# geloescht/mxnet-maintenance

Measured on AMD Instinct MI355X. Metric: images/sec (whole node) ResNet-50 fp16 batch 256/GPU at 1/2/4/8 MI355X, higher is better.
Workload: dtype fp16; 1 GPU; model=ResNet-50 v1b, global_batch=256, per_gpu_batch=256, image_size=224, parallelism=dp1, layout=NHWC, optimizer=mp-SGD momentum 0.9, lr 0.1 (linear warm-up 40 steps), hip_graph=True, deterministic=True

## Files before the change

mxnet_maintenance_amd/ops/kernel_fns.py:

```python
import os

import torch

from . import kernels as _K
from .. import _state
from ..utils import env as _env

__all__ = ['BatchNormNHWC', 'BatchNormDualTailNHWC', 'SoftmaxCE', 'GlobalAvgPoolNHWC', 'flat_sgd']

_DT = {torch.float32: 0, torch.float16: 1, torch.bfloat16: 2}


def _stream():
    return torch.cuda.current_stream().cuda_stream


def _p(t):
    return 0 if t is None else t.data_ptr()


def _f32(t):
    if t.dtype == torch.float32 and t.is_contiguous():
        return t
    m = getattr(t, '_mxamd_master', None)
# ... 314 lines not shown
        zout = torch.empty(5, C, dtype=torch.float32, device=dev)
        dg_ptr, db_ptr, accum, direct, _k1 = _bn_param_grad_dst(gamma_ref, beta_ref, need[2], need[3], out, C, dev)
        zdg_ptr, zdb_ptr, zaccum, zdirect, _k2 = _bn_param_grad_dst(zgamma_ref, zbeta_ref, need[4], need[5], zout, C,
                                                                    dev)
        ride = training and _BN_TAIL_DS[0]
        dkw, zpart, znblk = {}, None, 0
        if ride:
            znblk = lib.bn_tail_ds_rows(R, C)
            zpart = torch.empty(2 * znblk * C, dtype=torch.float32, device=dev)
            dkw = dict(ds_z=z.data_ptr(), ds_mean=zmean.data_ptr(), ds_part=zpart.data_ptr())
        else:
            zpart = torch.empty(2 * lib.bn_partials_rows(R, C) * C, dtype=torch.float32, device=dev)
        lib.bn_nhwc_backward(dt, x.data_ptr(), gy.data_ptr(), 0, mask.data_ptr(), dx.data_ptr(), 0, g.data_ptr(),
                             mean.data_ptr(), invstd.data_ptr(), 0, 0, part.data_ptr(), dg_ptr, db_ptr,
                             out[2].data_ptr(), R, C, 3, 0, int(training), accum, _stream(), ext_nblk, **dkw)
        lib.bn_nhwc_backward(dt, z.data_ptr(), gy.data_ptr(), 0, mask.data_ptr(), dzs.data_ptr(), 0, zg.data_ptr(),
                             zmean.data_ptr(), zinvstd.data_ptr(), 0, 0, zpart.data_ptr(), zdg_ptr, zdb_ptr,
                             zout[2].data_ptr(), R, C, 3, 0, int(training), zaccum, _stream(), znblk)
        dgamma = None if direct or not need[2] else out[0].to(gdt)
        dbeta = None if direct or not need[3] else out[1].to(bdt)
        zdgamma = None if zdirect or not need[4] else zout[0].to(zgdt)
        zdbeta = None if zdirect or not need[5] else zout[1].to(zbdt)
        return dx, dzs, dgamma, dbeta, zdgamma, zdbeta, None, None, None, None, None, None, None


def bnrelu_pool_ok(x, kernel, stride, pad):
    return (bn_ok(x) and tuple(kernel) == (3, 3) and pool_ok(x, kernel, stride, pad)
            and x.numel() + 256 * 32 * 256 * 8 < 2 ** 31 and hasattr(_K.lib(), 'pool_nhwc_forward_bnrelu'))


class SoftmaxCE(torch.autograd.Function):

    @staticmethod
    def forward(ctx, logits, label):
        lib = _K.lib()
        N, K = logits.shape
        lab = label.reshape(-1)
        is_int = not lab.is_floating_point()
        lab = lab.to(torch.int64).contiguous() if is_int else lab.float().contiguous()
        loss = torch.empty(N, dtype=torch.float32, device=logits.device)
        lse = torch.empty(N, dtype=torch.float32, device=logits.device)
        lib.softmax_ce_forward(_DT[logits.dtype], int(is_int), logits.data_ptr(), lab.data_ptr(), loss.data_ptr(),
                               lse.data_ptr(), N, K, _stream())
        ctx.save_for_backward(logits, lab, lse)
        ctx.is_int = is_int
        return loss

    @staticmethod
    def backward(ctx, gout):
        lib = _K.lib()
        logits, lab, lse = ctx.saved_tensors
        N, K = logits.shape
        g = gout.float().contiguous()
        dl = torch.empty_like(logits)
        lib.softmax_ce_backward(_DT[logits.dtype], int(ctx.is_int), logits.data_ptr(), lab.data_ptr(),
                                lse.data_ptr(), g.data_ptr(), dl.data_ptr(), N, K, _stream())
        return dl, None


class GlobalAvgPoolNHWC(torch.autograd.Function):
    @staticmethod
    def forward(ctx, x):
        lib = _K.lib()
        x = x.contiguous()
        N, C = x.shape[0], x.shape[-1]
        HW = x.numel() // (N * C)
        y = torch.empty((N,) + (1,) * (x.dim() - 2) + (C,), dtype=x.dtype, device=x.device)
        lib.gap_nhwc_forward(_DT[x.dtype], x.data_ptr(), y.data_ptr(), N, HW, C, _stream())
        ctx.shape = x.shape
        return y

    @staticmethod
    def backward(ctx, gy):
        lib = _K.lib()
        shape = ctx.shape
        N, C = shape[0], shape[-1]
        HW = int(torch.tensor(shape[1:-1]).prod())
        gy = gy.contiguous()
        dx = torch.empty(shape, dtype=gy.dtype, device=gy.device)
        lib.gap_nhwc_backward(_DT[gy.dtype], gy.data_ptr(), dx.data_ptr(), N, HW, C, _stream())
        return dx


def gap_ok(x):
    return x.dtype in _DT and x.is_contiguous() and x.shape[-1] % 8 == 0


class ReluHip(torch.autograd.Function):

    @staticmethod
    def forward(ctx, x):
        x = x.contiguous()
        y = torch.empty_like(x)
        _K.lib().relu_forward(_DT[x.dtype], x.data_ptr(), y.data_ptr(), x.numel(), _stream())
        ctx.save_for_backward(y)
        return y

    @staticmethod
    def backward(ctx, gy):
        y, = ctx.saved_tensors
        gy = gy.contiguous()
        dx = torch.empty_like(y)
        _K.lib().relu_backward(_DT[y.dtype], y.data_ptr(), gy.data_ptr(), dx.data_ptr(), y.numel(), _stream())
        return dx


def relu_ok(x):
    return x.dtype in _DT and x.is_cuda and x.numel() > 0 and x.data_ptr() % 16 == 0 and x.is_contiguous()


_PW_OPS = {'add': 0, 'sub': 1, 'mul': 2, 'div': 3, 'maximum': 4, 'minimum': 5}


def _bcast_strides(t, shape):
    lead = len(shape) - t.dim()
    st = [0] * lead + list(t.stride())
    sz = [1] * lead + list(t.shape)
    return [0 if sz[d] == 1 and shape[d] != 1 else st[d] for d in range(len(shape))]


def _collapse(shape, sa, sb):
    dims = [(n, a, b) for n, a, b in zip(shape, sa, sb) if n != 1] or [(1, 0, 0)]
    out = [list(dims[-1])]
    for n, a, b in reversed(dims[:-1]):
        pn, pa, pb = out[0]
        if a == pa * pn and b == pb * pn:
            out[0] = [n * pn, pa, pb]
        else:
            out.insert(0, [n, a, b])
    return [d[0] for d in out], [d[1] for d in out], [d[2] for d in out]


def _is_row(t, full):
    ts = tuple(t.shape)
    while ts and ts[0] == 1:
        ts = ts[1:]
    return len(ts) <= len(full) and ts == full[len(full) - len(ts):]


def binary_hip(op, a, b):
    shape = torch.broadcast_shapes(a.shape, b.shape)
    out = torch.empty(shape, dtype=a.dtype, device=a.device)
    n = out.numel()
    if n == 0:
        return out
    vec = 4 if a.dtype == torch.float32 else 8
    aligned = a.data_ptr() % 16 == 0 and b.data_ptr() % 16 == 0
    mode, row = 3, 0
    full = tuple(shape)
    if aligned and a.is_contiguous() and b.is_contiguous():
        if tuple(a.shape) == full and tuple(b.shape) == full:
            mode = 0
        elif tuple(a.shape) == full and _is_row(b, full) and b.numel() % vec == 0:
            mode, row = 1, b.numel()
        elif tuple(b.shape) == full and _is_row(a, full) and a.numel() % vec == 0:
            mode, row = 2, a.numel()
    if mode == 3:
        shp, sa, sb = _collapse(list(shape), _bcast_strides(a, shape), _bcast_strides(b, shape))
        if len(shp) > 6:
            return {'add': torch.add, 'sub': torch.sub, 'mul': torch.mul, 'div': torch.div,
                    'maximum': torch.maximum, 'minimum': torch.minimum}[op](a, b)
    else:
        shp, sa, sb = [], [], []
    _K.lib().pointwise_binary(_DT[a.dtype], _PW_OPS[op], a.data_ptr(), b.data_ptr(), out.data_ptr(), n, mode, row,
                              shp, sa, sb, _stream())
    return out


def _sum_to(g, shape):
    if tuple(g.shape) == tuple(shape):
        return g
    return g.sum_to_size(shape) if len(shape) else g.sum()


class BinaryHip(torch.autograd.Function):

    @staticmethod
    def forward(ctx, a, b, op):
        ctx.op = op
        ctx.sa, ctx.sb = tuple(a.shape), tuple(b.shape)
        if op in ('mul', 'div', 'maximum', 'minimum'):
            ctx.save_for_backward(a, b)
        return binary_hip(op, a, b)

    @staticmethod
    def backward(ctx, g):
        op = ctx.op
        g = g.contiguous()
        if op == 'add':
            return _sum_to(g, ctx.sa), _sum_to(g, ctx.sb), None
        if op == 'sub':
            return _sum_to(g, ctx.sa), _sum_to(-g, ctx.sb), None
        a, b = ctx.saved_tensors
        if op == 'mul':
            return _sum_to(binary_hip('mul', g, b), ctx.sa), _sum_to(binary_hip('mul', g, a), ctx.sb), None
        if op == 'div':
            ga = binary_hip('div', g, b)
            gb = -binary_hip('div', binary_hip('mul', ga, a), b)
            return _sum_to(ga, ctx.sa), _sum_to(gb, ctx.sb), None
        take_a = (a >= b) if op == 'maximum' else (a <= b)
        ga = torch.where(take_a, g, torch.zeros_like(g))
        return _sum_to(ga, ctx.sa), _sum_to(g - ga, ctx.sb), None


def binary_ok(a, b):
    return (a.is_cuda and b.is_cuda and a.dtype == b.dtype and a.dtype in _DT and a.numel() > 0 and
            b.numel() > 0 and a.device == b.device)


__all__ += ['ReluHip', 'relu_ok', 'BinaryHip', 'binary_ok', 'binary_hip']




def flat_sgd(w, g, mom, w32, lr, wd, momentum, rescale, clip, hp=None):
    lib = _K.lib()
    n = w.numel()
    assert n % 8 == 0 and g.numel() == n and w.dtype == g.dtype and w.dtype in _DT
    assert mom is None or (mom.dtype == torch.float32 and mom.numel() == n)
    assert w32 is None or (w32.dtype == torch.float32 and w32.numel() == n)
    if momentum == 0.0:
        mom = None
    args = (_DT[w.dtype], w.data_ptr(), g.data_ptr(), _p(mom), _p(w32), n, float(lr), float(wd),
            float(momentum), float(rescale), float(clip), _stream())
    lib.flat_sgd(*args) if hp is None else lib.flat_sgd(*args, hp.data_ptr())



import os as _os

_CONV_HIP = _env.get('MXAMD_CONV_HIP') != 0


def conv_ok_shape(x, w, stride, pad, dilate=(1, 1), groups=1):
    return (_CONV_HIP and x.dim() == 4 and w.dim() == 4 and groups == 1 and tuple(dilate) == (1, 1)
            and x.dtype in (torch.float16, torch.bfloat16) and w.dtype == x.dtype
            and x.is_contiguous() and w.is_contiguous() and x.shape[3] % 32 == 0 and w.shape[0] % 64 == 0
            and w.shape[3] == x.shape[3] and x.numel() < 2 ** 31 and x.data_ptr() % 16 == 0
            and w.data_ptr() % 16 == 0)


def stem_ok(x, w, stride, pad, bias=None):
    return (_CONV_HIP and bias is None and x.dim() == 4 and w.dim() == 4 and x.dtype in (torch.float16, torch.bfloat16)
            and w.dtype == x.dtype and x.is_contiguous() and w.is_contiguous() and 1 <= x.shape[3] <= 4
            and w.shape[3] == x.shape[3] and w.shape[0] == 64 and w.shape[1] <= 8 and w.shape[2] <= 8
            and tuple(stride) == (2, 2) and all(0 <= p < 8 for p in pad) and _K.available()
            and hasattr(_K.lib(), 'conv_stem_fwd'))


def conv_stem_fwd(x, w, pad, bn_stats=False):
    N, H, W, C = x.shape
    K, R, S, _ = w.shape
    Ho = (H + 2 * pad[0] - R) // 2 + 1
    Wo = (W + 2 * pad[1] - S) // 2 + 1
    y = torch.empty((N, Ho, Wo, K), dtype=x.dtype, device=x.device)
    lib = _K.lib()
    part, nparts = None, 0
    if bn_stats:
        nparts = 4 * lib.conv_stem_grid(N, H, W, R, S, pad[0], pad[1])
        part = torch.empty(2 * K * nparts, dtype=torch.float32, device=x.device)
    lib.conv_stem_fwd(_DT[x.dtype], x.data_ptr(), w.data_ptr(), y.data_ptr(), N, H, W, C, K, R, S, 2, 2, pad[0],
                      pad[1], _p(part), nparts, _stream())
    if part is not None:
        y._mxamd_bn_part = (part, nparts)
    return y


def conv_stem_wgrad(x, dy, wshape, pad, out=None, accum=False):
    N, H, W, C = x.shape
    K, R, S, _ = wshape
    dy = dy.contiguous()
    lib = _K.lib()
    slab = torch.empty(lib.conv_stem_wgrad_workspace(N, H, W, R, S, pad[0], pad[1]), dtype=torch.float32,
                       device=x.device)
    if out is None:
        out = torch.empty((K, R, S, C), dtype=x.dtype, device=x.device)
        accum = False
    assert out.is_contiguous() and out.numel() == K * R * S * C and out.dtype in _DT
    lib.conv_stem_wgrad(_DT[x.dtype], x.data_ptr(), dy.data_ptr(), slab.data_ptr(), _DT[out.dtype], out.data_ptr(),
                        int(bool(accum)), N, H, W, C, K, R, S, 2, 2, pad[0], pad[1], _stream())
    return out


_BIG_VARIANTS = {10: (256, 256), 11: (128, 256), 12: (64, 512), 13: (256, 128), 14: (128, 256), 15: (256, 128),
                 16: (256, 256), 17: (128, 256), 18: (64, 512), 19: (256, 128),
                 26: (256, 224), 27: (128, 448)}
_BIG_SKINNY = (14, 15)
_SKINNY_ON = os.environ.get('MXAMD_CONV_SKINNY', '0') == '1'
_RING_VARIANTS = {20: (128, 128), 21: (256, 128), 22: (128, 256), 23: (64, 256), 24: (256, 256), 25: (64, 128)}


def conv_up2_ok(dy, w, stride, pad, xshape):
    K, R, S, C = w.shape
    return (_CONV_HIP and R == 1 and S == 1 and tuple(stride) == (2, 2) and tuple(pad) == (0, 0)
            and dy.dtype in (torch.float16, torch.bfloat16) and dy.is_cuda and dy.dim() == 4 and K % 64 == 0
            and xshape[1] == 2 * dy.shape[1] and xshape[2] == 2 * dy.shape[2] and xshape[3] == C)


def conv_dgrad_up2(dy, w, variant, bn_bwd=None):
    wt = _dgrad_weight(w.contiguous())
    return conv_fwd(dy.contiguous(), wt, (1, 1), (0, 0), None, variant, bn_bwd=bn_bwd, up=2)


def conv_fwd(x, w, stride, pad, bias=None, variant=0, bn_stats=False, addend=None, bn_bwd=None, up=0, dil=(1, 1)):
    N, H, W, C = x.shape
    K, R, S, _ = w.shape
    dil = tuple(dil)
    Ho = (H + 2 * pad[0] - dil[0] * (R - 1) - 1) // stride[0] + 1
    Wo = (W + 2 * pad[1] - dil[1] * (S - 1) - 1) // stride[1] + 1
    assert dil == (1, 1) or (variant in _BIG_VARIANTS and not bn_stats and bn_bwd is None and up == 0), \
        'conv_fwd: dilation runs on the big-tile kernel without fused epilogues'
    assert up in (0, 2) and (up == 0 or (variant in _BIG_VARIANTS and addend is None and not bn_stats))
    y = torch.empty((N, Ho * max(up, 1), Wo * max(up, 1), K), dtype=x.dtype, device=x.device)
    if N * Ho * Wo * K >= 2 ** 31:
        raise ValueError('conv_fwd: output too large for 32-bit indexing')
    b = _f32(bias) if bias is not None else None
    if addend is not None:
        assert variant in _BIG_VARIANTS and addend.shape == y.shape and addend.dtype == y.dtype
        addend = addend.contiguous()
    if variant in _RING_VARIANTS:
        assert bias is None and addend is None, 'conv ring kernel: no bias / addend'
        lib = _K.lib()
        v = variant - 20
        part, nparts = None, 0
        if bn_stats:
            nparts = lib.conv_nhwc_fwd_ring_nparts(N, H, W, R, S, stride[0], stride[1], pad[0], pad[1], v)
            part = torch.empty(2 * K * nparts, dtype=torch.float32, device=x.device)
        lib.conv_nhwc_fwd_ring(_DT[x.dtype], x.data_ptr(), w.data_ptr(), y.data_ptr(), _zero_page(x.device).data_ptr(),
                               N, H, W, C, K, R, S, stride[0], stride[1], pad[0], pad[1], v, _p(part), nparts,
                               _stream())
        if part is not None:
            y._mxamd_bn_part = (part, nparts)
        return y
    if variant in _BIG_VARIANTS:
        lib = _K.lib()
        v = variant - 10
        part, nparts = None, 0
        if bn_stats:
            nparts = lib.conv_nhwc_fwd_big_nparts(N, H, W, R, S, stride[0], stride[1], pad[0], pad[1], v)
            part = torch.empty(2 * K * nparts, dtype=torch.float32, device=x.device)
        bkw = {}
        if bn_bwd is not None:
            z, bmean, bscale, bshift, bmask, bmode, token = bn_bwd
            assert z.shape == y.shape and z.dtype == y.dtype and z.is_contiguous()
            bnp = lib.conv_nhwc_fwd_big_bwd_nparts(N, H, W, R, S, stride[0], stride[1], pad[0], pad[1], v)
            bpart = torch.empty(2 * K * bnp, dtype=torch.float32, device=x.device)
            bkw = dict(bn_z=z.data_ptr(), bn_mean=bmean.data_ptr(), bn_scale=_p(bscale), bn_shift=_p(bshift),
                       bn_mask=_p(bmask), bn_mode=int(bmode), bn_part=bpart.data_ptr(), bn_nparts=bnp)
        lib.conv_nhwc_fwd_big(_DT[x.dtype], x.data_ptr(), w.data_ptr(), _p(b), y.data_ptr(),
                              _zero_page(x.device).data_ptr(), N, H, W, C, K, R, S, stride[0], stride[1],
                              pad[0], pad[1], v, _p(part), nparts, _p(addend), _stream(), up=int(up), dh=dil[0],
                              dw=dil[1], **bkw)
        if bkw:
            y._mxamd_bn_bwd = (bpart, bnp, bn_bwd[6], y._version)
        if part is not None:
            y._mxamd_bn_part = (part, nparts)
        return y
    if variant in (5, 6):
        lib = _K.lib()
        bco = 128 if variant == 5 else 64
        bkw = _glds_bnb(bn_bwd, y, lib.conv_glds_bwd_nparts(N * Ho * Wo, bco))
        part = bkw.pop('_part', None)
        lib.conv_nhwc_fwd_glds(_DT[x.dtype], x.data_ptr(), w.data_ptr(), _p(b), y.data_ptr(),
                               _zero_page(x.device).data_ptr(), N, H, W, C, K, R, S, stride[0], stride[1],
                               pad[0], pad[1], bco, _stream(), **bkw)
        if part is not None:
            y._mxamd_bn_bwd = (part, bkw['bn_nparts'], bn_bwd[6], y._version)
        return y
    _K.lib().conv_nhwc_fwd(_DT[x.dtype], x.data_ptr(), w.data_ptr(), _p(b), y.data_ptr(), N, H, W, C, K, R, S,
                           stride[0], stride[1], pad[0], pad[1], int(variant), _stream())
    return y


def halo_ok(x, w, stride, pad):
    K, R, S, C = w.shape
    return (_CONV_HIP and x.is_cuda and x.dtype in (torch.float16, torch.bfloat16) and x.dim() == 4
            and x.is_contiguous() and w.is_contiguous() and x.data_ptr() % 16 == 0 and w.data_ptr() % 16 == 0
            and hasattr(_K.lib(), 'conv3x3_halo')
            and bool(_K.lib().conv3x3_halo_ok(C, K, R, S, stride[0], stride[1], pad[0], pad[1], x.shape[2])))


def conv_halo(x, w, bn_stats=False, bn_bwd=None):
    N, H, W, C = x.shape
    K = w.shape[0]
    lib = _K.lib()
    y = torch.empty((N, H, W, K), dtype=x.dtype, device=x.device)
    nparts = lib.conv3x3_halo_nparts(N, H)
    part = torch.empty(2 * K * nparts, dtype=torch.float32, device=x.device) if (bn_stats or bn_bwd) else None
    kw = {}
    if bn_bwd is not None:
        z, bmean, bscale, bshift, _bmask, bmode, _token = bn_bwd
        assert int(bmode) in (0, 2) and z.shape == y.shape and z.dtype == y.dtype and z.is_contiguous()
        kw = dict(bn_z=z.data_ptr(), bn_mean=bmean.data_ptr(), bn_scale=_p(bscale), bn_shift=_p(bshift),
                  bn_mode=int(bmode), bn_part=part.data_ptr())
    lib.conv3x3_halo(_DT[x.dtype], x.data_ptr(), w.data_ptr(), y.data_ptr(), _zero_page(x.device).data_ptr(), N, H,
                     W, C, K, _p(part) if bn_bwd is None else 0, nparts if bn_bwd is None else 0, s=_stream(), **kw)
    if bn_bwd is not None:
        y._mxamd_bn_bwd = (part, nparts, bn_bwd[6], y._version)
    elif part is not None:
        y._mxamd_bn_part = (part, nparts)
    return y


def glds_bnb_ok(bn_src):
    return bn_src is not None and int(bn_src[5]) in (0, 2) and hasattr(_K.lib(), 'conv_glds_bwd_nparts')


def _glds_bnb(bn_bwd, y, nparts):
    if bn_bwd is None:
        return {}
    z, bmean, bscale, bshift, _bmask, bmode, _token = bn_bwd
    assert int(bmode) in (0, 2) and z.shape == y.shape and z.dtype == y.dtype and z.is_contiguous()
    part = torch.empty(2 * y.shape[-1] * nparts, dtype=torch.float32, device=y.device)
    return dict(bn_z=z.data_ptr(), bn_mean=bmean.data_ptr(), bn_scale=_p(bscale), bn_shift=_p(bshift),
                bn_part=part.data_ptr(), bn_nparts=nparts, _part=part)


_ZERO = {}


def _zero_page(dev):
    z = _ZERO.get(dev)
    if z is None:
        z = _ZERO[dev] = torch.zeros(128, dtype=torch.float16, device=dev)
    return z


def _fwd_variants(C, K, bias=False, ktot=None):
    v = []
    if C % 64 == 0 and not bias:
        v.extend(b for b, (bco, _bpix) in sorted(_RING_VARIANTS.items()) if K % bco == 0)
    if C % 64 == 0:
        v.extend(b for b, (bco, _bpix) in sorted(_BIG_VARIANTS.items())
                 if K % bco == 0 and (b not in _BIG_SKINNY or (_SKINNY_ON and ktot == 64)))
    if C % 64 == 0 and K % 128 == 0:
        v.append(5)
    if C % 64 == 0:
        v.append(6)
    if K % 128 == 0 and C % 64 == 0:
        v.append(1)
    if K % 128 == 0:
        v.append(2)
    if C % 64 == 0:
        v.append(3)
    v.append(4)
    return v


def conv_wgrad_ok(x, w):
    return (_CONV_HIP and x.dim() == 4 and w.dim() == 4 and x.dtype in (torch.float16, torch.bfloat16)
            and x.is_contiguous() and x.shape[3] % 64 == 0 and w.shape[0] % 64 == 0 and w.shape[3] == x.shape[3]
            and x.numel() < 2 ** 31 and x.data_ptr() % 16 == 0)


def conv_wgrad(x, dy, wshape, stride, pad, out=None, accum=False, dma=True, ring=0, dil=(1, 1)):
    N, H, W, C = x.shape
    K, R, S, _ = wshape
    dy = dy.contiguous()
    assert dy.dtype == x.dtype and dy.shape[0] == N and dy.shape[3] == K
    dh, dw = dil
    Ho = (H + 2 * pad[0] - dh * (R - 1) - 1) // stride[0] + 1
    Wo = (W + 2 * pad[1] - dw * (S - 1) - 1) // stride[1] + 1
    assert tuple(dy.shape[1:3]) == (Ho, Wo), 'conv_wgrad: dy shape does not match the conv geometry'
    assert dy.numel() < 2 ** 31 and dy.data_ptr() % 16 == 0
    lib = _K.lib()
    if ring:
        ws = lib.conv_nhwc_wgrad_ring_workspace(N, H, W, C, K, R, S, stride[0], stride[1], pad[0], pad[1], ring,
                                                dh=dh, dw=dw)
    else:
        ws = lib.conv_nhwc_wgrad_workspace(N, H, W, C, K, R, S, stride[0], stride[1], pad[0], pad[1], dh=dh, dw=dw)
    slab = torch.empty(ws, dtype=torch.float32, device=x.device)
    if out is None:
        out = torch.empty((K, R, S, C), dtype=x.dtype, device=x.device)
        accum = False
    assert out.is_contiguous() and out.numel() == K * R * S * C and out.dtype in _DT
    if ring:
        lib.conv_nhwc_wgrad_ring(_DT[x.dtype], x.data_ptr(), dy.data_ptr(), slab.data_ptr(), _DT[out.dtype],
                                 out.data_ptr(), int(bool(accum)), N, H, W, C, K, R, S, stride[0], stride[1], pad[0],
                                 pad[1], _zero_page(x.device).data_ptr(), int(ring), _stream(), dh=dh, dw=dw)
        return out
    lib.conv_nhwc_wgrad(_DT[x.dtype], x.data_ptr(), dy.data_ptr(), slab.data_ptr(), _DT[out.dtype], out.data_ptr(),
                        int(bool(accum)), N, H, W, C, K, R, S, stride[0], stride[1], pad[0], pad[1],
                        _zero_page(x.device).data_ptr() if dma else 0, _stream(), dh=dh, dw=dw)
    return out


def _taps_t(w, out, src, base, rstride):
    K, R, S, C = w.shape
    for i in range(0, len(src), 32):
        _K.lib().weight_taps_t(w.element_size(), w.data_ptr(), out.data_ptr(), K, R * S, C, src[i:i + 32],
                               base[i:i + 32], rstride[i:i + 32], _stream())
    return out


def _dgrad_weight(w):
    K, R, S, C = w.shape
    if not (w.is_cuda and w.is_contiguous() and w.element_size() in (2, 4) and _K.available()):
        return w.flip(1, 2).permute(3, 1, 2, 0).contiguous()
    T = R * S
    out = torch.empty((C, R, S, K), dtype=w.dtype, device=w.device)
    return _taps_t(w, out, [T - 1 - t for t in range(T)], [t * K for t in range(T)], [T * K] * T)


def transpose2d(w):
    R, C = w.shape
    if w.is_cuda and w.is_contiguous() and w.element_size() in (2, 4) and R % 8 == 0 and C % 8 == 0:
        return _dgrad_weight(w.view(R, 1, 1, C)).view(C, R)
    return w.t().contiguous()


def _phase_taps(R, P, s, ph):
    return sorted(((ph + P - r) // s, r) for r in range(R) if (ph + P - r) % s == 0)


def conv_dgrad_strided_ok(dy, w, stride, pad, xshape, bco=128):
    K, R, S, C = w.shape
    s = tuple(stride)
    return (_CONV_HIP and s != (1, 1) and s[0] == s[1] and s[0] <= 2 and dy.dtype in (torch.float16, torch.bfloat16)
            and dy.dim() == 4 and K % 64 == 0 and C % bco == 0 and xshape[1] % s[0] == 0 and xshape[2] % s[1] == 0
            and dy.is_cuda and all(0 <= p < k for p, k in zip(pad, (R, S))))


_PHASE_PLANS = {}


def _phase_plan(wshape, stride, pad, device):
    key = (tuple(wshape), tuple(stride), tuple(pad), device)
    plan = _PHASE_PLANS.get(key)
    if plan is not None:
        return plan
    K, R, S, C = wshape
    st = stride[0]
    phases, empty, idx, off = [], [], [], 0
    for ph in range(st):
        th = _phase_taps(R, pad[0], st, ph)
        for pw in range(st):
            tw = _phase_taps(S, pad[1], st, pw)
            if not th or not tw:
                empty.append((ph, pw))
                continue
            dh = [d for d, _ in th]
            dw = [d for d, _ in tw]
            if dh != list(range(dh[0], dh[0] + len(dh))) or dw != list(range(dw[0], dw[0] + len(dw))):
                raise ValueError('conv_dgrad_strided: non-contiguous phase taps')
            nt = len(th) * len(tw)
            for i, (_, r) in enumerate(th):
                for j, (_, c) in enumerate(tw):
                    idx.append((r * S + c, off + (i * len(tw) + j) * K, nt * K))
            phases.append((ph, pw, len(th), len(tw), -dh[0], -dw[0], off))
            off += C * nt * K
    plan = (phases, empty, (idx, off))
    _PHASE_PLANS[key] = plan
    return plan


def conv_dgrad_strided(dy, w, stride, pad, xshape, bco=128, bn_bwd=None):
    K, R, S, C = w.shape
    N, H, W, _ = xshape
    st = stride[0]
    Ho, Wo = H // st, W // st
    dy = dy.contiguous()
    phases, empty, gidx = _phase_plan(w.shape, stride, pad, w.device)
    if len(phases) > 4:
        raise ValueError('conv_dgrad_strided: at most 4 phases per launch')
    dx = torch.empty((N, H, W, C), dtype=dy.dtype, device=dy.device)
    if len(empty) > 3:
        raise ValueError('conv_dgrad_strided: at most 3 phases without taps')
    slots, total = gidx
    wsub = _taps_t(w.contiguous(), torch.empty(total, dtype=w.dtype, device=w.device), [t[0] for t in slots],
                   [t[1] for t in slots], [t[2] for t in slots])
    cols = list(zip(*phases))
    lib = _K.lib()
    bkw = _glds_bnb(bn_bwd, dx, len(phases) * lib.conv_glds_bwd_nparts(N * Ho * Wo, bco)) if bn_bwd else {}
    part = bkw.pop('_part', None)
    lib.conv_nhwc_dgrad_phases_glds(_DT[dy.dtype], dy.data_ptr(), wsub.data_ptr(), dx.data_ptr(),
                                    _zero_page(dy.device).data_ptr(), N, dy.shape[1], dy.shape[2], K, C, Ho, Wo,
                                    st, list(cols[0]), list(cols[1]), list(cols[2]), list(cols[3]),
                                    list(cols[4]), list(cols[5]), list(cols[6]), [e[0] for e in empty],
                                    [e[1] for e in empty], bco, _stream(), **bkw)
    if part is not None:
        dx._mxamd_bn_bwd = (part, bkw['bn_nparts'], bn_bwd[6], dx._version)
    return dx


def _conv_bwd_torch(dy, x, w, stride, pad, mask):
    xc = x.permute(0, 3, 1, 2)
    wc = w.permute(0, 3, 1, 2)
    dyc = dy.permute(0, 3, 1, 2)
    dx, dw, _ = torch.ops.aten.convolution_backward(dyc, xc, wc, None, list(stride), list(pad), [1, 1], False,
                                                    [0, 0], 1, [mask[0], mask[1], False])
    if dx is not None:
        dx = dx.permute(0, 2, 3, 1)
    if dw is not None:
        dw = dw.permute(0, 2, 3, 1)
    return dx, dw



_AUTOTUNE = _env.get('MXNET_CUDNN_AUTOTUNE_DEFAULT') > 0
_ALGO = {}
_TIMES = {}


_REJECTED = {}


def _rel_err(a, b):
    a = a.float()
    b = b.float()
    return float((a - b).abs().max() / (b.abs().max() + 1e-6))


_VENDOR = ('mm', 'miopen')
_VENDOR_PREFIX = ('splitk', 'blaslt', 'sk')
_VENDOR_MARGIN = float(os.environ.get('MXAMD_VENDOR_MARGIN', '0.03'))


def _is_vendor(name):
    return name in _VENDOR or name.startswith(_VENDOR_PREFIX)
_TUNE_ROUNDS = int(os.environ.get('MXAMD_TUNE_ROUNDS', '2'))


def _time_candidates(cands, reps=3, key=None, tol=2e-2):
    ref = None
    ref_name = next((n for n, _ in cands if n in ('mm', 'miopen')), None)
    if ref_name is not None:
        ref = dict(cands)[ref_name]()
        if isinstance(ref, torch.Tensor):
            ref = ref.detach().clone()
        else:
            ref = None
    ok = []
    for name, fn in cands:
        if ref is not None and name != ref_name:
            r = fn()
            if isinstance(r, torch.Tensor) and r.shape == ref.shape:
                err = _rel_err(r, ref)
                if not err <= tol:
                    _REJECTED.setdefault(key, {})[name] = err
                    continue
        ok.append((name, fn))
    times, outs = {}, {}
    for _ in range(_TUNE_ROUNDS):
        for name, fn in ok:
            fn()
            t, r = _measure(fn, reps)
            if name not in times or t < times[name]:
                times[name] = t
                outs[name] = r
    names = [n for n, _ in cands]
    agreed = _agree_times([times.get(n, float('inf')) for n in names])
    best, best_t = None, None
    for name, t in zip(names, agreed):
        if t == float('inf'):
            continue
        if key is not None:
            _TIMES.setdefault(key, {})[name] = t / reps
        if _is_vendor(name):
            t *= 1.0 + _VENDOR_MARGIN
        if best_t is None or t < best_t:
            best, best_t = name, t
    if best is not None and best not in outs:
        best = None
    return best, (outs[best] if best is not None else None)


def _measure(fn, reps):
    if torch.cuda.is_available():
        s, e = torch.cuda.Event(enable_timing=True), torch.cuda.Event(enable_timing=True)
        s.record()
        for _ in range(reps):
            r = fn()
        e.record()
        e.synchronize()
        return s.elapsed_time(e), r
    import time
    t0 = time.perf_counter()
    for _ in range(reps):
        r = fn()
    return (time.perf_counter() - t0) * 1e3, r


def _agree_times(vals):
    from ..parallel import dist
    if dist.world_size() <= 1 or not vals:
        return vals
    t = torch.tensor(vals, dtype=torch.float64)
    dist.all_reduce(t, op='max')
    return [float(v) for v in t.tolist()]


_DETERMINISTIC = [_env.get('MXNET_ENFORCE_DETERMINISM') != 0]
_NONDET = ('mm', 'miopen', 'sk', 'splitk', 'bmm', 'blaslt')


def _apply_torch_determinism(flag):
    torch.backends.cudnn.deterministic = bool(flag)
    if flag:
        torch.backends.cudnn.benchmark = False
    try:
        torch.use_deterministic_algorithms(bool(flag), warn_only=True)
    except Exception:
        pass


def set_deterministic(flag):
    _DETERMINISTIC[0] = bool(flag)
    _apply_torch_determinism(flag)


def deterministic():
    return _DETERMINISTIC[0]


if _DETERMINISTIC[0]:
    _apply_torch_determinism(True)


def _det_filter(cands):
    if not _DETERMINISTIC[0] or cands is None:
        return cands
    keep = [(n, f) for n, f in cands if not n.startswith(_NONDET)]
    return keep or cands


def _akey(key):
    return key + ('det',) if _DETERMINISTIC[0] else key


_FILE_ALGO = {}
_FILE_STATE = {'loaded': False}


def _tuning_file():
    return os.environ.get('MXAMD_AUTOTUNE_FILE', '')


def _load_tuning_file():
    if _FILE_STATE['loaded']:
        return
    _FILE_STATE['loaded'] = True
    path = _tuning_file()
    if path and os.path.exists(path):
        import json
        try:
            with open(path) as f:
                _FILE_ALGO.update(json.load(f))
        except (OSError, ValueError):
            pass


def _save_tuning_file(key, name):
    path = _tuning_file()
    if not path or name is None:
        return
    from ..parallel import dist
    if dist.rank() != 0:
        return
    import json
    _FILE_ALGO[repr(key)] = name
    tmp = path + '.tmp'
    try:
        with open(tmp, 'w') as f:
            json.dump(_FILE_ALGO, f, indent=0, sort_keys=True)
        os.replace(tmp, path)
    except OSError:
        pass


def _select(key, cands, default, timing=None):
    key = _akey(key)
    cands = _det_filter(cands)
    timing = _det_filter(timing)
    _load_tuning_file()
    name = _ALGO.get(key)
    if name is None:
        name = _FILE_ALGO.get(repr(key))
        if name is not None and name in dict(cands):
            _ALGO[key] = name
    if name is None:
        if _AUTOTUNE and not torch.cuda.is_current_stream_capturing() and len(cands) > 1:
            name, out = _time_candidates(timing or cands, key=key)
            _ALGO[key] = name
            _save_tuning_file(key, name)
            return out
        name = default
    table = dict(cands)
    return (table[name] if name in table else cands[0][1])()


_NCU = {}


def _num_cus(dev):
    n = _NCU.get(dev)
    if n is None:
        n = _NCU[dev] = torch.cuda.get_device_properties(dev).multi_processor_count
    return n


def pw_ok(x, kin, nout):
    return (_CONV_HIP and x.is_cuda and x.dtype in (torch.float16, torch.bfloat16) and x.is_contiguous()
            and x.data_ptr() % 16 == 0 and hasattr(_K.lib(), 'conv_pw_stream')
            and bool(_K.lib().conv_pw_stream_ok(int(kin), int(nout))))


def pw_bnb_ok(kin, nout, add, bn_src):
    return (bn_src is not None and int(bn_src[5]) in (2, 3) and hasattr(_K.lib(), 'conv_pw_stream_bnb_ok')
            and bool(_K.lib().conv_pw_stream_bnb_ok(int(kin), int(nout), int(bool(add)), int(bn_src[5]))))


def conv_pw(x, w2, bn_stats=False, addend=None, bn_bwd=None, addend_mask=None):
    C = x.shape[-1]
    K = w2.shape[0]
    M = x.numel() // C
    wt = int(w2.dim() == 2 and w2.stride() == (1, K) and not w2.is_contiguous() and w2.data_ptr() % 16 == 0
             and K % 8 == 0)
    if not wt:
        w2 = w2.contiguous()
    y = torch.empty(x.shape[:-1] + (K,), dtype=x.dtype, device=x.device)
    if addend is not None:
        addend = addend.contiguous()
        if tuple(addend.shape) != tuple(y.shape) or addend.dtype != y.dtype or addend.data_ptr() % 16:
            raise ValueError('conv_pw: addend must match the output (shape, dtype, 16-byte alignment)')
    lib = _K.lib()
    grid = lib.conv_pw_stream_grid(M, C, K, _num_cus(x.device), int(addend is not None or bn_bwd is not None))
    nparts = grid // max(1, lib.conv_pw_stream_slices(C, K))
    part = torch.empty(2 * K * nparts, dtype=torch.float32, device=x.device) if (bn_stats or bn_bwd) else None
    bkw = {}
    if bn_bwd is not None:
        assert not bn_stats, 'conv_pw: forward and backward statistics are exclusive'
        z, bmean, bscale, bshift, bmask, bmode, _token = bn_bwd
        assert z.shape == y.shape and z.dtype == y.dtype and z.is_contiguous() and z.data_ptr() % 16 == 0
        bkw = dict(bn_z=z.data_ptr(), bn_mask=_p(bmask), bn_mean=bmean.data_ptr(), bn_scale=_p(bscale),
                   bn_shift=_p(bshift), bn_mode=int(bmode))
    if addend_mask is not None:
        assert bn_bwd is not None and addend is not None and addend_mask.dtype == torch.uint8
        assert addend_mask.numel() * 8 == addend.numel() and addend_mask.is_contiguous()
        bkw['addend_mask'] = addend_mask.data_ptr()
    lib.conv_pw_stream(_DT[x.dtype], x.data_ptr(), w2.data_ptr(), y.data_ptr(), _zero_page(x.device).data_ptr(), M, C,
                       K, _p(part), grid, _stream(), _p(addend), wt, **bkw)
    if bn_bwd is not None:
        y._mxamd_bn_bwd = (part, nparts, bn_bwd[6], y._version)
    elif part is not None:
        y._mxamd_bn_part = (part, nparts)
    return y


def _fwd_candidates(x, w, stride, pad, bias):
    c = []
    K, R, S, C = w.shape
    if (R == 1 and S == 1 and tuple(stride) == (1, 1) and tuple(pad) == (0, 0) and bias is None
            and pw_ok(x, C, K)):
        c.append(('pw', lambda: conv_pw(x, w.reshape(K, C), bn_stats=bool(_state.STATE.training))))
    if stem_ok(x, w, stride, pad, bias):
        c.append(('stem', lambda: conv_stem_fwd(x, w, pad, bn_stats=bool(_state.STATE.training))))
    if bias is None and halo_ok(x, w, stride, pad):
        c.append(('halo', lambda: conv_halo(x, w, bn_stats=bool(_state.STATE.training))))
    if conv_ok_shape(x, w, stride, pad):
        c.append(('hip', lambda: conv_fwd(x, w, stride, pad, bias)))
        stats = bool(_state.STATE.training)
        for v in _fwd_variants(C, K, bias is not None, ktot=R * S * C):
            c.append(('hip%d' % v, lambda v=v: conv_fwd(x, w, stride, pad, bias, v, bn_stats=stats)))
    if R == 1 and S == 1 and tuple(stride) == (1, 1) and tuple(pad) == (0, 0):
        x2, w2 = x.reshape(-1, C), w.reshape(K, C)
        for name, fn in _gemm().candidates(x2, w2, bias=bias):
            c.append((name, lambda fn=fn: fn().view(x.shape[0], x.shape[1], x.shape[2], K)))

        def mm():
            y = torch.mm(x.reshape(-1, C), w.reshape(K, C).t())
            if bias is not None:
                y = y + bias.to(y.dtype)
            return y.view(x.shape[0], x.shape[1], x.shape[2], K)
        c.append(('mm', mm))

    def miopen():
        y = torch.nn.functional.conv2d(x.permute(0, 3, 1, 2), w.permute(0, 3, 1, 2), bias, tuple(stride), tuple(pad))
        return y.permute(0, 2, 3, 1).contiguous()
    c.append(('miopen', miopen))
    return c


_STATS_SCRATCH = {}


def _bn_stats_pass(y):
    C = y.shape[-1]
    R = y.numel() // C
    lib = _K.lib()
    n = 2 * lib.bn_partials_rows(R, C) * C
    buf = _STATS_SCRATCH.get(y.device)
    if buf is None or buf.numel() < n:
        buf = _STATS_SCRATCH[y.device] = torch.empty(n, dtype=torch.float32, device=y.device)
    lib.bn_nhwc_stats(_DT[y.dtype], y.data_ptr(), _zeros_f32(C, y.device).data_ptr(), buf.data_ptr(), R, C,
                      _stream())


def _fwd_timing(cands):
    if not _state.STATE.training:
        return None

    def charged(fn):
        def run():
            y = fn()
            if getattr(y, '_mxamd_bn_part', None) is None and y.shape[-1] % 8 == 0 and y.is_contiguous():
                _bn_stats_pass(y)
            return y
        return run
    return [(n, charged(fn)) for n, fn in cands]


def _fwd_default(x, w, stride):
    K, R, S, C = w.shape
    if C <= 4 and K == 64 and tuple(stride) == (2, 2) and R <= 8 and S <= 8:
        return 'stem'
    if R == 1 and S == 1 and tuple(stride) == (1, 1) and (K >= 256 or x.shape[1] * x.shape[2] <= 784):
        return 'mm'
    return 'hip'


def _dgrad_candidates(dy, x, w, stride, pad):
    c = []
    K, R, S, C = w.shape
    if R == 1 and S == 1 and tuple(stride) == (1, 1) and tuple(pad) == (0, 0):
        c.append(('mm', lambda: torch.mm(dy.reshape(-1, K), w.reshape(K, C)).view(x.shape)))
        if pw_ok(dy, K, C):
            c.append(('pw', lambda: conv_pw(dy, w.reshape(K, C).t())))
        c.extend(_gemm_dgrad_1x1(dy, w, x.shape))
    if (tuple(stride) == (1, 1) and C % 64 == 0 and K % 32 == 0 and 2 * pad[0] == R - 1 and 2 * pad[1] == S - 1
            and _CONV_HIP):
        c.append(('hip', lambda: conv_fwd(dy, _dgrad_weight(w), (1, 1), (R - 1 - pad[0], S - 1 - pad[1]))))
        for v in _fwd_variants(K, C, ktot=R * S * K):
            c.append(('hip%d' % v, lambda v=v: conv_fwd(dy, _dgrad_weight(w), (1, 1), (R - 1 - pad[0], S - 1 - pad[1]),
                                                        None, v)))
    for bco in (128, 64):
        if conv_dgrad_strided_ok(dy, w, stride, pad, x.shape, bco):
            c.append(('phase%d' % bco, lambda bco=bco: conv_dgrad_strided(dy, w, stride, pad, x.shape, bco)))
    if halo_ok(dy, w, stride, pad) and tuple(dy.shape) == tuple(x.shape[:3]) + (K,):
        c.append(('halo', lambda: conv_halo(dy, _dgrad_weight(w))))
    if conv_up2_ok(dy, w, stride, pad, x.shape):
        for v, (bco, _bpix) in sorted(_BIG_VARIANTS.items()):
            if C % bco == 0 and v not in _BIG_SKINNY:
                c.append(('up%d' % v, lambda v=v: conv_dgrad_up2(dy, w, v)))
    c.append(('miopen', lambda: _conv_bwd_torch(dy, x, w, stride, pad, (True, False))[0]))
    return c


def _gemm():
    from . import gemm
    return gemm


def _gemm_dgrad_1x1(dy, w, xshape, addend=None):
    K, C = w.shape[0], w.shape[3]
    G = _gemm()
    d2 = dy.reshape(-1, K)
    if not (K % 64 == 0 and C % 64 == 0 and d2.is_cuda and d2.dtype in G._DT and w.dtype == d2.dtype
            and d2.is_contiguous() and d2.data_ptr() % 16 == 0 and _K.available()):
        return []
    out = []
    for cfg in G.configs(d2.shape[0], C, K, G.AUTOTUNE_TILES):
        def run(cfg=cfg):
            add = addend.contiguous().view(-1, C) if addend is not None else None
            return G.gemm_nt(d2, transpose2d(w.reshape(K, C)), addend=add, cfg=cfg).view(xshape)
        out.append(('gemm%ds%d' % cfg, run))
    return out


def _big_algo(key):
    algo = _ALGO.get(_akey(key))
    if algo and algo.startswith('hip') and algo[3:].isdigit() and int(algo[3:]) in _BIG_VARIANTS:
        return int(algo[3:])
    return None


def _bn_bwd_fusable(bn_src, out_shape):
    return bn_src is not None and _BN_BWD_FUSE[0] and tuple(bn_src[0].shape) == tuple(out_shape)


def _charge_bn_bwd(cands, z):
    def charged(fn):
        def run():
            r = fn()
            if isinstance(r, torch.Tensor) and r.shape[-1] % 8 == 0 and r.is_contiguous():
                _bn_stats_pass(r)
                _bn_stats_pass(z)
            return r
        return run
    return [(n, charged(fn)) for n, fn in cands]


def _dgrad_bn_candidates(dy, x, w, stride, pad, bn_src):
    cands = _dgrad_candidates(dy, x, w, stride, pad)
    K, R, S, C = w.shape
    fused = []
    if (R == 1 and S == 1 and tuple(stride) == (1, 1) and tuple(pad) == (0, 0) and pw_ok(dy, K, C)
            and pw_bnb_ok(K, C, False, bn_src)):
        fused.append(('pw+bn', lambda: conv_pw(dy, w.reshape(K, C).t(), bn_bwd=bn_src)))
    if (_CONV_HIP and tuple(stride) == (1, 1) and 2 * pad[0] == R - 1 and 2 * pad[1] == S - 1
            and K % 64 == 0):
        for v in _fwd_variants(K, C, ktot=R * S * K):
            if v in _BIG_VARIANTS or (v in (5, 6) and glds_bnb_ok(bn_src)):
                fused.append(('hip%d+bn' % v, lambda v=v: conv_fwd(dy, _dgrad_weight(w), (1, 1),
                                                                   (R - 1 - pad[0], S - 1 - pad[1]), None, v,
                                                                   bn_bwd=bn_src)))
    if conv_up2_ok(dy, w, stride, pad, x.shape):
        for v, (bco, _bpix) in sorted(_BIG_VARIANTS.items()):
            if C % bco == 0 and v not in _BIG_SKINNY:
                fused.append(('up%d+bn' % v, lambda v=v: conv_dgrad_up2(dy, w, v, bn_bwd=bn_src)))
    if glds_bnb_ok(bn_src) and halo_ok(dy, w, stride, pad) and tuple(dy.shape) == tuple(x.shape[:3]) + (K,):
        fused.append(('halo+bn', lambda: conv_halo(dy, _dgrad_weight(w), bn_bwd=bn_src)))
    if glds_bnb_ok(bn_src):
        for bco in (128, 64):
            if conv_dgrad_strided_ok(dy, w, stride, pad, x.shape, bco):
                fused.append(('phase%d+bn' % bco, lambda bco=bco: conv_dgrad_strided(dy, w, stride, pad, x.shape, bco,
                                                                                     bn_bwd=bn_src)))
    return cands + fused, _charge_bn_bwd(cands, bn_src[0]) + fused


def _dgrad_default(w, stride):
    K, R, S, C = w.shape
    if tuple(stride) != (1, 1):
        return 'miopen'
    if R == 1 and S == 1:
        return 'mm' if C >= 128 else 'miopen'
    return 'hip' if C >= 128 and C % 64 == 0 else 'miopen'


def _wgrad_candidates(dy, x, w, stride, pad):
    c = [('miopen', lambda: _conv_bwd_torch(dy, x, w, stride, pad, (False, True))[1])]
    K, R, S, C = w.shape
    if stem_ok(x, w, stride, pad):
        c.insert(0, ('stem', lambda: conv_stem_wgrad(x, dy, w.shape, pad)))
    if conv_wgrad_ok(x, w):
        c.insert(0, ('hip', lambda: conv_wgrad(x, dy, w.shape, stride, pad)))
        c.insert(1, ('hipreg', lambda: conv_wgrad(x, dy, w.shape, stride, pad, dma=False)))
        lib = _K.lib()
        for v in range(1, 10):
            if lib.conv_nhwc_wgrad_ring_ok(C, K, R, S, v):
                c.insert(2, ('ring%d' % v, lambda v=v: conv_wgrad(x, dy, w.shape, stride, pad, ring=v)))
    if R == 1 and S == 1 and tuple(stride) == (1, 1) and tuple(pad) == (0, 0):
        P = dy.numel() // K
        for chunks in (16, 64):
            if P % chunks == 0 and P // chunks >= 1024:
                def splitk(chunks=chunks):
                    return _splitk_wgrad(dy, x, chunks)
                c.append(('splitk%d' % chunks, splitk))
    return c


_BMM_OUT_DTYPE = [None]


def _splitk_wgrad(dy, x, chunks, out=None):
    K, C = dy.shape[-1], x.shape[-1]
    P = dy.numel() // K
    d3 = dy.reshape(chunks, P // chunks, K).transpose(1, 2)
    x3 = x.reshape(chunks, P // chunks, C)
    part = _bmm_f32(d3, x3)
    if not part.is_contiguous() or (K * C) % 4:
        r = part.sum(0).view(K, 1, 1, C)
        if out is not None:
            out.add_(r.view(out.shape))
            return None
        return r
    lib = _K.lib()
    if out is None:
        r = torch.empty(K, 1, 1, C, dtype=torch.float32, device=dy.device)
        lib.slab_reduce(0, part.data_ptr(), chunks, K * C, r.data_ptr(), 0, _stream())
        return r
    lib.slab_reduce(_DT[out.dtype], part.data_ptr(), chunks, K * C, out.data_ptr(), 1, _stream())
    return None


def _bmm_f32(a, b):
    if _BMM_OUT_DTYPE[0] is not False:
        try:
            r = torch.bmm(a, b, out_dtype=torch.float32)
            _BMM_OUT_DTYPE[0] = True
            return r
        except (RuntimeError, TypeError):
            _BMM_OUT_DTYPE[0] = False
    return torch.bmm(a, b).float()


def _wgrad(dy, x, w, w_ref, stride, pad):
    key = ('wgrad', tuple(x.shape), tuple(w.shape), tuple(stride), tuple(pad), x.dtype)
    algo = _ALGO.get(_akey(key))
    if algo == 'stem':
        tgt = _leaf_grad(w_ref, dtype=w.dtype)
        if tgt is not None:
            conv_stem_wgrad(x, dy, w.shape, pad, out=tgt, accum=True)
            return None
    if algo in ('hip', 'hipreg') or (algo or '').startswith('ring'):
        tgt = _leaf_grad(w_ref, dtype=w.dtype)
        if tgt is not None:
            conv_wgrad(x, dy, w.shape, stride, pad, out=tgt, accum=True, dma=algo == 'hip',
                       ring=int(algo[4:]) if algo.startswith('ring') else 0)
            return None
    elif algo is not None and algo.startswith('splitk'):
        tgt = _leaf_grad(w_ref, dtype=w.dtype)
        if tgt is not None:
            _splitk_wgrad(dy, x, int(algo[6:]), out=tgt)
            return None
    default = 'stem' if stem_ok(x, w, stride, pad) else ('hip' if conv_wgrad_ok(x, w) else 'miopen')
    dw = _select(key, _wgrad_candidates(dy, x, w, stride, pad), default)
    if dw.dtype != w.dtype:
        tgt = _leaf_grad(w_ref, dtype=w.dtype)
        if tgt is not None:
            tgt.add_(dw)
            return None
        dw = dw.to(w.dtype)
    return dw


_WGRAD_SIDE = [os.environ.get('MXAMD_WGRAD_STREAM', '0') == '1']
_SIDE_STREAMS = {}
_SIDE_KEEP = []
_SIDE_DIRTY = set()


def join_side_streams():
    if not _SIDE_DIRTY:
        return
    for dev in list(_SIDE_DIRTY):
        torch.cuda.current_stream(dev).wait_stream(_SIDE_STREAMS[dev])
    _SIDE_DIRTY.clear()
    del _SIDE_KEEP[:]


def _wgrad_maybe_side(dy, x, w, w_ref, stride, pad):
    if not (_WGRAD_SIDE[0] and dy.is_cuda):
        return _wgrad(dy, x, w, w_ref, stride, pad)
    dev = dy.device.index
    side = _SIDE_STREAMS.get(dev)
    if side is None:
        side = _SIDE_STREAMS[dev] = torch.cuda.Stream(device=dev)
        from .. import engine
        engine.add_join_hook(join_side_streams)
    main = torch.cuda.current_stream(dev)
    side.wait_stream(main)
    with torch.cuda.stream(side):
        dw = _wgrad(dy, x, w, w_ref, stride, pad)
    _SIDE_KEEP.append((dy, x))
    _SIDE_DIRTY.add(dev)
    if dw is not None:
        main.wait_stream(side)
        dw.record_stream(main)
    return dw


class ConvNHWC(torch.autograd.Function):

    @staticmethod
    def forward(ctx, x, w, bias, stride, pad, dilate):
        key = ('fwd', tuple(x.shape), tuple(w.shape), tuple(stride), tuple(pad), x.dtype, bias is not None)
        cands = _fwd_candidates(x, w, stride, pad, bias)
        y = _select(key, cands, _fwd_default(x, w, stride), timing=_fwd_timing(cands))
        ctx.save_for_backward(x, w)
        ctx.stride, ctx.pad = stride, pad
        ctx.has_bias = bias is not None
        ctx.b_ref = bias
        ctx.w_ref = w
        ctx.bn_src = getattr(x, '_mxamd_bn_src', None)
        return y

    @staticmethod
    def backward(ctx, dy):
        x, w = ctx.saved_tensors
        dy = dy.contiguous()
        stride, pad = ctx.stride, ctx.pad
        dx = dw = db = None
        if ctx.needs_input_grad[1] and _WGRAD_SIDE[0]:
            dw = _wgrad_maybe_side(dy, x, w, ctx.w_ref, stride, pad)
        if ctx.needs_input_grad[0]:
            key = ('dgrad', tuple(x.shape), tuple(w.shape), tuple(stride), tuple(pad), x.dtype)
            if _bn_bwd_fusable(ctx.bn_src, x.shape):
                cands, timing = _dgrad_bn_candidates(dy, x, w, stride, pad, ctx.bn_src)
                dx = _select(key + ('bnbwd',), cands, _dgrad_default(w, stride), timing=timing)
            else:
                dx = _select(key, _dgrad_candidates(dy, x, w, stride, pad), _dgrad_default(w, stride))
        if ctx.needs_input_grad[1] and not _WGRAD_SIDE[0]:
            dw = _wgrad(dy, x, w, ctx.w_ref, stride, pad)
        if ctx.has_bias and ctx.needs_input_grad[2]:
            db = _conv_bias_grad(dy, ctx.b_ref)
        return dx, dw, db, None, None, None


def _conv_bias_grad(dy, b_ref):
    from .nlp_fns import bias_grad
    return bias_grad(dy.reshape(-1, dy.shape[-1]), b_ref, b_ref.dtype)


class ConvTeeNHWC(torch.autograd.Function):

    @staticmethod
    def forward(ctx, x, w, inplace_grad=False):
        stride, pad = (1, 1), (0, 0)
        key = ('fwd', tuple(x.shape), tuple(w.shape), stride, pad, x.dtype, False)
        cands = _fwd_candidates(x, w, stride, pad, None)
        y = _select(key, cands, _fwd_default(x, w, stride), timing=_fwd_timing(cands))
        ctx.save_for_backward(x, w)
        ctx.w_ref = w
        ctx.inplace_grad = inplace_grad
        ctx.bn_src = getattr(x, '_mxamd_bn_src', None)
        xp = x.view_as(x)
        xp._mxamd_tee_key = _tee_key(x, w, ctx.bn_src)
        return y, xp

    @staticmethod
    def backward(ctx, gy, gpass):
        x, w = ctx.saved_tensors
        K, C = w.shape[0], w.shape[3]
        dx = dw = None
        if gy is None:
            return gpass, None, None
        gy = gy.contiguous()
        if ctx.needs_input_grad[1] and _WGRAD_SIDE[0]:
            dw = _wgrad_maybe_side(gy, x, w, ctx.w_ref, (1, 1), (0, 0))
        if ctx.needs_input_grad[0]:
            dx = _tee_dgrad(gy, x, w, gpass, ctx.inplace_grad, ctx.bn_src)
        if ctx.needs_input_grad[1] and not _WGRAD_SIDE[0]:
            dw = _wgrad(gy, x, w, ctx.w_ref, (1, 1), (0, 0))
        return dx, dw, None


def _tee_key(x, w, bn_src):
    return ('teedgrad', tuple(x.shape), tuple(w.shape), x.dtype) + (('bnbwd',) if _bn_bwd_fusable(bn_src, x.shape)
                                                                     else ())


_LAZY_DZ = [os.environ.get('MXAMD_LAZY_SHORTCUT_GRAD', '1') != '0']
_LAZY_USED = [0]


def lazy_shortcut_ok(tee_key):
    return _LAZY_DZ[0] and tee_key is not None and _ALGO.get(_akey(tee_key)) == 'pw+bn'


def _unpack_lazy_dz(gpass):
    lz = getattr(gpass, '_mxamd_lazy_mask', None) if gpass is not None else None
    if lz is None or lz[1] != gpass._version:
        return None
    return lz[0]


def _materialize_dz(gpass, mask):
    bits = (mask.view(-1, 1) >> torch.arange(8, device=mask.device, dtype=torch.uint8)) & 1
    return gpass * bits.view(gpass.shape).to(gpass.dtype)


def _tee_dgrad(gy, x, w, gpass, inplace, bn_src=None):
    K, C = w.shape[0], w.shape[3]
    g2 = gy.reshape(-1, K)
    w2 = w.reshape(K, C)
    amask = _unpack_lazy_dz(gpass)
    if amask is not None:
        key = _tee_key(x, w, bn_src)
        if (_ALGO.get(_akey(key)) == 'pw+bn' and _bn_bwd_fusable(bn_src, x.shape) and pw_ok(gy, K, C)
                and pw_bnb_ok(K, C, True, bn_src) and gpass.is_contiguous() and gpass.data_ptr() % 16 == 0):
            _LAZY_USED[0] += 1
            return conv_pw(gy, w2.t(), addend=gpass, bn_bwd=bn_src, addend_mask=amask)
        gpass, inplace = _materialize_dz(gpass, amask), True

    def mm():
        if gpass is not None and inplace and gpass.is_contiguous():
            return gpass.view(-1, C).addmm_(g2, w2).view(x.shape)
        if gpass is not None:
            return torch.addmm(gpass.contiguous().reshape(-1, C), g2, w2).view(x.shape)
        return torch.mm(g2, w2).view(x.shape)

    cands = []
    fused = []
    fuse_bn = _bn_bwd_fusable(bn_src, x.shape)
    if _CONV_HIP and K % 64 == 0 and gy.dtype in (torch.float16, torch.bfloat16) and gy.numel() < 2 ** 31:
        wt = None
        for v, (bco, _bpix) in sorted(_BIG_VARIANTS.items()):
            if C % bco or (v in _BIG_SKINNY and not (_SKINNY_ON and K == 64)):
                continue
            if wt is None:
                wt = _dgrad_weight(w.contiguous())

            def big(v=v, wt=wt, bn=None):
                add = gpass.contiguous() if gpass is not None else None
                return conv_fwd(gy, wt, (1, 1), (0, 0), None, v, addend=add, bn_bwd=bn)
            cands.append(('hip%d' % v, big))
            if fuse_bn:
                fused.append(('hip%d+bn' % v, lambda big=big: big(bn=bn_src)))
    cands.extend(_gemm_dgrad_1x1(gy, w, x.shape, addend=gpass))
    if pw_ok(gy, K, C) and (gpass is None or (gpass.is_contiguous() and gpass.data_ptr() % 16 == 0)):
        cands.append(('pw', lambda: conv_pw(gy, w2.t(), addend=gpass)))
        if fuse_bn and gpass is not None and pw_bnb_ok(K, C, True, bn_src):
            fused.append(('pw+bn', lambda: conv_pw(gy, w2.t(), addend=gpass, bn_bwd=bn_src)))
    cands.append(('mm', lambda: mm() if not (gpass is not None and inplace) else
                  torch.addmm(gpass.reshape(-1, C), g2, w2).view(x.shape)))
    key = ('teedgrad', tuple(x.shape), tuple(w.shape), x.dtype) + (('bnbwd',) if fuse_bn else ())
    if _ALGO.get(_akey(key)) == 'mm':
        return mm()
    if fuse_bn:
        return _select(key, cands + fused, 'mm', timing=_charge_bn_bwd(cands, bn_src[0]) + fused)
    return _select(key, cands, 'mm')


def conv_tee_ok(x, w):
    return (conv_ok(x, w, (1, 1), (0, 0), (1, 1), 1) and w.shape[1] == 1 and w.shape[2] == 1
            and x.shape[3] == w.shape[3])




def conv_algos():
    return dict(_ALGO)


def conv_algo_times():
    return {k: dict(v) for k, v in _TIMES.items()}


def _conv_bwd_dil_torch(dy, x, w, stride, pad, dil, mask):
    r = torch.ops.aten.convolution_backward(dy.permute(0, 3, 1, 2), x.permute(0, 3, 1, 2), w.permute(0, 3, 1, 2),
                                            None, tuple(stride), tuple(pad), tuple(dil), False, (0, 0), 1,
                                            (mask[0], mask[1], False))
    return (r[0].permute(0, 2, 3, 1).contiguous() if mask[0] else None,
            r[1].permute(0, 2, 3, 1).contiguous() if mask[1] else None)


def dil_ok(x, w, dilate):
    K, R, S, C = w.shape
    return (_CONV_HIP and tuple(dilate) != (1, 1) and C % 64 == 0 and K % 64 == 0 and x.is_contiguous()
            and x.dtype in (torch.float16, torch.bfloat16) and x.numel() < 2 ** 31)


class ConvDilNHWC(torch.autograd.Function):

    @staticmethod
    def forward(ctx, x, w, bias, stride, pad, dilate):
        K, R, S, C = w.shape
        key = ('fwd-dil', tuple(x.shape), tuple(w.shape), tuple(stride), tuple(pad), tuple(dilate), x.dtype,
               bias is not None)
        cands = [('hip%d' % v, lambda v=v: conv_fwd(x, w, stride, pad, bias, v, dil=dilate))
                 for v, (bco, _bpix) in sorted(_BIG_VARIANTS.items()) if K % bco == 0 and v not in _BIG_SKINNY]

        def miopen():
            y = torch.nn.functional.conv2d(x.permute(0, 3, 1, 2), w.permute(0, 3, 1, 2), bias, tuple(stride),
                                           tuple(pad), tuple(dilate))
            return y.permute(0, 2, 3, 1).contiguous()
        cands.append(('miopen', miopen))
        y = _select(key, cands, cands[0][0])
        ctx.save_for_backward(x, w)
        ctx.cfg = (tuple(stride), tuple(pad), tuple(dilate))
        ctx.has_bias = bias is not None
        ctx.b_ref = bias
        return y

    @staticmethod
    def backward(ctx, dy):
        x, w = ctx.saved_tensors
        stride, pad, dil = ctx.cfg
        dy = dy.contiguous()
        K, R, S, C = w.shape
        dx = dw = db = None
        if ctx.needs_input_grad[0]:
            key = ('dgrad-dil', tuple(x.shape), tuple(w.shape), stride, pad, dil, x.dtype)
            cands = []
            pp = (dil[0] * (R - 1) - pad[0], dil[1] * (S - 1) - pad[1])
            if stride == (1, 1) and pp[0] >= 0 and pp[1] >= 0:
                cands = [('hip%d' % v, lambda v=v: conv_fwd(dy, _dgrad_weight(w), (1, 1), pp, None, v, dil=dil))
                         for v, (bco, _bpix) in sorted(_BIG_VARIANTS.items())
                         if C % bco == 0 and v not in _BIG_SKINNY]
            cands.append(('miopen', lambda: _conv_bwd_dil_torch(dy, x, w, stride, pad, dil, (True, False))[0]))
            dx = _select(key, cands, cands[0][0])
        if ctx.needs_input_grad[1]:
            key = ('wgrad-dil', tuple(x.shape), tuple(w.shape), stride, pad, dil, x.dtype)
            cands = []
            if conv_wgrad_ok(x, w):
                cands.append(('hip', lambda: conv_wgrad(x, dy, w.shape, stride, pad, dil=dil)))
                lib = _K.lib()
                for v in range(1, 10):
                    if lib.conv_nhwc_wgrad_ring_ok(C, K, R, S, v):
                        cands.append(('ring%d' % v, lambda v=v: conv_wgrad(x, dy, w.shape, stride, pad, ring=v,
                                                                          dil=dil)))
            cands.append(('miopen', lambda: _conv_bwd_dil_torch(dy, x, w, stride, pad, dil, (False, True))[1]))
            dw = _select(key, cands, cands[0][0]).to(w.dtype)
        if ctx.has_bias and ctx.needs_input_grad[2]:
            db = _conv_bias_grad(dy, ctx.b_ref)
        return dx, dw, db, None, None, None


_KPAD = _os.environ.get('MXAMD_CONV_KPAD', '1') == '1'


def kpad_ok(x, w):
    return _KPAD and w.shape[0] % 64 != 0 and w.shape[3] % 64 == 0 and w.shape[0] >= 8


def conv_kpad(x, w, bias, stride, pad, dilate):
    K = w.shape[0]
    Kp = (K + 63) // 64 * 64
    wp = torch.nn.functional.pad(w, (0, 0, 0, 0, 0, 0, 0, Kp - K))
    bp = None if bias is None else torch.nn.functional.pad(bias, (0, Kp - K))
    return ConvNHWC.apply(x, wp, bp, tuple(stride), tuple(pad), tuple(dilate))[..., :K]


def conv_ok(x, w, stride, pad, dilate, groups):
    return (len(stride) == 2 and x.dim() == 4 and groups == 1 and tuple(dilate) == (1, 1) and x.is_contiguous()
            and w.is_contiguous() and x.dtype in (torch.float16, torch.bfloat16) and w.dtype == x.dtype)


__all__ += ['ConvNHWC', 'ConvTeeNHWC', 'ConvDilNHWC', 'dil_ok', 'conv_kpad', 'kpad_ok', 'conv_fwd', 'conv_ok_shape', 'conv_wgrad', 'conv_wgrad_ok', 'stem_ok',
            'conv_stem_fwd', 'conv_stem_wgrad']



def _pool_out(n, k, s, p, full):
    if full:
        return -(-(n + 2 * p - k) // s) + 1
    return (n + 2 * p - k) // s + 1


def pool_ok(x, kernel, stride, pad):
    return (x.dim() == 4 and x.dtype in _DT and x.is_contiguous() and x.shape[3] % 8 == 0 and x.numel() > 0
            and min(x.shape[1] + 2 * pad[0] - kernel[0], x.shape[2] + 2 * pad[1] - kernel[1]) >= 0
            and len(kernel) == 2 and kernel[0] * kernel[1] <= 256 and x.data_ptr() % 16 == 0
            and all(p < k for p, k in zip(pad, kernel)))


class PoolNHWC(torch.autograd.Function):

    @staticmethod
    def forward(ctx, x, pool_type, kernel, stride, pad, full, count_include_pad):
        N, H, W, C = x.shape
        Ho = _pool_out(H, kernel[0], stride[0], pad[0], full)
        Wo = _pool_out(W, kernel[1], stride[1], pad[1], full)
        is_max = pool_type == 'max'
        y = torch.empty((N, Ho, Wo, C), dtype=x.dtype, device=x.device)
        arg = torch.empty((N, Ho, Wo, C), dtype=torch.uint8, device=x.device) if is_max else None
        geo = (N, H, W, C, Ho, Wo, kernel[0], kernel[1], stride[0], stride[1], pad[0], pad[1],
               int(bool(count_include_pad)))
        _K.lib().pool_nhwc_forward(_DT[x.dtype], int(is_max), x.data_ptr(), y.data_ptr(), _p(arg), *geo, _stream())
        ctx.geo, ctx.is_max, ctx.dt = geo, is_max, x.dtype
        if is_max:
            ctx.save_for_backward(arg)
        return y

    @staticmethod
    def backward(ctx, dy):
        dy = dy.contiguous()
        geo = ctx.geo
        arg = ctx.saved_tensors[0] if ctx.is_max else None
        dx = torch.empty((geo[0], geo[1], geo[2], geo[3]), dtype=ctx.dt, device=dy.device)
        _K.lib().pool_nhwc_backward(_DT[ctx.dt], int(ctx.is_max), dy.data_ptr(), _p(arg), dx.data_ptr(), *geo,
                                    _stream())
        return dx, None, None, None, None, None, None


__all__ += ['PoolNHWC']
```

src/kernels/bindings.cc:

```cpp
#include <hip/hip_runtime.h>
#include <pybind11/pybind11.h>
#include <pybind11/stl.h>

#include <cstdint>
#include <stdexcept>
#include <vector>

namespace py = pybind11;

namespace mxamd {
void bn_nhwc_forward(int dtype, const void* x, const void* addend, void* y, uint8_t* mask, const float* gamma,
                     const float* beta,
                     const float* center, float* part, float* mean, float* invstd, float* var, float* scale,
                     float* shift, int64_t R, int C, float eps, int training, int relu, int fix_gamma,
                     float momentum, float* mm_upd, float* mv_upd, int ext_nblk, hipStream_t s, const float* ascale,
                     const float* ashift);
void bn_nhwc_backward(int dtype, const void* x, const void* dy, const void* y, const uint8_t* mask, void* dx,
                      void* dz,
                      const float* gamma, const float* mean, const float* invstd, const float* fscale,
                      const float* fshift, float* part, float* dgamma, float* dbeta, float* coef, int64_t R, int C,
                      int relu_mode, int fix_gamma, int training, int accum, hipStream_t s, int ext_nblk, const void* ds_z, const float* ds_mean, float* ds_part);
int bn_partials_rows(int64_t R, int C);
int bn_tail_ds_rows(int64_t R, int C);
void gemm_nt(int dtype, const void* a, const void* b, const void* bias, const void* addend, void* c, int out_f32,
             int M, int N, int K, int lda, int ldb, int ldc, int act, int cfg, int splits, float* ws, hipStream_t s,
             int bias_lowp);
int gemm_nt_tile_n(int cfg);
int gemm_nt_tile_m(int cfg);
void int8_gemm(const int8_t* A, const int8_t* B, int32_t* C, int M, int N, int K, hipStream_t s);
void csr_dot_dense(int dtype, const int64_t* indptr, const int64_t* indices, const void* vals, const void* rhs,
                   void* out, int64_t M, int64_t K, int N, hipStream_t s);
void csrT_dot_dense(int dtype, const int64_t* indptr, const int64_t* indices, const void* vals, const void* rhs,
                    const int64_t* slot, float* out32, int64_t M, int64_t K, int N, hipStream_t s);
void embedding_forward(int dtype, int itype, const void* idx, const void* w, void* y, int64_t n, int V, int C,
                       hipStream_t s);
void embedding_backward(int dtype, int itype, const void* idx, const void* dy, float* acc, uint8_t* touched,
                        int out_dtype, void* grad, int accum, int64_t n, int V, int C, hipStream_t s);
int bn_nhwc_stats(int dtype, const void* x, const float* center, float* part, int64_t R, int C, hipStream_t s,
                  int total_blocks);
int64_t colsum_partials(int64_t R, int C);
void colsum_rows(int dtype, const void* x, const float* zeros, float* part, int64_t R, int C, int out_dtype,
                 void* out, int accum, hipStream_t s);
void softmax_ce_forward(int dtype, int label_is_int, const void* logits, const void* label, float* loss, float* lse,
                        int N, int K, hipStream_t s);
void softmax_ce_backward(int dtype, int label_is_int, const void* logits, const void* label, const float* lse,
                         const float* gout, void* dlogits, int N, int K, hipStream_t s);
void gap_nhwc_forward(int dtype, const void* x, void* y, int N, int HW, int C, hipStream_t s);
void relu_forward(int dtype, const void* x, void* y, int64_t n, hipStream_t s);
void relu_backward(int dtype, const void* y, const void* dy, void* dx, int64_t n, hipStream_t s);
void pointwise_binary(int dtype, int op, const void* a, const void* b, void* out, int64_t n, int mode, int64_t row,
                      int ndim, const int64_t* shape, const int64_t* astride, const int64_t* bstride, hipStream_t s);
void gap_nhwc_backward(int dtype, const void* dy, void* dx, int N, int HW, int C, hipStream_t s);
void flat_sgd(int dtype, void* w, const void* g, float* mom, float* w32, int64_t n, float lr, float wd,
              float momentum, float rescale, float clip, const float* hp, hipStream_t s);
void conv_nhwc_fwd(int dtype, const void* x, const void* w, const float* bias, void* y, int N, int H, int W, int C,
                   int K, int R, int S, int sh, int sw, int ph, int pw, int variant, hipStream_t s);
int conv_nhwc_fwd_big_nparts(int N, int H, int W, int R, int S, int sh, int sw, int ph, int pw, int variant);
void conv_nhwc_fwd_big(int dtype, const void* x, const void* w, const float* bias, void* y, const void* zero, int N,
                       int H, int W, int C, int K, int R, int S, int sh, int sw, int ph, int pw, int variant,
                       float* part, int nparts, const void* addend, hipStream_t s, const void* bn_z,
                       const float* bn_mean, const float* bn_scale, const float* bn_shift, const uint8_t* bn_mask,
                       int bn_mode, float* bn_part, int bn_nparts, int up, int dh, int dw);
int conv_nhwc_fwd_big_bwd_nparts(int N, int H, int W, int R, int S, int sh, int sw, int ph, int pw, int variant);
void conv_nhwc_fwd_glds(int dtype, const void* x, const void* w, const float* bias, void* y, const void* zero, int N,
                        int H, int W, int C, int K, int R, int S, int sh, int sw, int ph, int pw, int bco,
                        hipStream_t s, const void* bn_z, const float* bn_mean, const float* bn_scale,
                        const float* bn_shift, float* bn_part, int bn_nparts);
int conv_glds_bwd_nparts(int M, int bco);
void conv_nhwc_dgrad_phases_glds(int dtype, const void* dy, const void* w, void* dx, const void* zero, int N, int Hi,
                                 int Wi, int Cin, int Cout, int Ho, int Wo, int stride, int nph, const int* ph,
                                 const int* pw, const int* R, const int* S, const int* pad_h, const int* pad_w,
                                 const int64_t* w_off, int nzero, const int* zph, const int* zpw, int bco,
                                 hipStream_t s, const void* bn_z, const float* bn_mean, const float* bn_scale,
                                 const float* bn_shift, float* bn_part, int bn_nparts);
int conv_nhwc_fwd_ring_nparts(int N, int H, int W, int R, int S, int sh, int sw, int ph, int pw, int variant);
void conv_nhwc_fwd_ring(int dtype, const void* x, const void* w, void* y, const void* zero, int N, int H, int W, int C,
                        int K, int R, int S, int sh, int sw, int ph, int pw, int variant, float* part, int nparts,
                        hipStream_t s);
bool conv3x3_halo_ok(int C, int K, int R, int S, int sh, int sw, int ph, int pw, int W);
int conv3x3_halo_nparts(int N, int H);
void conv3x3_halo(int dtype, const void* x, const void* w, void* y, const void* zero, int N, int H, int W, int C, int K,
                  float* part, int nparts, const void* bn_z, const float* bn_mean, const float* bn_scale,
                  const float* bn_shift, int bn_mode, float* bn_part, hipStream_t s);
int conv_nhwc_wgrad_ring_ok(int C, int K, int R, int S, int variant);
int64_t conv_nhwc_wgrad_ring_workspace(int N, int H, int W, int C, int K, int R, int S, int sh, int sw, int ph, int pw,
                                       int variant, int dh, int dw);
void conv_nhwc_wgrad_ring(int dtype, const void* x, const void* dy, float* slab, int out_dtype, void* out, int accum,
                          int N, int H, int W, int C, int K, int R, int S, int sh, int sw, int ph, int pw,
                          const void* zero, int variant, hipStream_t s, int dh, int dw);
int64_t conv_nhwc_wgrad_workspace(int N, int H, int W, int C, int K, int R, int S, int sh, int sw, int ph, int pw,
                                  int dh, int dw);
void conv_nhwc_wgrad(int dtype, const void* x, const void* dy, float* slab, int out_dtype, void* out, int accum, int N,
                     int H, int W, int C, int K, int R, int S, int sh, int sw, int ph, int pw, const void* zero,
                     hipStream_t s, int dh, int dw);
int conv_stem_grid(int N, int H, int W, int R, int S, int ph, int pw);
void conv_stem_fwd(int dtype, const void* x, const void* w, void* y, int N, int H, int W, int C, int K, int R, int S,
                   int sh, int sw, int ph, int pw, float* part, int nparts, hipStream_t s);
int64_t conv_stem_wgrad_workspace(int N, int H, int W, int R, int S, int ph, int pw);
void conv_stem_wgrad(int dtype, const void* x, const void* dy, float* slab, int out_dtype, void* out, int accum, int N,
                     int H, int W, int C, int K, int R, int S, int sh, int sw, int ph, int pw, hipStream_t s);
int layernorm_bwd_partials(int M);
void layernorm_forward(int dtype, const void* x, const void* gamma, const void* beta, int pt, void* y, float* mean,
                       float* rstd, int M, int D, float eps, hipStream_t s);
void layernorm_backward(int dtype, const void* x, const void* dy, const void* gamma, int pt, const float* mean,
                        const float* rstd, void* dx, float* part, void* dgamma, void* dbeta, int gdtype, int accum,
                        int M, int D, hipStream_t s);
void add_dropout_ln_forward(int dtype, const void* x, const void* h, const void* gamma, const void* beta, int pt,
                            void* y, void* s_out, uint8_t* mask, float* mean, float* rstd, int M, int D, float eps,
                            float p, uint64_t seed, const uint64_t* seed_base, hipStream_t s);
void add_dropout_ln_backward(int dtype, const void* s_in, const void* dy, const void* gamma, int pt, const float* mean,
                             const float* rstd, const uint8_t* mask, float p, void* ds, void* dh, float* part,
                             float* hpart, void* dgamma, void* dbeta, int gdtype, int accum, int M, int D,
                             hipStream_t s);
void column_sum_partials(int gdtype, const float* part, int nb, int ncol, void* out, int accum, hipStream_t s);
void gelu_forward(int dtype, const void* x, void* y, int64_t n, hipStream_t s);
void gelu_backward(int dtype, const void* x, const void* dy, void* dx, int64_t n, hipStream_t s);
void gelu_backward_colpart(int dtype, const void* x, const void* dy, void* dx, float* part, int M, int N,
                           hipStream_t s);
int gelu_colpart_blocks(int M, int N);
void softmax_forward(int dtype, int log, const void* x, void* y, int M, int L, float scale, hipStream_t s);
void softmax_backward(int dtype, int log, const void* y, const void* dy, void* dx, int M, int L, float scale,
                      hipStream_t s);
void dropout_forward(int dtype, const void* x, void* y, uint8_t* mask, int64_t n, float p, uint64_t seed,
                     const uint64_t* seed_base, hipStream_t s);
void dropout_backward(int dtype, const void* dy, const uint8_t* mask, void* dx, int64_t n, float p, hipStream_t s);
int attention_max_seq();
void attention_forward(int dtype, const void* qkv, const float* kmask, void* out, float* lse, int S, int B, int H,
                       int D, float scale, float p, uint64_t seed, const uint64_t* seed_base, hipStream_t s);
void attention_backward(int dtype, const void* qkv, const float* kmask, const void* out, const void* dout,
                        const float* lse, float* delta, void* dqkv, int S, int B, int H, int D, float scale, float p,
                        uint64_t seed, const uint64_t* seed_base, hipStream_t s);
void flat_adam(int dtype, int mode, void* w, const void* g, float* mean, float* var, float* w32, int64_t n, float lr,
               float beta1, float beta2, float eps, float wd, float eta, float rescale, float clip, const float* hp,
               hipStream_t s);
void lamb_update(int dtype, void* w, const void* g, float* mean, float* var, float* w32, float* upd,
                 const void* chunks, int nchunks, float* nrm, int nseg, float lr, float beta1, float beta2, float eps,
                 float bc1, float bc2, float wd, float rescale, float clip, float lb, float ub, const float* hp,
                 hipStream_t s);
void seg_sumsq(int dtype, const void* x, const void* chunks, int nchunks, float* out, int nseg, hipStream_t s);
void all_finite(int dtype, const void* x, int64_t n, float scale, int* flag, int init, hipStream_t s);
void pool_nhwc_forward(int dtype, int is_max, const void* x, void* y, uint8_t* arg, int N, int H, int W, int C,
                       int Ho, int Wo, int kh, int kw, int sh, int sw, int ph, int pw, int cip, hipStream_t s,
                       const float* scale, const float* shift);
int bn_pool_bwd_blocks();
void bn_pool_backward(int dtype, const void* x, const void* dy, const uint8_t* arg, void* dx, const float* gamma,
                      const float* mean, const float* invstd, const float* fscale, const float* fshift, float* part,
                      float* dgamma, float* dbeta, float* coef, int N, int H, int W, int C, int Ho, int Wo, int kh,
                      int kw, int sh, int sw, int ph, int pw, int fix_gamma, int training, int accum,
                      hipStream_t s);
void pool_nhwc_backward(int dtype, int is_max, const void* dy, const uint8_t* arg, void* dx, int N, int H, int W,
                        int C, int Ho, int Wo, int kh, int kw, int sh, int sw, int ph, int pw, int cip,
                        hipStream_t s);
void deform_im2col(int dtype, const void* x, const void* off, const void* msk, void* cols, int N, int C, int H, int W,
                   int Ho, int Wo, int kh, int kw, int sh, int sw, int ph, int pw, int dh, int dw, int dg,
                   int rows, hipStream_t s);
void deform_col2im(int dtype, const void* off, const void* msk, const void* gcols, float* gx, int N, int C, int H,
                   int W, int Ho, int Wo, int kh, int kw, int sh, int sw, int ph, int pw, int dh, int dw, int dg,
                   int rows, hipStream_t s);
void deform_col2im_coord(int dtype, const void* x, const void* off, const void* msk, const void* gcols, void* goff,
                         void* gmsk, int N, int C, int H, int W, int Ho, int Wo, int kh, int kw, int sh, int sw,
                         int ph, int pw, int dh, int dw, int dg, int rows, hipStream_t s);
void deform_im2col_nhwc(int dtype, const void* x, const void* off, const void* msk, void* cols, const int* g,
                        int ld_off, int ld_msk, hipStream_t s);
void deform_bwd_nhwc(int dtype, const void* x, const void* off, const void* msk, const void* gcols, float* gx,
                     void* goff, void* gmsk, const int* g, int ld_off, int ld_msk, hipStream_t s);
void conv_dw_fwd(int dtype, const void* x, const void* wt, const float* bias, void* y, const int* gm, hipStream_t s);
void conv_dw_dgrad(int dtype, const void* dy, const void* wt, void* dx, const int* gm, hipStream_t s);
void conv_dw_wgrad(int dtype, const void* x, const void* dy, float* slab, int nslice, int out_dtype, void* out,
                   int accum, const int* gm, hipStream_t s);
int ssd_loss_blocks(int rows);
void ssd_loss_fwd(int dtype, const void* cls, const void* loc, const float* cls_t, const float* loc_t,
                  const float* loc_m, int rows, int C1, float lambd, float* part, float* out, hipStream_t s);
void ssd_loss_bwd(int dtype, const void* cls, const void* loc, const float* cls_t, const float* loc_t,
                  const float* loc_m, const float* stats, const float* gout, int rows, int C1, float lambd, void* dcls,
                  void* dloc, hipStream_t s);
void multibox_target(int dtype, const float* anchors, const float* labels, const void* cls_pred, float* loc_target,
                     float* loc_mask, float* cls_target, float* match_iou, int* match_gt, uint32_t* key, int B, int A,
                     int L, int W, int C, float thr, float ignore_label, float neg_ratio, float neg_thresh,
                     int min_neg, float v0, float v1, float v2, float v3, hipStream_t s);
void slab_reduce(int out_dtype, float* slab, int splits, int64_t n, void* out, int accum, hipStream_t s);
void twobit_quantize(int dtype, const void* g, float* res, void* packed, int64_t n, float thr, hipStream_t s);
void twobit_dequantize_sum(const void* packed, int64_t row_bytes, int nrows, int64_t n, float thr, float* out,
                           hipStream_t s);
int conv_pw_stream_ok(int kin, int nout);
int conv_pw_stream_grid(int M, int kin, int nout, int ncu, int add);
int conv_pw_stream_slices(int kin, int nout);
void weight_taps_t(int elem_bytes, const void* w, void* out, int K, int RS, int C, int n, const int* src,
                   const int64_t* base, const int64_t* rstride, hipStream_t s);
void conv_pw_stream(int dtype, const void* x, const void* w, void* y, const void* zero, int M, int kin, int nout,
                    float* part, int grid, hipStream_t s, const void* addend, int wt, const void* bn_z,
                    const uint8_t* bn_mask, const float* bn_mean, const float* bn_scale, const float* bn_shift,
                    int bn_mode, const uint8_t* addend_mask);
int conv_pw_stream_bnb_ok(int kin, int nout, int add, int mode);
void conv_gen(int dtype, int mode, const void* src, const void* wsrc, const float* bias, void* dst, const int* geom,
              int splits, hipStream_t s);
void rnn_fwd_seq(int dtype, int mode, const float* gx, const void* h0, const float* c0, const void* whh,
                 const float* bhh, void* out, int ldo, float* cseq, float* save, int Tn, int N, int H, int reverse,
                 hipStream_t s);
void rnn_bwd_seq(int dtype, int mode, const void* whhT, const void* dy, int ldy, const float* dhT,
                 const float* save, const float* cseq, const float* c0, const void* h0, const void* out, int ldo,
                 void* dgh, void* dgx, float* dc, float* dhd, float* dh0, int Tn, int N, int H, int reverse,
                 hipStream_t s);
}

using namespace mxamd;

template <typename T>
static inline T* P(uintptr_t p) {
  return reinterpret_cast<T*>(p);
}
static inline hipStream_t S(uintptr_t s) { return reinterpret_cast<hipStream_t>(s); }
static inline hipStream_t S_(uintptr_t s) { return reinterpret_cast<hipStream_t>(s); }

static void check_launch(const char* name) {
  hipError_t e = hipGetLastError();
  if (e != hipSuccess) throw std::runtime_error(std::string(name) + ": " + hipGetErrorString(e));
}

PYBIND11_MODULE(_hip_kernels, m) {
  m.doc() = "gfx950 HIP kernels for mxnet_maintenance_amd";
  m.attr("arch") = "gfx950";

  m.def("bn_partials_rows", &bn_partials_rows);
  m.def("bn_tail_ds_rows", &bn_tail_ds_rows);
  m.def("bn_nhwc_stats", [](int dt, uintptr_t x, uintptr_t center, uintptr_t part, int64_t R, int C, uintptr_t s) {
    int nblk = bn_nhwc_stats(dt, P<const void>(x), P<const float>(center), P<float>(part), R, C, S(s), 512);
    check_launch("bn_nhwc_stats");
    return nblk;
  });
  m.def("embedding_forward", [](int dt, int it, uintptr_t idx, uintptr_t w, uintptr_t y, int64_t n, int V, int C,
                                uintptr_t s) {
    embedding_forward(dt, it, P<const void>(idx), P<const void>(w), P<void>(y), n, V, C, S(s));
    check_launch("embedding_forward");
  });
  m.def("embedding_backward", [](int dt, int it, uintptr_t idx, uintptr_t dy, uintptr_t acc, uintptr_t touched,
                                 int odt, uintptr_t grad, int accum, int64_t n, int V, int C, uintptr_t s) {
    embedding_backward(dt, it, P<const void>(idx), P<const void>(dy), P<float>(acc), P<uint8_t>(touched), odt,
                       P<void>(grad), accum, n, V, C, S(s));
    check_launch("embedding_backward");
  });
  m.def("csr_dot_dense", [](int dt, uintptr_t indptr, uintptr_t indices, uintptr_t vals, uintptr_t rhs, uintptr_t out,
                            int64_t M, int64_t K, int N, uintptr_t s) {
    csr_dot_dense(dt, P<const int64_t>(indptr), P<const int64_t>(indices), P<const void>(vals), P<const void>(rhs),
                  P<void>(out), M, K, N, S(s));
    check_launch("csr_dot_dense");
  });
  m.def("csrT_dot_dense", [](int dt, uintptr_t indptr, uintptr_t indices, uintptr_t vals, uintptr_t rhs,
                             uintptr_t slot, uintptr_t out32, int64_t M, int64_t K, int N, uintptr_t s) {
    csrT_dot_dense(dt, P<const int64_t>(indptr), P<const int64_t>(indices), P<const void>(vals), P<const void>(rhs),
                   P<const int64_t>(slot), P<float>(out32), M, K, N, S(s));
    check_launch("csrT_dot_dense");
  });
  m.def("int8_gemm", [](uintptr_t a, uintptr_t b, uintptr_t c, int M, int N, int K, uintptr_t s) {
    int8_gemm(P<const int8_t>(a), P<const int8_t>(b), P<int32_t>(c), M, N, K, S(s));
    check_launch("int8_gemm");
  });
  m.def("colsum_partials", [](int64_t R, int C) { return colsum_partials(R, C); });
  m.def("colsum_rows", [](int dt, uintptr_t x, uintptr_t zeros, uintptr_t part, int64_t R, int C, int odt,
                          uintptr_t out, int accum, uintptr_t s) {
    colsum_rows(dt, P<const void>(x), P<const float>(zeros), P<float>(part), R, C, odt, P<void>(out), accum, S(s));
    check_launch("colsum_rows");
  });
  m.def("twobit_quantize", [](int dt, uintptr_t g, uintptr_t res, uintptr_t packed, int64_t n, float thr,
                              uintptr_t s) {
    twobit_quantize(dt, P<void>(g), P<float>(res), P<void>(packed), n, thr, S(s));
    check_launch("twobit_quantize");
  });
  m.def("twobit_dequantize_sum", [](uintptr_t packed, int64_t row_bytes, int nrows, int64_t n, float thr,
                                    uintptr_t out, uintptr_t s) {
    twobit_dequantize_sum(P<void>(packed), row_bytes, nrows, n, thr, P<float>(out), S(s));
    check_launch("twobit_dequantize_sum");
  });
  m.def("gemm_nt", [](int dt, uintptr_t a, uintptr_t b, uintptr_t bias, uintptr_t addend, uintptr_t c, int out_f32,
                      int M, int N, int K, int lda, int ldb, int ldc, int act, int cfg, int splits, uintptr_t ws,
                      uintptr_t s, int bias_lowp) {
    gemm_nt(dt, P<void>(a), P<void>(b), P<void>(bias), P<void>(addend), P<void>(c), out_f32, M, N, K, lda, ldb, ldc,
            act, cfg, splits, P<float>(ws), S(s), bias_lowp);
    check_launch("gemm_nt");
  }, py::arg("dt"), py::arg("a"), py::arg("b"), py::arg("bias"), py::arg("addend"), py::arg("c"), py::arg("out_f32"),
     py::arg("M"), py::arg("N"), py::arg("K"), py::arg("lda"), py::arg("ldb"), py::arg("ldc"), py::arg("act"),
     py::arg("cfg"), py::arg("splits"), py::arg("ws"), py::arg("s"), py::arg("bias_lowp") = 0);
  m.def("weight_taps_t", [](int eb, uintptr_t w, uintptr_t out, int K, int RS, int C, std::vector<int> src,
                            std::vector<int64_t> base, std::vector<int64_t> rstride, uintptr_t s) {
    if (src.size() != base.size() || src.size() != rstride.size()) throw std::runtime_error("weight_taps_t: table sizes");
    weight_taps_t(eb, P<const void>(w), P<void>(out), K, RS, C, static_cast<int>(src.size()), src.data(), base.data(),
                  rstride.data(), S(s));
    check_launch("weight_taps_t");
  });
  m.def("conv_pw_stream_ok", &conv_pw_stream_ok);
  m.def("conv_pw_stream_slices", &conv_pw_stream_slices);
  m.def("conv_pw_stream_grid", [](int M, int kin, int nout, int ncu, int add) {
    return conv_pw_stream_grid(M, kin, nout, ncu, add);
  }, pybind11::arg("M"), pybind11::arg("kin"), pybind11::arg("nout"), pybind11::arg("ncu"), pybind11::arg("add") = 0);
  m.def("conv_pw_stream", [](int dt, uintptr_t x, uintptr_t w, uintptr_t y, uintptr_t zero, int M, int kin, int nout,
                             uintptr_t part, int grid, uintptr_t s, uintptr_t addend, int wt, uintptr_t bn_z,
                             uintptr_t bn_mask, uintptr_t bn_mean, uintptr_t bn_scale, uintptr_t bn_shift, int bn_mode,
                             uintptr_t addend_mask) {
    conv_pw_stream(dt, P<const void>(x), P<const void>(w), P<void>(y), P<const void>(zero), M, kin, nout,
                   P<float>(part), grid, S(s), P<const void>(addend), wt, P<const void>(bn_z), P<const uint8_t>(bn_mask),
                   P<const float>(bn_mean), P<const float>(bn_scale), P<const float>(bn_shift), bn_mode,
                   P<const uint8_t>(addend_mask));
    check_launch("conv_pw_stream");
  }, pybind11::arg("dt"), pybind11::arg("x"), pybind11::arg("w"), pybind11::arg("y"), pybind11::arg("zero"),
     pybind11::arg("M"), pybind11::arg("kin"), pybind11::arg("nout"), pybind11::arg("part"), pybind11::arg("grid"),
     pybind11::arg("s"), pybind11::arg("addend"), pybind11::arg("wt") = 0, pybind11::arg("bn_z") = 0,
     pybind11::arg("bn_mask") = 0, pybind11::arg("bn_mean") = 0, pybind11::arg("bn_scale") = 0,
     pybind11::arg("bn_shift") = 0, pybind11::arg("bn_mode") = 0, pybind11::arg("addend_mask") = 0);
  m.def("conv_pw_stream_bnb_ok", &conv_pw_stream_bnb_ok);
  m.def("conv_gen", [](int dt, int mode, uintptr_t src, uintptr_t wsrc, uintptr_t bias, uintptr_t dst,
                       std::vector<int> geom, int splits, uintptr_t s) {
    if (geom.size() != 22) throw std::runtime_error("conv_gen: geometry needs 22 ints");
    conv_gen(dt, mode, P<const void>(src), P<const void>(wsrc), P<const float>(bias), P<void>(dst), geom.data(),
             splits, S(s));
    check_launch("conv_gen");
  });
  m.def("rnn_fwd_seq", [](int dt, int mode, uintptr_t gx, uintptr_t h0, uintptr_t c0, uintptr_t whh, uintptr_t bhh,
                          uintptr_t out, int ldo, uintptr_t cseq, uintptr_t save, int T, int N, int H, int reverse,
                          uintptr_t s) {
    rnn_fwd_seq(dt, mode, P<const float>(gx), P<const void>(h0), P<const float>(c0), P<const void>(whh),
                P<const float>(bhh), P<void>(out), ldo, P<float>(cseq), P<float>(save), T, N, H, reverse, S(s));
    check_launch("rnn_fwd_seq");
  });
  m.def("rnn_bwd_seq", [](int dt, int mode, uintptr_t whhT, uintptr_t dy, int ldy, uintptr_t dhT, uintptr_t save,
                          uintptr_t cseq, uintptr_t c0, uintptr_t h0, uintptr_t out, int ldo, uintptr_t dgh,
                          uintptr_t dgx, uintptr_t dc, uintptr_t dhd, uintptr_t dh0, int T, int N, int H, int reverse,
                          uintptr_t s) {
    rnn_bwd_seq(dt, mode, P<const void>(whhT), P<const void>(dy), ldy, P<const float>(dhT), P<const float>(save),
                P<const float>(cseq), P<const float>(c0), P<const void>(h0), P<const void>(out), ldo, P<void>(dgh),
                P<void>(dgx), P<float>(dc), P<float>(dhd), P<float>(dh0), T, N, H, reverse, S(s));
    check_launch("rnn_bwd_seq");
  });
  m.def("gemm_nt_tile_n", &gemm_nt_tile_n);
  m.def("gemm_nt_tile_m", &gemm_nt_tile_m);
  m.def("slab_reduce", [](int odt, uintptr_t slab, int splits, int64_t n, uintptr_t out, int accum, uintptr_t s) {
    slab_reduce(odt, P<float>(slab), splits, n, P<void>(out), accum, S(s));
    check_launch("slab_reduce");
  });
  m.def("deform_im2col", [](int dt, uintptr_t x, uintptr_t off, uintptr_t msk, uintptr_t cols, std::vector<int> g,
                            uintptr_t s) {
    if (g.size() != 15 && g.size() != 16) throw std::runtime_error("deform_im2col: geometry needs 15 or 16 ints");
    const int rows = g.size() == 16 ? g[15] : 0;
    deform_im2col(dt, P<void>(x), P<void>(off), P<void>(msk), P<void>(cols), g[0], g[1], g[2], g[3], g[4], g[5], g[6],
                  g[7], g[8], g[9], g[10], g[11], g[12], g[13], g[14], rows, S(s));
    check_launch("deform_im2col");
  });
  m.def("deform_col2im", [](int dt, uintptr_t off, uintptr_t msk, uintptr_t gcols, uintptr_t gx, std::vector<int> g,
                            uintptr_t s) {
    if (g.size() != 15 && g.size() != 16) throw std::runtime_error("deform_col2im: geometry needs 15 or 16 ints");
    const int rows = g.size() == 16 ? g[15] : 0;
    deform_col2im(dt, P<void>(off), P<void>(msk), P<void>(gcols), P<float>(gx), g[0], g[1], g[2], g[3], g[4], g[5],
                  g[6], g[7], g[8], g[9], g[10], g[11], g[12], g[13], g[14], rows, S(s));
    check_launch("deform_col2im");
  });
  m.def("deform_col2im_coord", [](int dt, uintptr_t x, uintptr_t off, uintptr_t msk, uintptr_t gcols, uintptr_t goff,
                                  uintptr_t gmsk, std::vector<int> g, uintptr_t s) {
    if (g.size() != 15 && g.size() != 16) throw std::runtime_error("deform_col2im_coord: geometry needs 15 or 16 ints");
    const int rows = g.size() == 16 ? g[15] : 0;
    deform_col2im_coord(dt, P<void>(x), P<void>(off), P<void>(msk), P<void>(gcols), P<void>(goff), P<void>(gmsk),
                        g[0], g[1], g[2], g[3], g[4], g[5], g[6], g[7], g[8], g[9], g[10], g[11], g[12], g[13], g[14],
                        rows, S(s));
    check_launch("deform_col2im_coord");
  });
  m.def("deform_im2col_nhwc", [](int dt, uintptr_t x, uintptr_t off, uintptr_t msk, uintptr_t cols, std::vector<int> g,
                                 int ld_off, int ld_msk, uintptr_t s) {
    if (g.size() != 15) throw std::runtime_error("deform_im2col_nhwc: geometry needs 15 ints");
    deform_im2col_nhwc(dt, P<void>(x), P<void>(off), P<void>(msk), P<void>(cols), g.data(), ld_off, ld_msk, S(s));
    check_launch("deform_im2col_nhwc");
  });
  m.def("deform_bwd_nhwc", [](int dt, uintptr_t x, uintptr_t off, uintptr_t msk, uintptr_t gcols, uintptr_t gx,
                              uintptr_t goff, uintptr_t gmsk, std::vector<int> g, int ld_off, int ld_msk, uintptr_t s) {
    if (g.size() != 15) throw std::runtime_error("deform_bwd_nhwc: geometry needs 15 ints");
    deform_bwd_nhwc(dt, P<void>(x), P<void>(off), P<void>(msk), P<void>(gcols), P<float>(gx), P<void>(goff),
                    P<void>(gmsk), g.data(), ld_off, ld_msk, S(s));
    check_launch("deform_bwd_nhwc");
  });
  m.def("conv_dw_fwd", [](int dt, uintptr_t x, uintptr_t wt, uintptr_t bias, uintptr_t y, std::vector<int> g,
                          uintptr_t s) {
    if (g.size() != 14) throw std::runtime_error("conv_dw_fwd: geometry needs 14 ints");
    conv_dw_fwd(dt, P<void>(x), P<void>(wt), P<float>(bias), P<void>(y), g.data(), S(s));
    check_launch("conv_dw_fwd");
  });
  m.def("conv_dw_dgrad", [](int dt, uintptr_t dy, uintptr_t wt, uintptr_t dx, std::vector<int> g, uintptr_t s) {
    if (g.size() != 14) throw std::runtime_error("conv_dw_dgrad: geometry needs 14 ints");
    conv_dw_dgrad(dt, P<void>(dy), P<void>(wt), P<void>(dx), g.data(), S(s));
    check_launch("conv_dw_dgrad");
  });
  m.def("conv_dw_wgrad", [](int dt, uintptr_t x, uintptr_t dy, uintptr_t slab, int nslice, int out_dt, uintptr_t out,
                            int accum, std::vector<int> g, uintptr_t s) {
    if (g.size() != 14) throw std::runtime_error("conv_dw_wgrad: geometry needs 14 ints");
    conv_dw_wgrad(dt, P<void>(x), P<void>(dy), P<float>(slab), nslice, out_dt, P<void>(out), accum, g.data(), S(s));
    check_launch("conv_dw_wgrad");
  });
  m.def("ssd_loss_blocks", &ssd_loss_blocks);
  m.def("ssd_loss_fwd", [](int dt, uintptr_t cls, uintptr_t loc, uintptr_t ct, uintptr_t lt, uintptr_t lm, int rows,
                           int C1, float lambd, uintptr_t part, uintptr_t out, uintptr_t s) {
    ssd_loss_fwd(dt, P<void>(cls), P<void>(loc), P<float>(ct), P<float>(lt), P<float>(lm), rows, C1, lambd,
                 P<float>(part), P<float>(out), S(s));
    check_launch("ssd_loss_fwd");
  });
  m.def("ssd_loss_bwd", [](int dt, uintptr_t cls, uintptr_t loc, uintptr_t ct, uintptr_t lt, uintptr_t lm,
                           uintptr_t stats, uintptr_t gout, int rows, int C1, float lambd, uintptr_t dcls, uintptr_t dloc,
                           uintptr_t s) {
    ssd_loss_bwd(dt, P<void>(cls), P<void>(loc), P<float>(ct), P<float>(lt), P<float>(lm), P<float>(stats),
                 P<float>(gout), rows, C1, lambd, P<void>(dcls), P<void>(dloc), S(s));
    check_launch("ssd_loss_bwd");
  });
  m.def("multibox_target", [](int dt, uintptr_t anchors, uintptr_t labels, uintptr_t cls_pred, uintptr_t loc_target,
                              uintptr_t loc_mask, uintptr_t cls_target, uintptr_t match_iou, uintptr_t match_gt,
                              uintptr_t key, int B, int A, int L, int W, int C, float thr, float ignore_label,
                              float neg_ratio, float neg_thresh, int min_neg, float v0, float v1, float v2, float v3,
                              uintptr_t s) {
    multibox_target(dt, P<float>(anchors), P<float>(labels), P<void>(cls_pred), P<float>(loc_target),
                    P<float>(loc_mask), P<float>(cls_target), P<float>(match_iou), P<int>(match_gt),
                    P<uint32_t>(key), B, A, L, W, C, thr, ignore_label, neg_ratio, neg_thresh, min_neg, v0, v1, v2,
                    v3, S(s));
    check_launch("multibox_target");
  });
  m.def("bn_nhwc_forward", [](int dt, uintptr_t x, uintptr_t add, uintptr_t y, uintptr_t mask, uintptr_t g, uintptr_t b,
                              uintptr_t center, uintptr_t part, uintptr_t mean, uintptr_t inv, uintptr_t var,
                              uintptr_t scale, uintptr_t shift, int64_t R, int C, float eps, int training, int relu,
                              int fix_gamma, float momentum, uintptr_t mm_upd, uintptr_t mv_upd, int ext_nblk,
                              uintptr_t s, uintptr_t ascale, uintptr_t ashift) {
    bn_nhwc_forward(dt, P<void>(x), P<void>(add), P<void>(y), P<uint8_t>(mask), P<float>(g), P<float>(b), P<float>(center),
                    P<float>(part), P<float>(mean), P<float>(inv), P<float>(var), P<float>(scale), P<float>(shift), R,
                    C, eps, training, relu, fix_gamma, momentum, P<float>(mm_upd), P<float>(mv_upd), ext_nblk, S(s),
                    P<const float>(ascale), P<const float>(ashift));
    check_launch("bn_nhwc_forward");
  }, py::arg("dt"), py::arg("x"), py::arg("add"), py::arg("y"), py::arg("mask"), py::arg("g"), py::arg("b"),
     py::arg("center"), py::arg("part"), py::arg("mean"), py::arg("inv"), py::arg("var"), py::arg("scale"),
     py::arg("shift"), py::arg("R"), py::arg("C"), py::arg("eps"), py::arg("training"), py::arg("relu"),
     py::arg("fix_gamma"), py::arg("momentum"), py::arg("mm_upd"), py::arg("mv_upd"), py::arg("ext_nblk"),
     py::arg("stream"), py::arg("ascale") = 0, py::arg("ashift") = 0);
  m.def("bn_nhwc_backward", [](int dt, uintptr_t x, uintptr_t dy, uintptr_t y, uintptr_t mask, uintptr_t dx,
                               uintptr_t dz,
                               uintptr_t g, uintptr_t mean, uintptr_t inv, uintptr_t fscale, uintptr_t fshift,
                               uintptr_t part, uintptr_t dgamma, uintptr_t dbeta, uintptr_t coef, int64_t R, int C,
                               int relu_mode, int fix_gamma, int training, int accum, uintptr_t s, int ext_nblk,
                               uintptr_t ds_z, uintptr_t ds_mean, uintptr_t ds_part) {
    bn_nhwc_backward(dt, P<void>(x), P<void>(dy), P<void>(y), P<uint8_t>(mask), P<void>(dx), P<void>(dz), P<float>(g), P<float>(mean),
                     P<float>(inv), P<float>(fscale), P<float>(fshift), P<float>(part), P<float>(dgamma),
                     P<float>(dbeta), P<float>(coef), R, C, relu_mode, fix_gamma, training, accum, S(s), ext_nblk,
                     P<const void>(ds_z), P<const float>(ds_mean), P<float>(ds_part));
    check_launch("bn_nhwc_backward");
  }, py::arg("dt"), py::arg("x"), py::arg("dy"), py::arg("y"), py::arg("mask"), py::arg("dx"), py::arg("dz"),
     py::arg("g"), py::arg("mean"), py::arg("inv"), py::arg("fscale"), py::arg("fshift"), py::arg("part"),
     py::arg("dgamma"), py::arg("dbeta"), py::arg("coef"), py::arg("R"), py::arg("C"), py::arg("relu_mode"),
     py::arg("fix_gamma"), py::arg("training"), py::arg("accum"), py::arg("stream"), py::arg("ext_nblk") = 0,
     py::arg("ds_z") = 0, py::arg("ds_mean") = 0, py::arg("ds_part") = 0);
  m.def("softmax_ce_forward", [](int dt, int li, uintptr_t logits, uintptr_t label, uintptr_t loss, uintptr_t lse,
                                 int N, int K, uintptr_t s) {
    softmax_ce_forward(dt, li, P<void>(logits), P<void>(label), P<float>(loss), P<float>(lse), N, K, S(s));
    check_launch("softmax_ce_forward");
  });
  m.def("softmax_ce_backward", [](int dt, int li, uintptr_t logits, uintptr_t label, uintptr_t lse, uintptr_t gout,
                                  uintptr_t dlogits, int N, int K, uintptr_t s) {
    softmax_ce_backward(dt, li, P<void>(logits), P<void>(label), P<float>(lse), P<float>(gout), P<void>(dlogits), N,
                        K, S(s));
    check_launch("softmax_ce_backward");
  });
  m.def("relu_forward", [](int dt, uintptr_t x, uintptr_t y, int64_t n, uintptr_t s) {
    relu_forward(dt, P<void>(x), P<void>(y), n, S(s));
    check_launch("relu_forward");
  });
  m.def("relu_backward", [](int dt, uintptr_t y, uintptr_t dy, uintptr_t dx, int64_t n, uintptr_t s) {
    relu_backward(dt, P<void>(y), P<void>(dy), P<void>(dx), n, S(s));
    check_launch("relu_backward");
  });
  m.def("pointwise_binary", [](int dt, int op, uintptr_t a, uintptr_t b, uintptr_t out, int64_t n, int mode,
                               int64_t row, std::vector<int64_t> shape, std::vector<int64_t> sa,
                               std::vector<int64_t> sb, uintptr_t s) {
    if (shape.size() != sa.size() || shape.size() != sb.size()) throw std::runtime_error("pointwise_binary: rank");
    pointwise_binary(dt, op, P<void>(a), P<void>(b), P<void>(out), n, mode, row, static_cast<int>(shape.size()),
                     shape.data(), sa.data(), sb.data(), S(s));
    check_launch("pointwise_binary");
  });
  m.def("gap_nhwc_forward", [](int dt, uintptr_t x, uintptr_t y, int N, int HW, int C, uintptr_t s) {
    gap_nhwc_forward(dt, P<void>(x), P<void>(y), N, HW, C, S(s));
    check_launch("gap_nhwc_forward");
  });
  m.def("gap_nhwc_backward", [](int dt, uintptr_t dy, uintptr_t dx, int N, int HW, int C, uintptr_t s) {
    gap_nhwc_backward(dt, P<void>(dy), P<void>(dx), N, HW, C, S(s));
    check_launch("gap_nhwc_backward");
  });
  m.def("flat_sgd", [](int dt, uintptr_t w, uintptr_t g, uintptr_t mom, uintptr_t w32, int64_t n, float lr,
                       float wd, float momentum, float rescale, float clip, uintptr_t s) {
    flat_sgd(dt, P<void>(w), P<void>(g), P<float>(mom), P<float>(w32), n, lr, wd, momentum, rescale, clip, nullptr,
             S(s));
    check_launch("flat_sgd");
  });
  m.def("flat_sgd", [](int dt, uintptr_t w, uintptr_t g, uintptr_t mom, uintptr_t w32, int64_t n, float lr,
                       float wd, float momentum, float rescale, float clip, uintptr_t s, uintptr_t hp) {
    flat_sgd(dt, P<void>(w), P<void>(g), P<float>(mom), P<float>(w32), n, lr, wd, momentum, rescale, clip,
             P<float>(hp), S(s));
    check_launch("flat_sgd");
  });
  m.def("conv_nhwc_fwd", [](int dt, uintptr_t x, uintptr_t w, uintptr_t bias, uintptr_t y, int N, int H, int W,
                            int C, int K, int R, int Sf, int sh, int sw, int ph, int pw, int variant, uintptr_t s) {
    conv_nhwc_fwd(dt, P<void>(x), P<void>(w), P<float>(bias), P<void>(y), N, H, W, C, K, R, Sf, sh, sw, ph, pw,
                  variant, S(s));
    check_launch("conv_nhwc_fwd");
  });
  m.def("conv_nhwc_fwd_glds", [](int dt, uintptr_t x, uintptr_t w, uintptr_t bias, uintptr_t y, uintptr_t zero, int N,
                                 int H, int W, int C, int K, int R, int Sf, int sh, int sw, int ph, int pw, int bco,
                                 uintptr_t s, uintptr_t bn_z, uintptr_t bn_mean, uintptr_t bn_scale,
                                 uintptr_t bn_shift, uintptr_t bn_part, int bn_nparts) {
    conv_nhwc_fwd_glds(dt, P<void>(x), P<void>(w), P<float>(bias), P<void>(y), P<void>(zero), N, H, W, C, K, R, Sf,
                       sh, sw, ph, pw, bco, S(s), P<void>(bn_z), P<float>(bn_mean), P<float>(bn_scale),
                       P<float>(bn_shift), P<float>(bn_part), bn_nparts);
    check_launch("conv_nhwc_fwd_glds");
  }, py::arg("dtype"), py::arg("x"), py::arg("w"), py::arg("bias"), py::arg("y"), py::arg("zero"), py::arg("N"),
     py::arg("H"), py::arg("W"), py::arg("C"), py::arg("K"), py::arg("R"), py::arg("S"), py::arg("sh"),
     py::arg("sw"), py::arg("ph"), py::arg("pw"), py::arg("bco"), py::arg("stream"), py::arg("bn_z") = 0,
     py::arg("bn_mean") = 0, py::arg("bn_scale") = 0, py::arg("bn_shift") = 0, py::arg("bn_part") = 0,
     py::arg("bn_nparts") = 0);
  m.def("conv_glds_bwd_nparts", &conv_glds_bwd_nparts);
  m.def("conv_nhwc_dgrad_phases_glds",
        [](int dt, uintptr_t dy, uintptr_t w, uintptr_t dx, uintptr_t zero, int N, int Hi, int Wi, int Cin, int Cout,
           int Ho, int Wo, int stride, std::vector<int> ph, std::vector<int> pw, std::vector<int> R,
           std::vector<int> Sf, std::vector<int> pad_h, std::vector<int> pad_w, std::vector<int64_t> w_off,
           std::vector<int> zph, std::vector<int> zpw, int bco, uintptr_t s, uintptr_t bn_z, uintptr_t bn_mean,
           uintptr_t bn_scale, uintptr_t bn_shift, uintptr_t bn_part, int bn_nparts) {
          const size_t n = ph.size();
          if (pw.size() != n || R.size() != n || Sf.size() != n || pad_h.size() != n || pad_w.size() != n ||
              w_off.size() != n || zph.size() != zpw.size())
            throw std::runtime_error("conv_nhwc_dgrad_phases_glds: per-phase lists differ in length");
          conv_nhwc_dgrad_phases_glds(dt, P<void>(dy), P<void>(w), P<void>(dx), P<void>(zero), N, Hi, Wi, Cin, Cout,
                                      Ho, Wo, stride, (int)n, ph.data(), pw.data(), R.data(), Sf.data(),
                                      pad_h.data(), pad_w.data(), w_off.data(), (int)zph.size(), zph.data(),
                                      zpw.data(), bco, S(s), P<void>(bn_z), P<float>(bn_mean), P<float>(bn_scale),
                                      P<float>(bn_shift), P<float>(bn_part), bn_nparts);
          check_launch("conv_nhwc_dgrad_phases_glds");
        },
        py::arg("dtype"), py::arg("dy"), py::arg("w"), py::arg("dx"), py::arg("zero"), py::arg("N"), py::arg("Hi"),
        py::arg("Wi"), py::arg("Cin"), py::arg("Cout"), py::arg("Ho"), py::arg("Wo"), py::arg("stride"),
        py::arg("ph"), py::arg("pw"), py::arg("R"), py::arg("S"), py::arg("pad_h"), py::arg("pad_w"),
        py::arg("w_off"), py::arg("zph"), py::arg("zpw"), py::arg("bco"), py::arg("stream"), py::arg("bn_z") = 0,
        py::arg("bn_mean") = 0, py::arg("bn_scale") = 0, py::arg("bn_shift") = 0, py::arg("bn_part") = 0,
        py::arg("bn_nparts") = 0);
  m.def("conv_stem_grid", &conv_stem_grid);
  m.def("conv_stem_wgrad_workspace", &conv_stem_wgrad_workspace);
  m.def("conv_stem_fwd", [](int dt, uintptr_t x, uintptr_t w, uintptr_t y, int N, int H, int W, int C, int K, int R,
                            int Sf, int sh, int sw, int ph, int pw, uintptr_t part, int nparts, uintptr_t s) {
    conv_stem_fwd(dt, P<void>(x), P<void>(w), P<void>(y), N, H, W, C, K, R, Sf, sh, sw, ph, pw, P<float>(part),
                  nparts, S(s));
    check_launch("conv_stem_fwd");
  });
  m.def("conv_stem_wgrad", [](int dt, uintptr_t x, uintptr_t dy, uintptr_t slab, int odt, uintptr_t out, int accum,
                              int N, int H, int W, int C, int K, int R, int Sf, int sh, int sw, int ph, int pw,
                              uintptr_t s) {
    conv_stem_wgrad(dt, P<void>(x), P<void>(dy), P<float>(slab), odt, P<void>(out), accum, N, H, W, C, K, R, Sf, sh,
                    sw, ph, pw, S(s));
    check_launch("conv_stem_wgrad");
  });
  m.def("conv_nhwc_fwd_big_nparts", &conv_nhwc_fwd_big_nparts);
  m.def("conv_nhwc_fwd_big_bwd_nparts", &conv_nhwc_fwd_big_bwd_nparts);
  m.def("conv_nhwc_fwd_big", [](int dt, uintptr_t x, uintptr_t w, uintptr_t bias, uintptr_t y, uintptr_t zero, int N,
                                int H, int W, int C, int K, int R, int Sf, int sh, int sw, int ph, int pw, int variant,
                                uintptr_t part, int nparts, uintptr_t addend, uintptr_t s, uintptr_t bz,
                                uintptr_t bmean, uintptr_t bscale, uintptr_t bshift, uintptr_t bmask, int bmode,
                                uintptr_t bpart, int bnparts, int up, int dh, int dw) {
    conv_nhwc_fwd_big(dt, P<void>(x), P<void>(w), P<float>(bias), P<void>(y), P<void>(zero), N, H, W, C, K, R, Sf, sh,
                      sw, ph, pw, variant, P<float>(part), nparts, P<void>(addend), S(s), P<void>(bz), P<float>(bmean),
                      P<float>(bscale), P<float>(bshift), P<uint8_t>(bmask), bmode, P<float>(bpart), bnparts, up, dh,
                      dw);
    check_launch("conv_nhwc_fwd_big");
  }, py::arg("dt"), py::arg("x"), py::arg("w"), py::arg("bias"), py::arg("y"), py::arg("zero"), py::arg("N"),
     py::arg("H"), py::arg("W"), py::arg("C"), py::arg("K"), py::arg("R"), py::arg("S"), py::arg("sh"),
     py::arg("sw"), py::arg("ph"), py::arg("pw"), py::arg("variant"), py::arg("part"), py::arg("nparts"),
     py::arg("addend"), py::arg("stream"), py::arg("bn_z") = 0, py::arg("bn_mean") = 0, py::arg("bn_scale") = 0,
     py::arg("bn_shift") = 0, py::arg("bn_mask") = 0, py::arg("bn_mode") = 0, py::arg("bn_part") = 0,
     py::arg("bn_nparts") = 0, py::arg("up") = 0, py::arg("dh") = 1, py::arg("dw") = 1);
  m.def("conv_nhwc_fwd_ring_nparts", &conv_nhwc_fwd_ring_nparts);
  m.def("conv_nhwc_fwd_ring", [](int dt, uintptr_t x, uintptr_t w, uintptr_t y, uintptr_t zero, int N, int H, int W,
                                 int C, int K, int R, int Sf, int sh, int sw, int ph, int pw, int variant, uintptr_t part,
                                 int nparts, uintptr_t s) {
    conv_nhwc_fwd_ring(dt, P<void>(x), P<void>(w), P<void>(y), P<void>(zero), N, H, W, C, K, R, Sf, sh, sw, ph, pw,
                       variant, P<float>(part), nparts, S(s));
    check_launch("conv_nhwc_fwd_ring");
  });
  m.def("conv3x3_halo_ok", &conv3x3_halo_ok);
  m.def("conv3x3_halo_nparts", &conv3x3_halo_nparts);
  m.def("conv3x3_halo", [](int dt, uintptr_t x, uintptr_t w, uintptr_t y, uintptr_t zero, int N, int H, int W, int C,
                           int K, uintptr_t part, int nparts, uintptr_t bn_z, uintptr_t bn_mean, uintptr_t bn_scale,
                           uintptr_t bn_shift, int bn_mode, uintptr_t bn_part, uintptr_t s) {
    conv3x3_halo(dt, P<void>(x), P<void>(w), P<void>(y), P<void>(zero), N, H, W, C, K, P<float>(part), nparts,
                 P<void>(bn_z), P<float>(bn_mean), P<float>(bn_scale), P<float>(bn_shift), bn_mode, P<float>(bn_part),
                 S(s));
    check_launch("conv3x3_halo");
  }, py::arg("dt"), py::arg("x"), py::arg("w"), py::arg("y"), py::arg("zero"), py::arg("N"), py::arg("H"),
     py::arg("W"), py::arg("C"), py::arg("K"), py::arg("part"), py::arg("nparts"), py::arg("bn_z") = 0,
     py::arg("bn_mean") = 0, py::arg("bn_scale") = 0, py::arg("bn_shift") = 0, py::arg("bn_mode") = 0,
     py::arg("bn_part") = 0, py::arg("s") = 0);
  m.def("conv_nhwc_wgrad_workspace", &conv_nhwc_wgrad_workspace, py::arg("N"), py::arg("H"), py::arg("W"), py::arg("C"),
        py::arg("K"), py::arg("R"), py::arg("S"), py::arg("sh"), py::arg("sw"), py::arg("ph"), py::arg("pw"),
        py::arg("dh") = 1, py::arg("dw") = 1);
  m.def("conv_nhwc_wgrad_ring_ok", &conv_nhwc_wgrad_ring_ok);
  m.def("conv_nhwc_wgrad_ring_workspace", &conv_nhwc_wgrad_ring_workspace, py::arg("N"), py::arg("H"), py::arg("W"),
        py::arg("C"), py::arg("K"), py::arg("R"), py::arg("S"), py::arg("sh"), py::arg("sw"), py::arg("ph"),
        py::arg("pw"), py::arg("variant"), py::arg("dh") = 1, py::arg("dw") = 1);
  m.def("conv_nhwc_wgrad_ring", [](int dt, uintptr_t x, uintptr_t dy, uintptr_t slab, int odt, uintptr_t out,
                                   int accum, int N, int H, int W, int C, int K, int R, int Sf, int sh, int sw, int ph,
                                   int pw, uintptr_t zero, int variant, uintptr_t s, int dh, int dw) {
    conv_nhwc_wgrad_ring(dt, P<void>(x), P<void>(dy), P<float>(slab), odt, P<void>(out), accum, N, H, W, C, K, R, Sf,
                         sh, sw, ph, pw, P<void>(zero), variant, S(s), dh, dw);
    check_launch("conv_nhwc_wgrad_ring");
  }, py::arg("dt"), py::arg("x"), py::arg("dy"), py::arg("slab"), py::arg("odt"), py::arg("out"), py::arg("accum"),
     py::arg("N"), py::arg("H"), py::arg("W"), py::arg("C"), py::arg("K"), py::arg("R"), py::arg("S"), py::arg("sh"),
     py::arg("sw"), py::arg("ph"), py::arg("pw"), py::arg("zero"), py::arg("variant"), py::arg("stream"),
     py::arg("dh") = 1, py::arg("dw") = 1);
  m.def("conv_nhwc_wgrad", [](int dt, uintptr_t x, uintptr_t dy, uintptr_t slab, int odt, uintptr_t out, int accum,
                              int N, int H, int W, int C, int K, int R, int Sf, int sh, int sw, int ph, int pw,
                              uintptr_t zero, uintptr_t s, int dh, int dw) {
    conv_nhwc_wgrad(dt, P<void>(x), P<void>(dy), P<float>(slab), odt, P<void>(out), accum, N, H, W, C, K, R, Sf, sh,
                    sw, ph, pw, P<void>(zero), S(s), dh, dw);
    check_launch("conv_nhwc_wgrad");
  }, py::arg("dt"), py::arg("x"), py::arg("dy"), py::arg("slab"), py::arg("odt"), py::arg("out"), py::arg("accum"),
     py::arg("N"), py::arg("H"), py::arg("W"), py::arg("C"), py::arg("K"), py::arg("R"), py::arg("S"), py::arg("sh"),
     py::arg("sw"), py::arg("ph"), py::arg("pw"), py::arg("zero"), py::arg("stream"), py::arg("dh") = 1,
     py::arg("dw") = 1);
  m.def("layernorm_bwd_partials", &layernorm_bwd_partials);
  m.def("layernorm_forward", [](int dt, uintptr_t x, uintptr_t g, uintptr_t b, uintptr_t y, uintptr_t mean,
                                uintptr_t rstd, int M, int D, float eps, uintptr_t s, int pt) {
    layernorm_forward(dt, P<void>(x), P<void>(g), P<void>(b), pt, P<void>(y), P<float>(mean), P<float>(rstd), M, D,
                      eps, S(s));
    check_launch("layernorm_forward");
  }, py::arg("dtype"), py::arg("x"), py::arg("gamma"), py::arg("beta"), py::arg("y"), py::arg("mean"),
     py::arg("rstd"), py::arg("M"), py::arg("D"), py::arg("eps"), py::arg("stream"), py::arg("pt") = 0);
  m.def("layernorm_backward", [](int dt, uintptr_t x, uintptr_t dy, uintptr_t g, uintptr_t mean, uintptr_t rstd,
                                 uintptr_t dx, uintptr_t part, uintptr_t dg, uintptr_t db, int gdt, int accum, int M,
                                 int D, uintptr_t s, int pt) {
    layernorm_backward(dt, P<void>(x), P<void>(dy), P<void>(g), pt, P<float>(mean), P<float>(rstd), P<void>(dx),
                       P<float>(part), P<void>(dg), P<void>(db), gdt, accum, M, D, S(s));
    check_launch("layernorm_backward");
  }, py::arg("dtype"), py::arg("x"), py::arg("dy"), py::arg("gamma"), py::arg("mean"), py::arg("rstd"),
     py::arg("dx"), py::arg("part"), py::arg("dgamma"), py::arg("dbeta"), py::arg("gdtype"), py::arg("accum"),
     py::arg("M"), py::arg("D"), py::arg("stream"), py::arg("pt") = 0);
  m.def("add_dropout_ln_forward", [](int dt, uintptr_t x, uintptr_t h, uintptr_t g, uintptr_t b, int pt, uintptr_t y,
                                     uintptr_t sum, uintptr_t mask, uintptr_t mean, uintptr_t rstd, int M, int D,
                                     float eps, float p, uint64_t seed, uintptr_t seed_base, uintptr_t s) {
    add_dropout_ln_forward(dt, P<void>(x), P<void>(h), P<void>(g), P<void>(b), pt, P<void>(y), P<void>(sum),
                           P<uint8_t>(mask), P<float>(mean), P<float>(rstd), M, D, eps, p, seed,
                           P<uint64_t>(seed_base), S(s));
    check_launch("add_dropout_ln_forward");
  });
  m.def("add_dropout_ln_backward", [](int dt, uintptr_t sum, uintptr_t dy, uintptr_t g, int pt, uintptr_t mean,
                                      uintptr_t rstd, uintptr_t mask, float p, uintptr_t ds, uintptr_t dh,
                                      uintptr_t part, uintptr_t hpart, uintptr_t dg, uintptr_t db, int gdt, int accum,
                                      int M, int D, uintptr_t s) {
    add_dropout_ln_backward(dt, P<void>(sum), P<void>(dy), P<void>(g), pt, P<float>(mean), P<float>(rstd),
                            P<uint8_t>(mask), p, P<void>(ds), P<void>(dh), P<float>(part), P<float>(hpart),
                            P<void>(dg), P<void>(db), gdt, accum, M, D, S(s));
    check_launch("add_dropout_ln_backward");
  });
  m.def("column_sum_partials", [](int gdt, uintptr_t part, int nb, int ncol, uintptr_t out, int accum, uintptr_t s) {
    column_sum_partials(gdt, P<float>(part), nb, ncol, P<void>(out), accum, S(s));
    check_launch("column_sum_partials");
  });
  m.def("gelu_forward", [](int dt, uintptr_t x, uintptr_t y, int64_t n, uintptr_t s) {
    gelu_forward(dt, P<void>(x), P<void>(y), n, S(s));
    check_launch("gelu_forward");
  });
  m.def("gelu_colpart_blocks", &gelu_colpart_blocks);
  m.def("gelu_backward_colpart", [](int dt, uintptr_t x, uintptr_t dy, uintptr_t dx, uintptr_t part, int M, int N,
                                    uintptr_t s) {
    gelu_backward_colpart(dt, P<void>(x), P<void>(dy), P<void>(dx), P<float>(part), M, N, S(s));
    check_launch("gelu_backward_colpart");
  });
  m.def("gelu_backward", [](int dt, uintptr_t x, uintptr_t dy, uintptr_t dx, int64_t n, uintptr_t s) {
    gelu_backward(dt, P<void>(x), P<void>(dy), P<void>(dx), n, S(s));
    check_launch("gelu_backward");
  });
  m.def("softmax_forward", [](int dt, int log, uintptr_t x, uintptr_t y, int M, int L, float scale, uintptr_t s) {
    softmax_forward(dt, log, P<void>(x), P<void>(y), M, L, scale, S(s));
    check_launch("softmax_forward");
  });
  m.def("softmax_backward", [](int dt, int log, uintptr_t y, uintptr_t dy, uintptr_t dx, int M, int L, float scale,
                               uintptr_t s) {
    softmax_backward(dt, log, P<void>(y), P<void>(dy), P<void>(dx), M, L, scale, S(s));
    check_launch("softmax_backward");
  });
  m.def("dropout_forward", [](int dt, uintptr_t x, uintptr_t y, uintptr_t mask, int64_t n, float p, uint64_t seed,
                              uintptr_t s) {
    dropout_forward(dt, P<void>(x), P<void>(y), P<uint8_t>(mask), n, p, seed, nullptr, S(s));
    check_launch("dropout_forward");
  });
  m.def("dropout_forward", [](int dt, uintptr_t x, uintptr_t y, uintptr_t mask, int64_t n, float p, uint64_t seed,
                              uintptr_t s, uintptr_t seed_base) {
    dropout_forward(dt, P<void>(x), P<void>(y), P<uint8_t>(mask), n, p, seed, P<uint64_t>(seed_base), S(s));
    check_launch("dropout_forward");
  });
  m.def("attention_max_seq", []() { return attention_max_seq(); });
  m.def("attention_forward", [](int dt, uintptr_t qkv, uintptr_t kmask, uintptr_t out, uintptr_t lse, int S, int B,
                                int H, int D, float scale, float p, uint64_t seed, uintptr_t seed_base, uintptr_t s) {
    attention_forward(dt, P<const void>(qkv), P<const float>(kmask), P<void>(out), P<float>(lse), S, B, H, D, scale, p,
                      seed, P<const uint64_t>(seed_base), S_(s));
    check_launch("attention_forward");
  });
  m.def("attention_backward", [](int dt, uintptr_t qkv, uintptr_t kmask, uintptr_t out, uintptr_t dout, uintptr_t lse,
                                 uintptr_t delta, uintptr_t dqkv, int S, int B, int H, int D, float scale, float p,
                                 uint64_t seed, uintptr_t seed_base, uintptr_t s) {
    attention_backward(dt, P<const void>(qkv), P<const float>(kmask), P<const void>(out), P<const void>(dout),
                       P<const float>(lse), P<float>(delta), P<void>(dqkv), S, B, H, D, scale, p, seed,
                       P<const uint64_t>(seed_base), S_(s));
    check_launch("attention_backward");
  });
  m.def("dropout_backward", [](int dt, uintptr_t dy, uintptr_t mask, uintptr_t dx, int64_t n, float p, uintptr_t s) {
    dropout_backward(dt, P<void>(dy), P<uint8_t>(mask), P<void>(dx), n, p, S(s));
    check_launch("dropout_backward");
  });
  m.def("flat_adam", [](int dt, int mode, uintptr_t w, uintptr_t g, uintptr_t mean, uintptr_t var, uintptr_t w32,
                        int64_t n, float lr, float b1, float b2, float eps, float wd, float eta, float rescale,
                        float clip, uintptr_t s) {
    flat_adam(dt, mode, P<void>(w), P<void>(g), P<float>(mean), P<float>(var), P<float>(w32), n, lr, b1, b2, eps, wd,
              eta, rescale, clip, nullptr, S(s));
    check_launch("flat_adam");
  });
  m.def("flat_adam", [](int dt, int mode, uintptr_t w, uintptr_t g, uintptr_t mean, uintptr_t var, uintptr_t w32,
                        int64_t n, float lr, float b1, float b2, float eps, float wd, float eta, float rescale,
                        float clip, uintptr_t s, uintptr_t hp) {
    flat_adam(dt, mode, P<void>(w), P<void>(g), P<float>(mean), P<float>(var), P<float>(w32), n, lr, b1, b2, eps, wd,
              eta, rescale, clip, P<float>(hp), S(s));
    check_launch("flat_adam");
  });
  m.def("lamb_update", [](int dt, uintptr_t w, uintptr_t g, uintptr_t mean, uintptr_t var, uintptr_t w32,
                          uintptr_t upd, uintptr_t chunks, int nchunks, uintptr_t nrm, int nseg, float lr, float b1,
                          float b2, float eps, float bc1, float bc2, float wd, float rescale, float clip, float lb,
                          float ub, uintptr_t s) {
    lamb_update(dt, P<void>(w), P<void>(g), P<float>(mean), P<float>(var), P<float>(w32), P<float>(upd),
                P<void>(chunks), nchunks, P<float>(nrm), nseg, lr, b1, b2, eps, bc1, bc2, wd, rescale, clip, lb, ub,
                nullptr, S(s));
    check_launch("lamb_update");
  });
  m.def("lamb_update", [](int dt, uintptr_t w, uintptr_t g, uintptr_t mean, uintptr_t var, uintptr_t w32,
                          uintptr_t upd, uintptr_t chunks, int nchunks, uintptr_t nrm, int nseg, float lr, float b1,
                          float b2, float eps, float bc1, float bc2, float wd, float rescale, float clip, float lb,
                          float ub, uintptr_t s, uintptr_t hp) {
    lamb_update(dt, P<void>(w), P<void>(g), P<float>(mean), P<float>(var), P<float>(w32), P<float>(upd),
                P<void>(chunks), nchunks, P<float>(nrm), nseg, lr, b1, b2, eps, bc1, bc2, wd, rescale, clip, lb, ub,
                P<float>(hp), S(s));
    check_launch("lamb_update");
  });
  m.def("seg_sumsq", [](int dt, uintptr_t x, uintptr_t chunks, int nchunks, uintptr_t out, int nseg, uintptr_t s) {
    seg_sumsq(dt, P<void>(x), P<void>(chunks), nchunks, P<float>(out), nseg, S(s));
    check_launch("seg_sumsq");
  });
  m.def("all_finite", [](int dt, uintptr_t x, int64_t n, float scale, uintptr_t flag, int init, uintptr_t s) {
    all_finite(dt, P<void>(x), n, scale, P<int>(flag), init, S(s));
    check_launch("all_finite");
  });
  m.def("pool_nhwc_forward", [](int dt, int is_max, uintptr_t x, uintptr_t y, uintptr_t arg, int N, int H, int W,
                                int C, int Ho, int Wo, int kh, int kw, int sh, int sw, int ph, int pw, int cip,
                                uintptr_t s) {
    pool_nhwc_forward(dt, is_max, P<void>(x), P<void>(y), P<uint8_t>(arg), N, H, W, C, Ho, Wo, kh, kw, sh, sw, ph, pw,
                      cip, S(s), nullptr, nullptr);
    check_launch("pool_nhwc_forward");
  });
  m.def("bn_pool_bwd_blocks", &bn_pool_bwd_blocks);
  m.def("bn_pool_backward", [](int dt, uintptr_t x, uintptr_t dy, uintptr_t arg, uintptr_t dx, uintptr_t gamma,
                               uintptr_t mean, uintptr_t invstd, uintptr_t fscale, uintptr_t fshift, uintptr_t part,
                               uintptr_t dgamma, uintptr_t dbeta, uintptr_t coef, int N, int H, int W, int C, int Ho,
                               int Wo, int kh, int kw, int sh, int sw, int ph, int pw, int fix_gamma, int training,
                               int accum, uintptr_t s) {
    bn_pool_backward(dt, P<void>(x), P<void>(dy), P<uint8_t>(arg), P<void>(dx), P<float>(gamma), P<float>(mean),
                     P<float>(invstd), P<float>(fscale), P<float>(fshift), P<float>(part), P<float>(dgamma),
                     P<float>(dbeta), P<float>(coef), N, H, W, C, Ho, Wo, kh, kw, sh, sw, ph, pw, fix_gamma, training,
                     accum, S(s));
    check_launch("bn_pool_backward");
  });
  m.def("pool_nhwc_forward_bnrelu", [](int dt, uintptr_t x, uintptr_t y, uintptr_t arg, int N, int H, int W, int C,
                                       int Ho, int Wo, int kh, int kw, int sh, int sw, int ph, int pw, int cip,
                                       uintptr_t s, uintptr_t scale, uintptr_t shift) {
    pool_nhwc_forward(dt, 1, P<void>(x), P<void>(y), P<uint8_t>(arg), N, H, W, C, Ho, Wo, kh, kw, sh, sw, ph, pw, cip,
                      S(s), P<float>(scale), P<float>(shift));
    check_launch("pool_nhwc_forward_bnrelu");
  });
  m.def("pool_nhwc_backward", [](int dt, int is_max, uintptr_t dy, uintptr_t arg, uintptr_t dx, int N, int H, int W,
                                 int C, int Ho, int Wo, int kh, int kw, int sh, int sw, int ph, int pw, int cip,
                                 uintptr_t s) {
    pool_nhwc_backward(dt, is_max, P<void>(dy), P<uint8_t>(arg), P<void>(dx), N, H, W, C, Ho, Wo, kh, kw, sh, sw, ph,
                       pw, cip, S(s));
    check_launch("pool_nhwc_backward");
  });
}
```

src/kernels/conv_big.hip:

```cpp
#include <stdexcept>
#include <type_traits>

#include "common.h"
#include "mfma.h"

namespace mxamd {

namespace {

typedef _Float16 half8_t __attribute__((ext_vector_type(8)));
typedef __bf16 bf16x8_t __attribute__((ext_vector_type(8)));
typedef float f4_t __attribute__((ext_vector_type(4)));
typedef uint32_t u32x4 __attribute__((ext_vector_type(4)));
typedef __attribute__((address_space(3))) void lds_void;
typedef __attribute__((address_space(1))) void gbl_void;

template <typename T>
struct MfmaB : mfma::Op<T> {};

struct BnBwdFuse {
  const void* z;
  const float* mean;
  const float* scale;
  const float* shift;
  const uint8_t* mask;
  int mode;
  float* part;
  int nparts;
};

struct GeomB {
  int N, H, W, C, K, R, S;
  int Ho, Wo;
  int sh, sw, ph, pw;
  int M;
  int Ktot;
  int up;
  int dh, dw;
};

__device__ __forceinline__ void glds16(const void* src, void* lds_base) {
  __builtin_amdgcn_global_load_lds((gbl_void*)src, (lds_void*)lds_base, 16, 0, 0);
}

__device__ __forceinline__ float row16_sum(float v) {
  v += __shfl_xor(v, 1, 64);
  v += __shfl_xor(v, 2, 64);
  v += __shfl_xor(v, 4, 64);
  v += __shfl_xor(v, 8, 64);
  return v;
}

template <int BCO, int BPIX>
struct BigCfg {
  static constexpr int STAGE = (BCO + BPIX) * 128;
  static constexpr int PITCH = BCO * 2 + 16;
  static constexpr int EPI = BPIX * PITCH;
  static constexpr int SMEM = (2 * STAGE > EPI ? 2 * STAGE : EPI);
};

template <typename T, int WCO, int FJ, int MINB, int MF>
__global__ void __launch_bounds__(512) __attribute__((amdgpu_waves_per_eu(2 * MINB))) conv_fwd_big_kernel(const T* __restrict__ x, const T* __restrict__ w,
                                                           const float* __restrict__ bias, T* __restrict__ y,
                                                           const T* __restrict__ zero, GeomB g, int tiles_co,
                                                           float* __restrict__ part, int nparts,
                                                           const T* __restrict__ addend, BnBwdFuse bf) {
  constexpr int WPIX = 8 / WCO;
  constexpr int BCO = WCO * 64;
  constexpr int BPIX = WPIX * FJ * 16;
  constexpr int BK = 64;
  constexpr int A_BYTES = BCO * 128;
  constexpr int STAGE = BigCfg<BCO, BPIX>::STAGE;
  constexpr int PITCH = BigCfg<BCO, BPIX>::PITCH;
  constexpr int A_INS = BCO / 64;
  constexpr int B_INS = (BPIX + 63) / 64;
  extern __shared__ __attribute__((aligned(1024))) char smem[];

  const int tid = threadIdx.x;
  const int lane = tid & 63;
  const int wid = tid >> 6;

  const int nblk = gridDim.x;
  const int orig = blockIdx.x;
  const int xcd = orig & 7;
  const int q = nblk >> 3, rr = nblk & 7;
  const int wgid = (xcd < rr ? xcd * (q + 1) : rr * (q + 1) + (xcd - rr) * q) + (orig >> 3);
  const int tco = wgid % tiles_co;
  const int tpix = wgid / tiles_co;
  const int co0 = tco * BCO;
  const int pix0 = tpix * BPIX;

  static_assert(MF == 16 || (MF == 32 && FJ % 2 == 0), "conv_big: MFMA shape");
  const int lrow = lane >> 3;
  const int gch = (lane & 7) ^ (MF == 32 ? (((wid & 1) << 2) | (lrow >> 1)) : lrow);

  int a_off[A_INS];
#pragma unroll
  for (int i = 0; i < A_INS; ++i) a_off[i] = (co0 + (i * 8 + wid) * 8 + lrow) * g.Ktot + gch * 8;
  int b_base[B_INS], b_hi[B_INS], b_wi[B_INS];
#pragma unroll
  for (int i = 0; i < B_INS; ++i) {
    const int p = pix0 + (i * 8 + wid) * 8 + lrow;
    if (p < g.M) {
      const int n = p / (g.Ho * g.Wo);
      const int rem = p - n * g.Ho * g.Wo;
      const int ho = rem / g.Wo;
      const int wo = rem - ho * g.Wo;
      b_hi[i] = ho * g.sh - g.ph;
      b_wi[i] = wo * g.sw - g.pw;
      b_base[i] = ((n * g.H + b_hi[i]) * g.W + b_wi[i]) * g.C + gch * 8;
    } else {
      b_hi[i] = -(1 << 20);
      b_wi[i] = 0;
      b_base[i] = 0;
    }
  }
  const T* zsrc = zero + gch * 8;

  const int KT = g.Ktot / BK;
  auto issue = [&](int kt, int stage) {
    const int k0 = kt * BK;
    const int rs = k0 / g.C;
    const int c0 = k0 - rs * g.C;
    const int r = rs / g.S;
    const int s = rs - r * g.S;
    char* sbase = smem + stage * STAGE;
#pragma unroll
    for (int i = 0; i < A_INS; ++i) glds16(w + a_off[i] + k0, sbase + (i * 8 + wid) * 1024);
    const int doff = (r * g.dh * g.W + s * g.dw) * g.C + c0;
#pragma unroll
    for (int i = 0; i < B_INS; ++i) {
      if (BPIX % 64 != 0 && (i * 8 + wid) * 8 >= BPIX) continue;
      const int hi = b_hi[i] + r * g.dh, wi = b_wi[i] + s * g.dw;
      const bool ok = (unsigned)hi < (unsigned)g.H && (unsigned)wi < (unsigned)g.W;
      const T* src = ok ? x + b_base[i] + doff : zsrc;
      glds16(src, sbase + A_BYTES + (i * 8 + wid) * 1024);
    }
  };

  constexpr int NI = MF == 32 ? 2 : 4;
  constexpr int NJ = MF == 32 ? FJ / 2 : FJ;
  typedef typename std::conditional<MF == 32, mfma::f16x, f4_t>::type acc_t;
  acc_t acc[NI][NJ];
#pragma unroll
  for (int i = 0; i < NI; ++i)
#pragma unroll
    for (int j = 0; j < NJ; ++j) acc[i][j] = acc_t{};

  const int wco = wid % WCO;
  const int wpix = wid / WCO;
  const int frag_r = lane & 15;
  const int fchunk = lane >> 4;
  const int a_row0 = (wco * 64 + (MF == 32 ? (lane & 31) : frag_r)) * 128;
  const int b_row0 = A_BYTES + (wpix * FJ * 16 + (MF == 32 ? (lane & 31) : frag_r)) * 128;
  const int sw = MF == 32 ? ((lane & 31) >> 1) & 7 : frag_r & 7;

  issue(0, 0);
  __syncthreads();
  for (int kt = 0; kt < KT; ++kt) {
    const int stage = kt & 1;
    if (kt + 1 < KT) issue(kt + 1, stage ^ 1);
    const char* sb = smem + stage * STAGE;
    if constexpr (MF == 32) {
#pragma unroll
      for (int kk = 0; kk < 4; ++kk) {
        const int ch = ((kk * 2 + (lane >> 5)) ^ sw) * 16;
        u32x4 af[NI], bf[NJ];
#pragma unroll
        for (int i = 0; i < NI; ++i) af[i] = *reinterpret_cast<const u32x4*>(sb + a_row0 + i * 32 * 128 + ch);
#pragma unroll
        for (int j = 0; j < NJ; ++j) bf[j] = *reinterpret_cast<const u32x4*>(sb + b_row0 + j * 32 * 128 + ch);
#pragma unroll
        for (int i = 0; i < NI; ++i)
#pragma unroll
          for (int j = 0; j < NJ; ++j) acc[i][j] = MfmaB<T>::run32(af[i], bf[j], acc[i][j]);
      }
    } else {
#pragma unroll
      for (int kk = 0; kk < 2; ++kk) {
        const int ch = ((kk * 4 + fchunk) ^ sw) * 16;
        u32x4 af[NI], bf[NJ];
#pragma unroll
        for (int i = 0; i < NI; ++i) af[i] = *reinterpret_cast<const u32x4*>(sb + a_row0 + i * 16 * 128 + ch);
#pragma unroll
        for (int j = 0; j < NJ; ++j) bf[j] = *reinterpret_cast<const u32x4*>(sb + b_row0 + j * 16 * 128 + ch);
#pragma unroll
        for (int i = 0; i < NI; ++i)
#pragma unroll
          for (int j = 0; j < NJ; ++j) acc[i][j] = MfmaB<T>::run(af[i], bf[j], acc[i][j]);
      }
    }
    __syncthreads();
  }

  const int pw0 = wpix * FJ * 16;
  auto bias4 = [&](int cl, float* b) {
#pragma unroll
    for (int t = 0; t < 4; ++t) b[t] = bias ? bias[co0 + cl + t] : 0.f;
  };
  auto write_part = [&](int cl, const float* s, const float* q) {
    const int pid = tpix * WPIX + wpix;
    const int64_t c = co0 + cl;
    float* p1 = part;
    float* p2 = part + static_cast<int64_t>(g.K) * nparts;
#pragma unroll
    for (int t = 0; t < 4; ++t) {
      p1[(c + t) * nparts + pid] = s[t];
      p2[(c + t) * nparts + pid] = q[t];
    }
  };
  if constexpr (MF == 32) {
#pragma unroll
    for (int i = 0; i < NI; ++i) {
#pragma unroll
      for (int gq = 0; gq < 4; ++gq) {
        const int cl = wco * 64 + i * 32 + gq * 8 + (lane >> 5) * 4;
        float b[4], s4[4] = {0.f, 0.f, 0.f, 0.f}, q4[4] = {0.f, 0.f, 0.f, 0.f};
        bias4(cl, b);
#pragma unroll
        for (int j = 0; j < NJ; ++j) {
          const int pl = pw0 + j * 32 + (lane & 31);
          float v[4];
#pragma unroll
          for (int t = 0; t < 4; ++t) v[t] = acc[i][j][gq * 4 + t] + b[t];
          *reinterpret_cast<uint2*>(smem + pl * PITCH + cl * 2) = MfmaB<T>::pack4(v[0], v[1], v[2], v[3]);
          if (part != nullptr && pix0 + pl < g.M) {
#pragma unroll
            for (int t = 0; t < 4; ++t) {
              s4[t] += v[t];
              q4[t] += v[t] * v[t];
            }
          }
        }
        if (part != nullptr) {
#pragma unroll
          for (int t = 0; t < 4; ++t) {
            s4[t] = row16_sum(s4[t]);
            s4[t] += __shfl_xor(s4[t], 16, 64);
            q4[t] = row16_sum(q4[t]);
            q4[t] += __shfl_xor(q4[t], 16, 64);
          }
          if ((lane & 31) == 0) write_part(cl, s4, q4);
        }
      }
    }
  } else {
    const int co_l = (lane >> 4) * 4;
#pragma unroll
    for (int i = 0; i < NI; ++i) {
      const int cl = wco * 64 + i * 16 + co_l;
      float b[4], s4[4] = {0.f, 0.f, 0.f, 0.f}, q4[4] = {0.f, 0.f, 0.f, 0.f};
      bias4(cl, b);
#pragma unroll
      for (int j = 0; j < NJ; ++j) {
        const int pl = pw0 + j * 16 + frag_r;
        float v[4];
#pragma unroll
        for (int t = 0; t < 4; ++t) v[t] = acc[i][j][t] + b[t];
        *reinterpret_cast<uint2*>(smem + pl * PITCH + cl * 2) = MfmaB<T>::pack4(v[0], v[1], v[2], v[3]);
        if (part != nullptr && pix0 + pl < g.M) {
#pragma unroll
          for (int t = 0; t < 4; ++t) {
            s4[t] += v[t];
            q4[t] += v[t] * v[t];
          }
        }
      }
      if (part != nullptr) {
#pragma unroll
        for (int t = 0; t < 4; ++t) {
          s4[t] = row16_sum(s4[t]);
          q4[t] = row16_sum(q4[t]);
        }
        if (frag_r == 0) write_part(cl, s4, q4);
      }
    }
  }
  __syncthreads();
  constexpr int CPR = BCO / 8;
  constexpr int TOTAL = BPIX * CPR;
  constexpr int ITERS = TOTAL / 512;
  static_assert(512 % CPR == 0 && TOTAL % 512 == 0, "each thread keeps one 8-channel group");
  const bool bnb = bf.part != nullptr;
  float s1[8], s2[8], bm[8], bsc[8], bsh[8];
#pragma unroll
  for (int t = 0; t < 8; ++t) {
    s1[t] = 0.f;
    s2[t] = 0.f;
  }
  if (bnb) {
    const int cb = co0 + (tid % CPR) * 8;
#pragma unroll
    for (int t = 0; t < 8; ++t) {
      bm[t] = bf.mean[cb + t];
      bsc[t] = bf.mode == 2 ? bf.scale[cb + t] : 0.f;
      bsh[t] = bf.mode == 2 ? bf.shift[cb + t] : 0.f;
    }
  }
  constexpr int DMAX = MINB > 1 ? 4 : 8;
  constexpr int D = ITERS < DMAX ? ITERS : DMAX;
  const T* zsrc_b = static_cast<const T*>(bf.z);
  uint4 ad_ring[D], z_ring[D];
  auto out_pix = [&](int p) -> int64_t {
    if (g.up != 2) return p;
    const int n = p / (g.Ho * g.Wo);
    const int rem = p - n * g.Ho * g.Wo;
    const int ho = rem / g.Wo;
    const int wo = rem - ho * g.Wo;
    return ((int64_t)n * 2 * g.Ho + 2 * ho) * (2 * g.Wo) + 2 * wo;
  };
  auto row_off = [&](int it, int64_t* off) -> bool {
    const int e = tid + it * 512;
    const int pl = e / CPR;
    const int c8 = e - pl * CPR;
    const int p = pix0 + pl;
    *off = out_pix(p < g.M ? p : 0) * g.K + co0 + c8 * 8;
    return p < g.M;
  };
#pragma unroll
  for (int it = 0; it < D; ++it) {
    int64_t off;
    const bool ok = row_off(it, &off);
    if (addend != nullptr && ok) ad_ring[it] = *reinterpret_cast<const uint4*>(addend + off);
    if (bnb && ok) z_ring[it] = *reinterpret_cast<const uint4*>(zsrc_b + off);
  }
#pragma unroll
  for (int it = 0; it < ITERS; ++it) {
    const int e = tid + it * 512;
    const int pl = e / CPR;
    const int c8 = e - pl * CPR;
    const int p = pix0 + pl;
    int64_t off;
    const bool ok = row_off(it, &off);
    uint4 ad_cur = ad_ring[it % D], z_cur = z_ring[it % D];
    if (it + D < ITERS) {
      int64_t off2;
      const bool ok2 = row_off(it + D, &off2);
      if (addend != nullptr && ok2) ad_ring[it % D] = *reinterpret_cast<const uint4*>(addend + off2);
      if (bnb && ok2) z_ring[it % D] = *reinterpret_cast<const uint4*>(zsrc_b + off2);
    }
    if (ok) {
      Vec8<T> v;
      v.raw = *reinterpret_cast<const uint4*>(smem + pl * PITCH + c8 * 16);
      if (addend != nullptr) {
        Vec8<T> a;
        a.raw = ad_cur;
#pragma unroll
        for (int t = 0; t < 8; ++t) v.set(t, v.get(t) + a.get(t));
      }
      v.store(y + off);
      if (g.up == 2) {
        const uint4 z4 = {0u, 0u, 0u, 0u};
        const int64_t rowp = (int64_t)2 * g.Wo * g.K;
        *reinterpret_cast<uint4*>(y + off + g.K) = z4;
        *reinterpret_cast<uint4*>(y + off + rowp) = z4;
        *reinterpret_cast<uint4*>(y + off + rowp + g.K) = z4;
      }
      if (bnb) {
        Vec8<T> zv;
        zv.raw = z_cur;
        const uint32_t mb = bf.mode == 3 ? bf.mask[off >> 3] : 0xffu;
#pragma unroll
        for (int t = 0; t < 8; ++t) {
          const float zt = zv.get(t);
          bool keep = true;
          if (bf.mode == 2) keep = fmaf(zt, bsc[t], bsh[t]) > 0.f;
          if (bf.mode == 3) keep = (mb >> t) & 1u;
          const float dz = keep ? v.get(t) : 0.f;
          s1[t] += dz;
          s2[t] += dz * (zt - bm[t]);
        }
      }
    }
    (void)p;
  }
  if (bnb) {
    constexpr int ROWS = 512 / CPR;
    float* red = reinterpret_cast<float*>(smem);
    __syncthreads();
#pragma unroll
    for (int t = 0; t < 8; ++t) {
      red[(tid / CPR) * BCO + (tid % CPR) * 8 + t] = s1[t];
      red[ROWS * BCO + (tid / CPR) * BCO + (tid % CPR) * 8 + t] = s2[t];
    }
    __syncthreads();
    for (int q = tid; q < 2 * BCO; q += 512) {
      const int which = q / BCO, ch = q - which * BCO;
      const float* col = red + which * ROWS * BCO + ch;
      float acc_s = 0.f;
#pragma unroll 8
      for (int r = 0; r < ROWS; ++r) acc_s += col[r * BCO];
      bf.part[(int64_t)which * g.K * bf.nparts + (int64_t)(co0 + ch) * bf.nparts + tpix] = acc_s;
    }
  }
}

template <typename T, int WCO, int FJ, int MINB, int MF = 16>
void launch_big(const void* x, const void* w, const float* bias, void* y, const void* zero, const GeomB& g,
                float* part, int nparts, const void* addend, const BnBwdFuse& bf, hipStream_t s) {
  constexpr int BCO = WCO * 64;
  constexpr int BPIX = (8 / WCO) * FJ * 16;
  constexpr int SMEM = BigCfg<BCO, BPIX>::SMEM;
  static_assert(SMEM <= 160 * 1024, "conv_big: LDS budget");
  static bool attr_set = false;
  if (!attr_set) {
    hipFuncSetAttribute(reinterpret_cast<const void*>(&conv_fwd_big_kernel<T, WCO, FJ, MINB, MF>),
                        hipFuncAttributeMaxDynamicSharedMemorySize, SMEM);
    attr_set = true;
  }
  const int tiles_co = g.K / BCO;
  const int tiles_pix = (g.M + BPIX - 1) / BPIX;
  constexpr int ONE_STAGE = BigCfg<BCO, BPIX>::STAGE > BigCfg<BCO, BPIX>::EPI ? BigCfg<BCO, BPIX>::STAGE
                                                                               : BigCfg<BCO, BPIX>::EPI;
  const int smem = g.Ktot / 64 > 1 ? SMEM : ONE_STAGE;
  hipLaunchKernelGGL((conv_fwd_big_kernel<T, WCO, FJ, MINB, MF>), dim3(tiles_co * tiles_pix), dim3(512), smem, s,
                     static_cast<const T*>(x), static_cast<const T*>(w), bias, static_cast<T*>(y),
                     static_cast<const T*>(zero), g, tiles_co, part, nparts, static_cast<const T*>(addend), bf);
}

static void big_tile(int variant, int* bco, int* bpix) {
  if (variant == 16) { *bco = 256; *bpix = 224; return; }
  if (variant == 17) { *bco = 128; *bpix = 448; return; }
  if (variant == 4) variant = 1;
  if (variant == 5) variant = 3;
  if (variant >= 6 && variant <= 9) variant -= 6;
  switch (variant) {
    case 0: *bco = 256; *bpix = 256; break;
    case 1: *bco = 128; *bpix = 256; break;
    case 2: *bco = 64; *bpix = 512; break;
    case 3: *bco = 256; *bpix = 128; break;
    default: throw std::runtime_error("conv_nhwc_fwd_big: unknown variant");
  }
}

template <typename T>
void dispatch_big(int variant, const void* x, const void* w, const float* bias, void* y, const void* zero,
                  const GeomB& g, float* part, int nparts, const void* addend, const BnBwdFuse& bf, hipStream_t s) {
  switch (variant) {
    case 0: launch_big<T, 4, 8, 1>(x, w, bias, y, zero, g, part, nparts, addend, bf, s); break;
    case 1: launch_big<T, 2, 4, 1>(x, w, bias, y, zero, g, part, nparts, addend, bf, s); break;
    case 2: launch_big<T, 1, 4, 1>(x, w, bias, y, zero, g, part, nparts, addend, bf, s); break;
    case 3: launch_big<T, 4, 4, 1>(x, w, bias, y, zero, g, part, nparts, addend, bf, s); break;
    case 4: launch_big<T, 2, 4, 2>(x, w, bias, y, zero, g, part, nparts, addend, bf, s); break;
    case 5: launch_big<T, 4, 4, 2>(x, w, bias, y, zero, g, part, nparts, addend, bf, s); break;
    case 6: launch_big<T, 4, 8, 1, 32>(x, w, bias, y, zero, g, part, nparts, addend, bf, s); break;
    case 7: launch_big<T, 2, 4, 1, 32>(x, w, bias, y, zero, g, part, nparts, addend, bf, s); break;
    case 8: launch_big<T, 1, 4, 1, 32>(x, w, bias, y, zero, g, part, nparts, addend, bf, s); break;
    case 9: launch_big<T, 4, 4, 1, 32>(x, w, bias, y, zero, g, part, nparts, addend, bf, s); break;
    case 16: launch_big<T, 4, 7, 1>(x, w, bias, y, zero, g, part, nparts, addend, bf, s); break;
    case 17: launch_big<T, 2, 7, 1>(x, w, bias, y, zero, g, part, nparts, addend, bf, s); break;
    default: throw std::runtime_error("conv_nhwc_fwd_big: unknown variant");
  }
}

}

int conv_nhwc_fwd_big_nparts(int N, int H, int W, int R, int S, int sh, int sw, int ph, int pw, int variant) {
  int bco, bpix;
  big_tile(variant, &bco, &bpix);
  const int Ho = (H + 2 * ph - R) / sh + 1;
  const int Wo = (W + 2 * pw - S) / sw + 1;
  const int M = N * Ho * Wo;
  return ((M + bpix - 1) / bpix) * (8 / (bco / 64));
}

int conv_nhwc_fwd_big_bwd_nparts(int N, int H, int W, int R, int S, int sh, int sw, int ph, int pw, int variant) {
  int bco, bpix;
  big_tile(variant, &bco, &bpix);
  const int Ho = (H + 2 * ph - R) / sh + 1;
  const int Wo = (W + 2 * pw - S) / sw + 1;
  return (N * Ho * Wo + bpix - 1) / bpix;
}

void conv_nhwc_fwd_big(int dtype, const void* x, const void* w, const float* bias, void* y, const void* zero, int N,
                       int H, int W, int C, int K, int R, int S, int sh, int sw, int ph, int pw, int variant,
                       float* part, int nparts, const void* addend, hipStream_t s, const void* bn_z,
                       const float* bn_mean, const float* bn_scale, const float* bn_shift, const uint8_t* bn_mask,
                       int bn_mode, float* bn_part, int bn_nparts, int up, int dh, int dw) {
  GeomB g;
  g.N = N; g.H = H; g.W = W; g.C = C; g.K = K; g.R = R; g.S = S;
  g.sh = sh; g.sw = sw; g.ph = ph; g.pw = pw;
  g.dh = dh; g.dw = dw;
  MXAMD_HOST_CHECK(dh >= 1 && dw >= 1, "conv_nhwc_fwd_big: dilation must be >= 1");
  MXAMD_HOST_CHECK((dh == 1 && dw == 1) || (part == nullptr && bn_part == nullptr && up == 0),
                   "conv_nhwc_fwd_big: dilated convolutions take no fused BN epilogue / upsampled output");
  g.Ho = (H + 2 * ph - dh * (R - 1) - 1) / sh + 1;
  g.Wo = (W + 2 * pw - dw * (S - 1) - 1) / sw + 1;
  MXAMD_HOST_CHECK(g.Ho > 0 && g.Wo > 0, "conv_nhwc_fwd_big: empty output");
  g.M = N * g.Ho * g.Wo;
  g.Ktot = R * S * C;
  g.up = up;
  int bco, bpix;
  big_tile(variant, &bco, &bpix);
  MXAMD_HOST_CHECK(C % 64 == 0 && K % bco == 0, "conv_nhwc_fwd_big: need Cin % 64 == 0 and Cout % BCO == 0");
  MXAMD_HOST_CHECK(up == 0 || (up == 2 && addend == nullptr && (int64_t)g.M * 4 * K < (1ll << 31)),
                   "conv_nhwc_fwd_big: the 2x upsampled output takes no addend and must fit 32-bit indexing");
  MXAMD_HOST_CHECK((int64_t)N * H * W * C < (1ll << 31) && (int64_t)g.M * K < (1ll << 31) &&
                       (int64_t)K * g.Ktot < (1ll << 31),
                   "conv_nhwc_fwd_big: tensor too large for 32-bit indexing");
  MXAMD_HOST_CHECK(part == nullptr || nparts == conv_nhwc_fwd_big_nparts(N, H, W, R, S, sh, sw, ph, pw, variant),
                   "conv_nhwc_fwd_big: wrong BN partials count");
  BnBwdFuse bf{bn_z, bn_mean, bn_scale, bn_shift, bn_mask, bn_mode, bn_part, bn_nparts};
  MXAMD_HOST_CHECK(bn_part == nullptr ||
                       (bn_z && bn_mean && bn_nparts == conv_nhwc_fwd_big_bwd_nparts(N, H, W, R, S, sh, sw, ph, pw,
                                                                                     variant) &&
                        (bn_mode != 2 || (bn_scale && bn_shift)) && (bn_mode != 3 || bn_mask)),
                   "conv_nhwc_fwd_big: bad BN-backward epilogue arguments");
  if (dtype == kF16) dispatch_big<__half>(variant, x, w, bias, y, zero, g, part, nparts, addend, bf, s);
  else if (dtype == kBF16) dispatch_big<__hip_bfloat16>(variant, x, w, bias, y, zero, g, part, nparts, addend, bf, s);
  else throw std::runtime_error("conv_nhwc_fwd_big: dtype must be f16 or bf16");
}

}
```

src/kernels/conv_pw.hip:

```cpp
#include <stdexcept>

#include "common.h"
#include "mfma.h"

namespace mxamd {

namespace {

typedef _Float16 half8_t __attribute__((ext_vector_type(8)));
typedef __bf16 bf16x8_t __attribute__((ext_vector_type(8)));
typedef float f4_t __attribute__((ext_vector_type(4)));
typedef uint32_t u32x4 __attribute__((ext_vector_type(4)));
typedef __attribute__((address_space(3))) void lds_void;
typedef __attribute__((address_space(1))) void gbl_void;

template <typename T>
struct PwM : mfma::Op<T> {
  template <typename V>
  static __device__ __forceinline__ f4_t mma(const V& a, const V& b, f4_t c) {
    return mfma::Op<T>::run(a, b, c);
  }
};

template <int N>
__device__ __forceinline__ void vm_wait() {
  static_assert(N >= 0 && N < 64, "vmcnt range");
  __builtin_amdgcn_s_waitcnt((N & 15) | (7 << 4) | (15 << 8) | ((N >> 4) << 14));
}

__device__ __forceinline__ void lds_barrier() { asm volatile("s_waitcnt lgkmcnt(0)\n\ts_barrier" ::: "memory"); }

__device__ __forceinline__ uint32_t lds_byte(const char* p) {
  const uintptr_t a = reinterpret_cast<uintptr_t>(p);
  return (*reinterpret_cast<const uint32_t*>(a & ~static_cast<uintptr_t>(3)) >> ((a & 3u) * 8)) & 0xffu;
}

constexpr int pw_bm(int kin, int nout, bool add) {
  const int in_rows = (8192 / kin) > 16 ? (8192 / kin) : 16;
  const int bm0 = (16384 / nout) < in_rows ? (16384 / nout) : in_rows;
  if (!add) return bm0;
  const int wp = 8 / ((nout / 16) < 8 ? (nout / 16) : 8);
  int bm = bm0 < 32 ? bm0 : 32;
  if (bm > 8192 / nout) bm = 8192 / nout;
  if (bm < 16 * wp) bm = 16 * wp;
  return bm;
}

constexpr int kPwBnbNone = 0;
constexpr int kPwBnbPlain = 1;
constexpr int kPwBnbFromZ = 2;
constexpr int kPwBnbMask = 3;

struct PwBnb {
  const void* z;
  const uint8_t* mask;
  const float* mean;
  const float* scale;
  const float* shift;
  const uint8_t* amask;
};

template <int KIN, int NOUT, int WPC = 2, bool ADD = false, int BNB = kPwBnbNone, bool AMK = false>
struct PwCfg {
  static constexpr bool EXT = ADD || BNB != kPwBnbNone;
  static constexpr int BM = pw_bm(KIN, NOUT, EXT);
  static constexpr int WC = NOUT / 16 < 8 ? NOUT / 16 : 8;
  static constexpr int WP = 8 / WC;
  static constexpr int FC = NOUT / WC / 16;
  static constexpr int FP = BM / WP / 16;
  static constexpr int KS = KIN / 32;
  static constexpr int ROWB = KIN * 2;
  static constexpr int STAGE_IN = BM * ROWB;
  static constexpr int STAGE_ADD = ADD ? BM * NOUT * 2 : 0;
  static constexpr int STAGE_Z = BNB ? BM * NOUT * 2 : 0;
  static constexpr int STAGE_M = BNB == kPwBnbMask ? (BM * NOUT / 8 + 1023) / 1024 * 1024 : 0;
  static constexpr int STAGE_AM = AMK ? (BM * NOUT / 8 + 1023) / 1024 * 1024 : 0;
  static constexpr int STAGE = STAGE_IN + STAGE_ADD + STAGE_Z + STAGE_M + STAGE_AM;
  static constexpr int LPT = STAGE_IN / (512 * 16);
  static constexpr int APT = STAGE_ADD / (512 * 16);
  static constexpr int TI = STAGE_IN / 1024;
  static constexpr int TA = STAGE_ADD / 1024;
  static constexpr int TZ = STAGE_Z / 1024;
  static constexpr int TM = STAGE_M / 1024;
  static constexpr int TAM = STAGE_AM / 1024;
  static constexpr int PITCH = NOUT * 2 + 16;
  static constexpr int EPI = BM * PITCH;
  static constexpr int OCH = NOUT / 8;
  static constexpr int SPT = (BM * OCH + 511) / 512;
  static constexpr int LDS = WPC == 1 ? 156 * 1024 : 80 * 1024;
  static constexpr int NMAX = EXT ? 6 : 4;
  static constexpr int NST = (NMAX * STAGE + EPI <= LDS) ? NMAX
                           : ((NMAX - 1) * STAGE + EPI <= LDS) ? NMAX - 1
                           : ((NMAX - 2) * STAGE + EPI <= LDS) ? NMAX - 2 : 2;
  static constexpr int D = NST - 1;
  static constexpr int SMEM = NST * STAGE + EPI;
  static_assert(FC >= 1 && FP >= 1, "at least one fragment pair per wave");
  static_assert(EXT || (LPT >= 1 && STAGE_IN % (512 * 16) == 0), "whole LDS-DMA instructions per tile");
  static_assert(!EXT || (STAGE_IN % 1024 == 0 && STAGE_ADD % 1024 == 0 && STAGE_Z % 1024 == 0),
                "whole 1 KB LDS-DMA instructions");
  static_assert(!EXT || WPC == 1, "the extra stages need the LDS of a whole CU");
  static_assert(BNB != kPwBnbMask || (NOUT / 8) % 16 == 0, "mask rows of whole 16-byte chunks");
  static_assert((BM * OCH) % 512 == 0 || BM * OCH < 512, "whole store rounds, or a single partial one");
  static_assert(512 % OCH == 0, "a thread keeps one output chunk");
  static_assert(D * ((TI + 7) / 8 + (TA + 7) / 8 + (TZ + 7) / 8 + (TM + 7) / 8 + (TAM + 7) / 8 + SPT) <
                    (EXT ? 40 : 64),
                "vmcnt range (vm_wait_n covers < 40)");
  static_assert(!AMK || (ADD && (NOUT / 8) % 16 == 0), "the addend mask rides with an addend, whole 16-byte rows");
  static_assert(FC * KS * 4 <= (WPC == 1 ? 128 : 64), "resident weights exceed the register budget");
  static_assert(ROWB % 128 == 0, "rows of whole 128-byte swizzle groups");
};

__device__ __forceinline__ void vm_wait_n(int n) {
  switch (n) {
#define MXAMD_VMW(K) \
  case K:            \
    vm_wait<K>();    \
    break;
    MXAMD_VMW(0) MXAMD_VMW(1) MXAMD_VMW(2) MXAMD_VMW(3) MXAMD_VMW(4) MXAMD_VMW(5) MXAMD_VMW(6) MXAMD_VMW(7)
    MXAMD_VMW(8) MXAMD_VMW(9) MXAMD_VMW(10) MXAMD_VMW(11) MXAMD_VMW(12) MXAMD_VMW(13) MXAMD_VMW(14) MXAMD_VMW(15)
    MXAMD_VMW(16) MXAMD_VMW(17) MXAMD_VMW(18) MXAMD_VMW(19) MXAMD_VMW(20) MXAMD_VMW(21) MXAMD_VMW(22)
    MXAMD_VMW(23) MXAMD_VMW(24) MXAMD_VMW(25) MXAMD_VMW(26) MXAMD_VMW(27) MXAMD_VMW(28) MXAMD_VMW(29)
    MXAMD_VMW(30) MXAMD_VMW(31) MXAMD_VMW(32) MXAMD_VMW(33) MXAMD_VMW(34) MXAMD_VMW(35) MXAMD_VMW(36)
    MXAMD_VMW(37) MXAMD_VMW(38) MXAMD_VMW(39)
#undef MXAMD_VMW
    default:
      vm_wait<39>();
  }
}

__device__ __forceinline__ void vm_wait_le(int n) {
  if (n >= 48) vm_wait<48>();
  else if (n >= 32) vm_wait<32>();
  else if (n >= 24) vm_wait<24>();
  else if (n >= 16) vm_wait<16>();
  else if (n >= 12) vm_wait<12>();
  else if (n >= 8) vm_wait<8>();
  else if (n >= 6) vm_wait<6>();
  else if (n >= 4) vm_wait<4>();
  else if (n >= 3) vm_wait<3>();
  else if (n >= 2) vm_wait<2>();
  else if (n >= 1) vm_wait<1>();
  else vm_wait<0>();
}

template <typename T, int KIN, int NOUT, bool STATS, bool ADD, int WPC, int S, int BNB, bool AMK = false>
__global__ void __launch_bounds__(512) __attribute__((amdgpu_waves_per_eu(2 * WPC))) conv_pw_stream_kernel(
    const T* __restrict__ x, const T* __restrict__ w, T* __restrict__ y, const T* __restrict__ zero, int M, int ntiles,
    float* __restrict__ part, const T* __restrict__ addend, int wt, PwBnb bnb) {
  using C = PwCfg<KIN, NOUT, WPC, ADD, BNB, AMK>;
  constexpr bool EXT = C::EXT;
  extern __shared__ __attribute__((aligned(1024))) char smem[];
  const int tid = threadIdx.x;
  const int lane = tid & 63;
  const int wid = tid >> 6;
  const int wc = wid % C::WC, wp = wid / C::WC;
  const int grid = gridDim.x;
  const int xcd = blockIdx.x & 7;
  const int q8 = grid >> 3, r8 = grid & 7;
  const int wg0 = (xcd < r8 ? xcd * (q8 + 1) : r8 * (q8 + 1) + (xcd - r8) * q8) + (blockIdx.x >> 3);
  constexpr int NT = NOUT * S;
  const int slice = S > 1 ? wg0 % S : 0;
  const int wg = S > 1 ? wg0 / S : wg0;
  const int gs = grid / S;

  u32x4 wa[C::FC][C::KS];
  if (!wt) {
#pragma unroll
    for (int f = 0; f < C::FC; ++f)
#pragma unroll
      for (int s = 0; s < C::KS; ++s) {
        const int co = slice * NOUT + wc * C::FC * 16 + f * 16 + (lane & 15);
        wa[f][s] = *reinterpret_cast<const u32x4*>(w + static_cast<int64_t>(co) * KIN + s * 32 + (lane >> 4) * 8);
      }
  } else {
#pragma unroll
    for (int f = 0; f < C::FC; ++f)
#pragma unroll
      for (int s = 0; s < C::KS; ++s) {
        const int k = s * 32 + (lane >> 1);
        const int co = slice * NOUT + wc * C::FC * 16 + f * 16 + (lane & 1) * 8;
        wa[f][s] = *reinterpret_cast<const u32x4*>(w + static_cast<int64_t>(k) * NT + co);
      }
  }

  vm_wait<0>();
  if (wt) {
    uint16_t* scr = reinterpret_cast<uint16_t*>(smem + wid * 1280);
#pragma unroll
    for (int f = 0; f < C::FC; ++f)
#pragma unroll
      for (int s = 0; s < C::KS; ++s) {
        const uint4 v = __builtin_bit_cast(uint4, wa[f][s]);
        const uint32_t wv[4] = {v.x, v.y, v.z, v.w};
#pragma unroll
        for (int q = 0; q < 8; ++q)
          scr[((lane & 1) * 8 + q) * 40 + (lane >> 1)] = static_cast<uint16_t>(wv[q >> 1] >> ((q & 1) * 16));
        asm volatile("s_waitcnt lgkmcnt(0)" ::: "memory");
        wa[f][s] = *reinterpret_cast<const u32x4*>(scr + (lane & 15) * 40 + (lane >> 4) * 8);
        asm volatile("s_waitcnt lgkmcnt(0)" ::: "memory");
      }
    __syncthreads();
  }
#pragma unroll
  for (int f = 0; f < C::FC; ++f)
#pragma unroll
    for (int s = 0; s < C::KS; ++s) asm volatile("" ::"v"(wa[f][s]));

  auto issue = [&](int t, int st) {
    char* sb = smem + st * C::STAGE;
    constexpr int NI = EXT ? (C::TI + 7) / 8 : C::LPT;
#pragma unroll
    for (int j = 0; j < NI; ++j) {
      const int i = j * 8 + wid;
      if (EXT && i >= C::TI) break;
      const int byte = (i * 64 + lane) * 16;
      const int row = byte / C::ROWB;
      const int slot = (byte % C::ROWB) / 16;
      const int chunk = slot ^ (row & 7);
      const int p = t * C::BM + row;
      const T* src = p < M ? x + static_cast<int64_t>(p) * KIN + chunk * 8 : zero + (chunk & 7) * 8;
      __builtin_amdgcn_global_load_lds((gbl_void*)src, (lds_void*)(sb + i * 1024), 16, 0, 0);
    }
#pragma unroll
    for (int j = 0; j < (C::TA + 7) / 8; ++j) {
      const int i = j * 8 + wid;
      if (i >= C::TA) break;
      const int byte = (i * 64 + lane) * 16;
      const int row = byte / (NOUT * 2);
      const int p = t * C::BM + row;
      const T* src = p < M ? addend + static_cast<int64_t>(p) * NT + slice * NOUT + (byte % (NOUT * 2)) / 2 : zero;
      __builtin_amdgcn_global_load_lds((gbl_void*)src, (lds_void*)(sb + C::STAGE_IN + i * 1024), 16, 0, 0);
    }
#pragma unroll
    for (int j = 0; j < (C::TZ + 7) / 8; ++j) {
      const int i = j * 8 + wid;
      if (i >= C::TZ) break;
      const int byte = (i * 64 + lane) * 16;
      const int row = byte / (NOUT * 2);
      const int p = t * C::BM + row;
      const T* src = p < M ? static_cast<const T*>(bnb.z) + static_cast<int64_t>(p) * NT + slice * NOUT +
                                 (byte % (NOUT * 2)) / 2
                           : zero;
      __builtin_amdgcn_global_load_lds((gbl_void*)src, (lds_void*)(sb + C::STAGE_IN + C::STAGE_ADD + i * 1024), 16, 0,
                                       0);
    }
#pragma unroll
    for (int j = 0; j < (C::TM + 7) / 8; ++j) {
      const int i = j * 8 + wid;
      if (i >= C::TM) break;
      const int byte = (i * 64 + lane) * 16;
      const int row = byte / (NOUT / 8);
      const int p = t * C::BM + row;
      const void* src = (row < C::BM && p < M)
                            ? static_cast<const void*>(bnb.mask + (static_cast<int64_t>(p) * NT + slice * NOUT) / 8 +
                                                       byte % (NOUT / 8))
                            : static_cast<const void*>(zero);
      __builtin_amdgcn_global_load_lds((gbl_void*)src,
                                       (lds_void*)(sb + C::STAGE_IN + C::STAGE_ADD + C::STAGE_Z + i * 1024), 16, 0, 0);
    }
#pragma unroll
    for (int j = 0; j < (C::TAM + 7) / 8; ++j) {
      const int i = j * 8 + wid;
      if (i >= C::TAM) break;
      const int byte = (i * 64 + lane) * 16;
      const int row = byte / (NOUT / 8);
      const int p = t * C::BM + row;
      const void* src = (row < C::BM && p < M)
                            ? static_cast<const void*>(bnb.amask + (static_cast<int64_t>(p) * NT + slice * NOUT) / 8 +
                                                       byte % (NOUT / 8))
                            : static_cast<const void*>(zero);
      __builtin_amdgcn_global_load_lds(
          (gbl_void*)src, (lds_void*)(sb + C::STAGE_IN + C::STAGE_ADD + C::STAGE_Z + C::STAGE_M + i * 1024), 16, 0, 0);
    }
  };
  const int ops_per_tile = EXT ? (C::TI - wid + 7) / 8 + (C::TA - wid + 7) / 8 + (C::TZ - wid + 7) / 8 +
                                      (C::TM - wid + 7) / 8 + (C::TAM - wid + 7) / 8
                                : C::LPT;

  const int my_tiles = wg < ntiles ? (ntiles - wg + gs - 1) / gs : 0;
  for (int j = 0; j < C::D && j < my_tiles; ++j) issue(wg + j * gs, j);

  float s1[8], s2[8];
#pragma unroll
  for (int e = 0; e < 8; ++e) {
    s1[e] = 0.f;
    s2[e] = 0.f;
  }
  const int my_c8 = tid % C::OCH;
  char* epi = smem + C::NST * C::STAGE;
  float bmean[8], bsc[8], bsh[8];
#pragma unroll
  for (int q = 0; q < 8; ++q) {
    const int ch = slice * NOUT + my_c8 * 8 + q;
    bmean[q] = BNB ? bnb.mean[ch] : 0.f;
    bsc[q] = BNB == kPwBnbFromZ ? bnb.scale[ch] : 0.f;
    bsh[q] = BNB == kPwBnbFromZ ? bnb.shift[ch] : 0.f;
  }

  for (int it = 0; it < my_tiles; ++it) {
    const int t = wg + it * gs;
    const int st = it % C::NST;
    if (!EXT) {
      if (it + C::D < my_tiles) issue(wg + (it + C::D) * gs, (it + C::D) % C::NST);
      const int later = (my_tiles - 1 - it) < C::D ? (my_tiles - 1 - it) : C::D;
      const int epis = it < C::D ? it : C::D;
      if (later == C::D && epis == C::D) vm_wait<C::D*(C::LPT + C::SPT)>();
      else vm_wait_le(later * C::LPT + epis * C::SPT);
      lds_barrier();
    } else {
      const int later = (my_tiles - 1 - it) < C::D - 1 ? (my_tiles - 1 - it) : C::D - 1;
      const int epis = it < C::D ? it : C::D;
      vm_wait_n(later * ops_per_tile + epis * C::SPT);
      lds_barrier();
      if (it + C::D < my_tiles) issue(wg + (it + C::D) * gs, (it + C::D) % C::NST);
    }

    const char* sb = smem + st * C::STAGE;
    f4_t acc[C::FC][C::FP];
#pragma unroll
    for (int f = 0; f < C::FC; ++f)
#pragma unroll
      for (int p = 0; p < C::FP; ++p) acc[f][p] = f4_t{0.f, 0.f, 0.f, 0.f};
#pragma unroll
    for (int s = 0; s < C::KS; ++s) {
      u32x4 bf[C::FP];
#pragma unroll
      for (int p = 0; p < C::FP; ++p) {
        const int row = wp * C::FP * 16 + p * 16 + (lane & 15);
        const int chunk = s * 4 + (lane >> 4);
        bf[p] = *reinterpret_cast<const u32x4*>(sb + row * C::ROWB + ((chunk ^ (row & 7)) * 16));
      }
#pragma unroll
      for (int f = 0; f < C::FC; ++f)
#pragma unroll
        for (int p = 0; p < C::FP; ++p) acc[f][p] = PwM<T>::mma(wa[f][s], bf[p], acc[f][p]);
    }
#pragma unroll
    for (int f = 0; f < C::FC; ++f)
#pragma unroll
      for (int p = 0; p < C::FP; ++p) {
        const int pix = wp * C::FP * 16 + p * 16 + (lane & 15);
        const int co = wc * C::FC * 16 + f * 16 + (lane >> 4) * 4;
        const f4_t v = acc[f][p];
        *reinterpret_cast<uint2*>(epi + pix * C::PITCH + co * 2) = PwM<T>::pack4(v[0], v[1], v[2], v[3]);
      }
    lds_barrier();
    const __amdgpu_buffer_rsrc_t yrs = __builtin_amdgcn_make_buffer_rsrc(
        y, 0, static_cast<int>(static_cast<uint32_t>(M) * NT * sizeof(T)), 0x00020000);
#pragma unroll
    for (int k = 0; k < C::SPT; ++k) {
      const int e = tid + k * 512;
      const bool in_tile = e < C::BM * C::OCH;
      const int pix = in_tile ? e / C::OCH : 0;
      const int c8 = e % C::OCH;
      const int p = t * C::BM + pix;
      Vec8<T> v;
      v.raw = *reinterpret_cast<const uint4*>(epi + pix * C::PITCH + c8 * 16);
      if (ADD) {
        Vec8<T> a;
        a.raw = *reinterpret_cast<const uint4*>(sb + C::STAGE_IN + pix * (NOUT * 2) + c8 * 16);
        if (AMK) {
          const uint32_t amb = lds_byte(sb + C::STAGE_IN + C::STAGE_ADD + C::STAGE_Z + C::STAGE_M + pix * (NOUT / 8) + c8);
          auto m2 = [&](int j) -> uint32_t {
            const uint32_t b = (amb >> (2 * j)) & 3u;
            return (b & 1u) * 0xFFFFu | (b >> 1) * 0xFFFF0000u;
          };
          a.raw.x &= m2(0);
          a.raw.y &= m2(1);
          a.raw.z &= m2(2);
          a.raw.w &= m2(3);
        }
#pragma unroll
        for (int q = 0; q < 8; ++q) v.set(q, v.get(q) + a.get(q));
      }
      const bool live = in_tile && p < M;
      if (BNB && live) {
        Vec8<T> zv;
        zv.raw = *reinterpret_cast<const uint4*>(sb + C::STAGE_IN + C::STAGE_ADD + pix * (NOUT * 2) + c8 * 16);
        const uint32_t mb =
            BNB == kPwBnbMask ? lds_byte(sb + C::STAGE_IN + C::STAGE_ADD + C::STAGE_Z + pix * (NOUT / 8) + c8)
                              : 0xffu;
#pragma unroll
        for (int q = 0; q < 8; ++q) {
          const float zq = zv.get(q);
          bool keep = true;
          if (BNB == kPwBnbFromZ) keep = fmaf(zq, bsc[q], bsh[q]) > 0.f;
          if (BNB == kPwBnbMask) keep = (mb >> q) & 1u;
          const float dz = keep ? v.get(q) : 0.f;
          s1[q] += dz;
          s2[q] += dz * (zq - bmean[q]);
        }
      }
      const uint32_t off = live ? (static_cast<uint32_t>(p) * NT + slice * NOUT + c8 * 8) * sizeof(T) : 0xFFFFFFF0u;
      __builtin_amdgcn_raw_buffer_store_b128(__builtin_bit_cast(u32x4, v.raw), yrs, off, 0, 0);
      if (STATS && live) {
#pragma unroll
        for (int q = 0; q < 8; ++q) {
          const float z = v.get(q);
          s1[q] += z;
          s2[q] += z * z;
        }
      }
    }
    (void)my_c8;
  }
  if (STATS || BNB) {
    vm_wait<0>();
    lds_barrier();
    float* red = reinterpret_cast<float*>(smem);
    constexpr int ROWS = 512 / C::OCH;
#pragma unroll
    for (int q = 0; q < 8; ++q) {
      red[(tid / C::OCH) * NOUT + my_c8 * 8 + q] = s1[q];
      red[ROWS * NOUT + (tid / C::OCH) * NOUT + my_c8 * 8 + q] = s2[q];
    }
    lds_barrier();
    for (int qq = tid; qq < 2 * NOUT; qq += 512) {
      const int which = qq / NOUT, ch = qq - which * NOUT;
      const float* col = red + which * ROWS * NOUT + ch;
      float a = 0.f;
      for (int r = 0; r < ROWS; ++r) a += col[r * NOUT];
      part[static_cast<int64_t>(which) * NT * gs + static_cast<int64_t>(slice * NOUT + ch) * gs + wg] = a;
    }
  }
}

template <typename T, int KIN, int NOUT, int WPC, int S, bool STATS, bool ADD, int BNB = kPwBnbNone, bool AMK = false>
void launch_pw_v(const void* x, const void* w, void* y, const void* zero, int M, float* part, const void* addend,
                 int grid, hipStream_t s, int wt, const PwBnb& bnb = PwBnb{}) {
  using C = PwCfg<KIN, NOUT, WPC, ADD, BNB, AMK>;
  static_assert(C::SMEM <= C::LDS && C::NST >= 2, "LDS budget / ring depth");
  static bool set = false;
  if (!set) {
    hipFuncSetAttribute(
        reinterpret_cast<const void*>(&conv_pw_stream_kernel<T, KIN, NOUT, STATS, ADD, WPC, S, BNB, AMK>),
        hipFuncAttributeMaxDynamicSharedMemorySize, C::SMEM);
    set = true;
  }
  const int ntiles = (M + C::BM - 1) / C::BM;
  hipLaunchKernelGGL((conv_pw_stream_kernel<T, KIN, NOUT, STATS, ADD, WPC, S, BNB, AMK>), dim3(grid), dim3(512), C::SMEM,
                     s, static_cast<const T*>(x), static_cast<const T*>(w), static_cast<T*>(y),
                     static_cast<const T*>(zero), M, ntiles, part, static_cast<const T*>(addend), wt, bnb);
}

template <int KIN, int NOUT>
constexpr bool pw_bnb_built(bool add, int mode) {
  return add ? (mode == kPwBnbMask && (NOUT / 8) % 16 == 0) : mode == kPwBnbFromZ;
}

template <typename T, int KIN, int NOUT, int S>
bool launch_pw_bnb(const void* x, const void* w, void* y, const void* zero, int M, float* part, const void* addend,
                   int grid, hipStream_t s, int wt, const PwBnb& bnb, int mode) {
  if constexpr ((NOUT / 8) % 16 == 0) {
    if (addend && mode == kPwBnbMask) {
      if (bnb.amask)
        launch_pw_v<T, KIN, NOUT, 1, S, false, true, kPwBnbMask, true>(x, w, y, zero, M, part, addend, grid, s, wt,
                                                                        bnb);
      else
        launch_pw_v<T, KIN, NOUT, 1, S, false, true, kPwBnbMask>(x, w, y, zero, M, part, addend, grid, s, wt, bnb);
      return true;
    }
  }
  if (!addend && mode == kPwBnbFromZ) {
    launch_pw_v<T, KIN, NOUT, 1, S, false, false, kPwBnbFromZ>(x, w, y, zero, M, part, addend, grid, s, wt, bnb);
    return true;
  }
  return false;
}

template <typename T, int KIN, int NOUT, int WPC, int S>
void launch_pw(const void* x, const void* w, void* y, const void* zero, int M, float* part, const void* addend,
               int grid, hipStream_t s, int wt, const PwBnb* bnb, int mode) {
  if (bnb) {
    MXAMD_HOST_CHECK((launch_pw_bnb<T, KIN, NOUT, S>(x, w, y, zero, M, part, addend, grid, s, wt, *bnb, mode)),
                     "conv_pw_stream: BN-backward variant not built");
    return;
  }
  using C = PwCfg<KIN, NOUT, WPC>;
  using CA = PwCfg<KIN, NOUT, 1, true>;
  static_assert(C::SMEM <= C::LDS && CA::SMEM <= CA::LDS, "workgroups per CU");
  static_assert(C::NST >= 2 && CA::NST >= 2, "ring depth");
  if (part) {
    if (addend) launch_pw_v<T, KIN, NOUT, 1, S, true, true>(x, w, y, zero, M, part, addend, grid, s, wt);
    else launch_pw_v<T, KIN, NOUT, WPC, S, true, false>(x, w, y, zero, M, part, addend, grid, s, wt);
  } else {
    if (addend) launch_pw_v<T, KIN, NOUT, 1, S, false, true>(x, w, y, zero, M, part, addend, grid, s, wt);
    else launch_pw_v<T, KIN, NOUT, WPC, S, false, false>(x, w, y, zero, M, part, addend, grid, s, wt);
  }
}

#define MXAMD_PW_SHAPES(X)                                                                                  \
  X(64, 64, 2, 1) X(64, 128, 2, 1) X(64, 256, 2, 1) X(128, 128, 2, 1) X(128, 256, 2, 1) X(256, 64, 2, 1)     \
  X(256, 128, 2, 1) X(512, 128, 2, 1) X(128, 512, 1, 1) X(256, 512, 1, 1) X(512, 256, 1, 1) X(256, 512, 1, 2) \
  X(1024, 128, 1, 2) X(512, 256, 1, 8)

template <typename T>
bool dispatch_pw(int kin, int nout, const void* x, const void* w, void* y, const void* zero, int M, float* part,
                 const void* addend, int grid, hipStream_t s, int wt, const PwBnb* bnb, int mode) {
#define MXAMD_PW_CASE(K, N, W, SL)                                        \
  if (kin == K && nout == N * SL) {                                       \
    launch_pw<T, K, N, W, SL>(x, w, y, zero, M, part, addend, grid, s, wt, bnb, mode); \
    return true;                                                          \
  }
  MXAMD_PW_SHAPES(MXAMD_PW_CASE)
#undef MXAMD_PW_CASE
  return false;
}

}

int conv_pw_stream_ok(int kin, int nout) {
#define MXAMD_PW_OK(K, N, W, SL) \
  if (kin == K && nout == N * SL) return W;
  MXAMD_PW_SHAPES(MXAMD_PW_OK)
#undef MXAMD_PW_OK
  return 0;
}

int conv_pw_stream_slices(int kin, int nout) {
#define MXAMD_PW_SL(K, N, W, SL) \
  if (kin == K && nout == N * SL) return SL;
  MXAMD_PW_SHAPES(MXAMD_PW_SL)
#undef MXAMD_PW_SL
  return 0;
}

int conv_pw_stream_bnb_ok(int kin, int nout, int add, int mode) {
#define MXAMD_PW_BOK(K, N, W, SL) \
  if (kin == K && nout == N * SL) return pw_bnb_built<K, N>(add != 0, mode) ? 1 : 0;
  MXAMD_PW_SHAPES(MXAMD_PW_BOK)
#undef MXAMD_PW_BOK
  return 0;
}

int conv_pw_stream_grid(int M, int kin, int nout, int ncu, int add) {
  const int sl = conv_pw_stream_slices(kin, nout);
  if (sl == 0) return 0;
  const int bm = pw_bm(kin, nout / sl, add != 0);
  const int ntiles = (M + bm - 1) / bm;
  const int wpc = add ? 1 : conv_pw_stream_ok(kin, nout);
  int per = (wpc * ncu + sl - 1) / sl;
  if (per > ntiles) per = ntiles;
  return per * sl;
}

void conv_pw_stream(int dtype, const void* x, const void* w, void* y, const void* zero, int M, int kin, int nout,
                    float* part, int grid, hipStream_t s, const void* addend, int wt, const void* bn_z,
                    const uint8_t* bn_mask, const float* bn_mean, const float* bn_scale, const float* bn_shift,
                    int bn_mode, const uint8_t* addend_mask) {
  MXAMD_HOST_CHECK(conv_pw_stream_ok(kin, nout), "conv_pw_stream: unsupported (Cin, Cout)");
  MXAMD_HOST_CHECK(grid >= 1 && grid % conv_pw_stream_slices(kin, nout) == 0 &&
                   (int64_t)M * nout * 2 < (1ll << 31) - 64 && (int64_t)M * kin < (1ll << 31),
                   "conv_pw_stream: tensor too large for 32-bit offsets");
  PwBnb bnb{bn_z, bn_mask, bn_mean, bn_scale, bn_shift, addend_mask};
  MXAMD_HOST_CHECK(addend_mask == nullptr || (addend && bn_z && bn_mode == kPwBnbMask),
                   "conv_pw_stream: the addend mask is built for the tee data gradient with the tail's BN statistics");
  const PwBnb* pb = nullptr;
  if (bn_z) {
    MXAMD_HOST_CHECK(part && bn_mean && conv_pw_stream_bnb_ok(kin, nout, addend != nullptr, bn_mode) &&
                         (bn_mode != kPwBnbFromZ || (bn_scale && bn_shift)) && (bn_mode != kPwBnbMask || bn_mask),
                     "conv_pw_stream: BN-backward statistics need partials, mean, a built mode and its mask source");
    pb = &bnb;
  }
  bool ok = false;
  if (dtype == kF16) ok = dispatch_pw<__half>(kin, nout, x, w, y, zero, M, part, addend, grid, s, wt, pb, bn_mode);
  else if (dtype == kBF16)
    ok = dispatch_pw<__hip_bfloat16>(kin, nout, x, w, y, zero, M, part, addend, grid, s, wt, pb, bn_mode);
  MXAMD_HOST_CHECK(ok, "conv_pw_stream: dtype must be f16 or bf16");
}

}
```

Baseline: 12580 images/sec.

## Keep strided shortcut dgrad compact and fuse its upsampled add into tee dgrad

The stride-2 1x1 shortcut's data gradient is now computed at half resolution and passed lazily to the tee conv backward as a placeholder. The tee dgrad kernels (pointwise stream and big-tile conv) can read that compact addend with on-the-fly 2x upsampling, which zero-fills odd positions. This avoids materialising and then re-reading a full-resolution, mostly-zero gradient tensor and a separate add. It adds new kernel template paths, a token hand-off between autograd functions, and fallbacks that densify when the chosen algorithm cannot take a compact addend.

```diff
diff --git a/mxnet_maintenance_amd/ops/kernel_fns.py b/mxnet_maintenance_amd/ops/kernel_fns.py
--- a/mxnet_maintenance_amd/ops/kernel_fns.py
+++ b/mxnet_maintenance_amd/ops/kernel_fns.py
@@ -640,7 +640,8 @@
     return conv_fwd(dy.contiguous(), wt, (1, 1), (0, 0), None, variant, bn_bwd=bn_bwd, up=2)
 
 
-def conv_fwd(x, w, stride, pad, bias=None, variant=0, bn_stats=False, addend=None, bn_bwd=None, up=0, dil=(1, 1)):
+def conv_fwd(x, w, stride, pad, bias=None, variant=0, bn_stats=False, addend=None, bn_bwd=None, up=0, dil=(1, 1),
+             addend_up=0):
     N, H, W, C = x.shape
     K, R, S, _ = w.shape
     dil = tuple(dil)
@@ -653,8 +654,11 @@
     if N * Ho * Wo * K >= 2 ** 31:
         raise ValueError('conv_fwd: output too large for 32-bit indexing')
     b = _f32(bias) if bias is not None else None
+    assert addend_up in (0, 2) and (addend_up == 0 or (addend is not None and up == 0))
     if addend is not None:
-        assert variant in _BIG_VARIANTS and addend.shape == y.shape and addend.dtype == y.dtype
+        ashape = tuple(y.shape) if not addend_up else (N, Ho // 2, Wo // 2, K)
+        assert variant in _BIG_VARIANTS and tuple(addend.shape) == ashape and addend.dtype == y.dtype
+        assert not addend_up or (Ho % 2 == 0 and Wo % 2 == 0), 'conv_fwd: a half-resolution addend needs even Ho, Wo'
         addend = addend.contiguous()
     if variant in _RING_VARIANTS:
         assert bias is None and addend is None, 'conv ring kernel: no bias / addend'
@@ -688,7 +692,7 @@
         lib.conv_nhwc_fwd_big(_DT[x.dtype], x.data_ptr(), w.data_ptr(), _p(b), y.data_ptr(),
                               _zero_page(x.device).data_ptr(), N, H, W, C, K, R, S, stride[0], stride[1],
                               pad[0], pad[1], v, _p(part), nparts, _p(addend), _stream(), up=int(up), dh=dil[0],
-                              dw=dil[1], **bkw)
+                              dw=dil[1], aup=int(addend_up), **bkw)
         if bkw:
             y._mxamd_bn_bwd = (bpart, bnp, bn_bwd[6], y._version)
         if part is not None:
@@ -1148,7 +1152,7 @@
             and bool(_K.lib().conv_pw_stream_bnb_ok(int(kin), int(nout), int(bool(add)), int(bn_src[5]))))
 
 
-def conv_pw(x, w2, bn_stats=False, addend=None, bn_bwd=None, addend_mask=None):
+def conv_pw(x, w2, bn_stats=False, addend=None, bn_bwd=None, addend_mask=None, addend_up=0):
     C = x.shape[-1]
     K = w2.shape[0]
     M = x.numel() // C
@@ -1157,20 +1161,28 @@
     if not wt:
         w2 = w2.contiguous()
     y = torch.empty(x.shape[:-1] + (K,), dtype=x.dtype, device=x.device)
+    if addend_up not in (0, 2) or (addend_up and (addend is None or bn_stats or addend_mask is not None)):
+        raise ValueError('conv_pw: addend_up=2 takes a plain addend without forward statistics')
     if addend is not None:
         addend = addend.contiguous()
-        if tuple(addend.shape) != tuple(y.shape) or addend.dtype != y.dtype or addend.data_ptr() % 16:
+        ashape = tuple(y.shape)
+        if addend_up:
+            if y.dim() != 4 or y.shape[1] % 2 or y.shape[2] % 2:
+                raise ValueError('conv_pw: a half-resolution addend needs an [N, H, W, C] output of even H and W')
+            ashape = (y.shape[0], y.shape[1] // 2, y.shape[2] // 2, K)
+            bkw_up = dict(addend_up=2, H=int(y.shape[1]), W=int(y.shape[2]))
+        if tuple(addend.shape) != ashape or addend.dtype != y.dtype or addend.data_ptr() % 16:
             raise ValueError('conv_pw: addend must match the output (shape, dtype, 16-byte alignment)')
     lib = _K.lib()
     grid = lib.conv_pw_stream_grid(M, C, K, _num_cus(x.device), int(addend is not None or bn_bwd is not None))
     nparts = grid // max(1, lib.conv_pw_stream_slices(C, K))
     part = torch.empty(2 * K * nparts, dtype=torch.float32, device=x.device) if (bn_stats or bn_bwd) else None
-    bkw = {}
+    bkw = dict(bkw_up) if addend_up else {}
     if bn_bwd is not None:
         assert not bn_stats, 'conv_pw: forward and backward statistics are exclusive'
         z, bmean, bscale, bshift, bmask, bmode, _token = bn_bwd
         assert z.shape == y.shape and z.dtype == y.dtype and z.is_contiguous() and z.data_ptr() % 16 == 0
-        bkw = dict(bn_z=z.data_ptr(), bn_mask=_p(bmask), bn_mean=bmean.data_ptr(), bn_scale=_p(bscale),
+        bkw.update(bn_z=z.data_ptr(), bn_mask=_p(bmask), bn_mean=bmean.data_ptr(), bn_scale=_p(bscale),
                    bn_shift=_p(bshift), bn_mode=int(bmode))
     if addend_mask is not None:
         assert bn_bwd is not None and addend is not None and addend_mask.dtype == torch.uint8
@@ -1501,6 +1513,7 @@
         ctx.b_ref = bias
         ctx.w_ref = w
         ctx.bn_src = getattr(x, '_mxamd_bn_src', None)
+        ctx.tee_token = getattr(x, '_mxamd_tee_token', None) if tuple(stride) == (2, 2) else None
         return y
 
     @staticmethod
@@ -1513,7 +1526,9 @@
             dw = _wgrad_maybe_side(dy, x, w, ctx.w_ref, stride, pad)
         if ctx.needs_input_grad[0]:
             key = ('dgrad', tuple(x.shape), tuple(w.shape), tuple(stride), tuple(pad), x.dtype)
-            if _bn_bwd_fusable(ctx.bn_src, x.shape):
+            if compact_shortcut_ok(ctx.tee_token, dy, x, w, stride, pad):
+                dx = _compact_shortcut_dgrad(ctx.tee_token, dy, x, w)
+            elif _bn_bwd_fusable(ctx.bn_src, x.shape):
                 cands, timing = _dgrad_bn_candidates(dy, x, w, stride, pad, ctx.bn_src)
                 dx = _select(key + ('bnbwd',), cands, _dgrad_default(w, stride), timing=timing)
             else:
@@ -1544,6 +1559,7 @@
         ctx.bn_src = getattr(x, '_mxamd_bn_src', None)
         xp = x.view_as(x)
         xp._mxamd_tee_key = _tee_key(x, w, ctx.bn_src)
+        ctx.tee_token = xp._mxamd_tee_token = _TeeToken(xp._mxamd_tee_key)
         return y, xp
 
     @staticmethod
@@ -1551,13 +1567,14 @@
         x, w = ctx.saved_tensors
         K, C = w.shape[0], w.shape[3]
         dx = dw = None
+        compact, ctx.tee_token.compact = ctx.tee_token.compact, None
         if gy is None:
-            return gpass, None, None
+            return _densify_compact(gpass, compact, x.shape)[0], None, None
         gy = gy.contiguous()
         if ctx.needs_input_grad[1] and _WGRAD_SIDE[0]:
             dw = _wgrad_maybe_side(gy, x, w, ctx.w_ref, (1, 1), (0, 0))
         if ctx.needs_input_grad[0]:
-            dx = _tee_dgrad(gy, x, w, gpass, ctx.inplace_grad, ctx.bn_src)
+            dx = _tee_dgrad(gy, x, w, gpass, ctx.inplace_grad, ctx.bn_src, compact)
         if ctx.needs_input_grad[1] and not _WGRAD_SIDE[0]:
             dw = _wgrad(gy, x, w, ctx.w_ref, (1, 1), (0, 0))
         return dx, dw, None
@@ -1588,10 +1605,96 @@
     return gpass * bits.view(gpass.shape).to(gpass.dtype)
 
 
-def _tee_dgrad(gy, x, w, gpass, inplace, bn_src=None):
+_COMPACT_DX = [os.environ.get('MXAMD_COMPACT_SHORTCUT_GRAD', '1') != '0']
+_COMPACT_USED = [0]
+_ZERO_ELEM = {}
+
+
+class _TeeToken:
+    __slots__ = ('key', 'compact')
+
+    def __init__(self, key):
+        self.key = key
+        self.compact = None
+
+
+def _chosen_algo(key):
+    key = _akey(key)
+    name = _ALGO.get(key)
+    if name is None:
+        _load_tuning_file()
+        name = _FILE_ALGO.get(repr(key))
+    return name
+
+
+def _takes_compact(name):
+    base = (name or '').split('+')[0]
+    return base == 'pw' or (base.startswith('hip') and base[3:].isdigit() and int(base[3:]) in _BIG_VARIANTS)
+
+
+def compact_shortcut_ok(token, dy, x, w, stride, pad):
+    return (_COMPACT_DX[0] and token is not None and token.compact is None
+            and conv_up2_ok(dy, w, stride, pad, x.shape) and x.numel() < 2 ** 31
+            and _takes_compact(_chosen_algo(token.key)))
+
+
+def _compact_shortcut_dgrad(token, dy, x, w):
+    xs = x[:, ::2, ::2]
+    key = ('dgrad', tuple(xs.shape), tuple(w.shape), (1, 1), (0, 0), x.dtype)
+    dc = _select(key, _dgrad_candidates(dy, xs, w, (1, 1), (0, 0)), _dgrad_default(w, (1, 1)))
+    z = _ZERO_ELEM.get((x.dtype, x.device))
+    if z is None:
+        z = _ZERO_ELEM[(x.dtype, x.device)] = torch.zeros(1, dtype=x.dtype, device=x.device)
+    ph = z.expand(x.shape)
+    token.compact = (dc.contiguous(), ph, ph._version)
+    return ph
+
+
+def _densify_compact(gpass, compact, shape):
+    if compact is None:
+        return gpass, False
+    dc, ph, ver = compact
+    dense = torch.zeros(shape, dtype=dc.dtype, device=dc.device)
+    dense[:, ::2, ::2] = dc
+    if gpass is None or (gpass is ph and ph._version == ver):
+        return dense, True
+    return dense.add_(gpass), True
+
+
+def _tee_dgrad_compact(gy, x, w, dc, bn_src):
+    K, C = w.shape[0], w.shape[3]
+    fuse_bn = _bn_bwd_fusable(bn_src, x.shape)
+    name = _chosen_algo(_tee_key(x, w, bn_src))
+    if not _takes_compact(name) or x.dim() != 4 or x.shape[1] % 2 or x.shape[2] % 2:
+        return None
+    base, _, bn = name.partition('+')
+    if bn and not (bn == 'bn' and fuse_bn):
+        return None
+    bnb = bn_src if bn else None
+    if base == 'pw':
+        if not (pw_ok(gy, K, C) and dc.data_ptr() % 16 == 0 and (bnb is None or pw_bnb_ok(K, C, True, bn_src))):
+            return None
+        return conv_pw(gy, w.reshape(K, C).t(), addend=dc, bn_bwd=bnb, addend_up=2)
+    v = int(base[3:])
+    if not (_CONV_HIP and K % 64 == 0 and gy.dtype in (torch.float16, torch.bfloat16) and gy.numel() < 2 ** 31
+            and C % _BIG_VARIANTS[v][0] == 0 and (v not in _BIG_SKINNY or (_SKINNY_ON and K == 64))):
+        return None
+    return conv_fwd(gy, _dgrad_weight(w.contiguous()), (1, 1), (0, 0), None, v, addend=dc, bn_bwd=bnb, addend_up=2)
+
+
+def _tee_dgrad(gy, x, w, gpass, inplace, bn_src=None, compact=None):
     K, C = w.shape[0], w.shape[3]
     g2 = gy.reshape(-1, K)
     w2 = w.reshape(K, C)
+    if compact is not None:
+        dc, ph, ver = compact
+        r = None
+        if gpass is ph and ph._version == ver and _COMPACT_DX[0]:
+            r = _tee_dgrad_compact(gy, x, w, dc, bn_src)
+        if r is not None:
+            _COMPACT_USED[0] += 1
+            return r
+        gpass, inplace = _densify_compact(gpass, compact, x.shape)
     amask = _unpack_lazy_dz(gpass)
     if amask is not None:
         key = _tee_key(x, w, bn_src)
diff --git a/src/kernels/bindings.cc b/src/kernels/bindings.cc
--- a/src/kernels/bindings.cc
+++ b/src/kernels/bindings.cc
@@ -60,7 +60,7 @@
                        int H, int W, int C, int K, int R, int S, int sh, int sw, int ph, int pw, int variant,
                        float* part, int nparts, const void* addend, hipStream_t s, const void* bn_z,
                        const float* bn_mean, const float* bn_scale, const float* bn_shift, const uint8_t* bn_mask,
-                       int bn_mode, float* bn_part, int bn_nparts, int up, int dh, int dw);
+                       int bn_mode, float* bn_part, int bn_nparts, int up, int dh, int dw, int aup);
 int conv_nhwc_fwd_big_bwd_nparts(int N, int H, int W, int R, int S, int sh, int sw, int ph, int pw, int variant);
 void conv_nhwc_fwd_glds(int dtype, const void* x, const void* w, const float* bias, void* y, const void* zero, int N,
                         int H, int W, int C, int K, int R, int S, int sh, int sw, int ph, int pw, int bco,
@@ -190,7 +190,7 @@
 void conv_pw_stream(int dtype, const void* x, const void* w, void* y, const void* zero, int M, int kin, int nout,
                     float* part, int grid, hipStream_t s, const void* addend, int wt, const void* bn_z,
                     const uint8_t* bn_mask, const float* bn_mean, const float* bn_scale, const float* bn_shift,
-                    int bn_mode, const uint8_t* addend_mask);
+                    int bn_mode, const uint8_t* addend_mask, int addend_up, int H, int W);
 int conv_pw_stream_bnb_ok(int kin, int nout, int add, int mode);
 void conv_gen(int dtype, int mode, const void* src, const void* wsrc, const float* bias, void* dst, const int* geom,
               int splits, hipStream_t s);
@@ -295,17 +295,18 @@
   m.def("conv_pw_stream", [](int dt, uintptr_t x, uintptr_t w, uintptr_t y, uintptr_t zero, int M, int kin, int nout,
                              uintptr_t part, int grid, uintptr_t s, uintptr_t addend, int wt, uintptr_t bn_z,
                              uintptr_t bn_mask, uintptr_t bn_mean, uintptr_t bn_scale, uintptr_t bn_shift, int bn_mode,
-                             uintptr_t addend_mask) {
+                             uintptr_t addend_mask, int addend_up, int H, int W) {
     conv_pw_stream(dt, P<const void>(x), P<const void>(w), P<void>(y), P<const void>(zero), M, kin, nout,
                    P<float>(part), grid, S(s), P<const void>(addend), wt, P<const void>(bn_z), P<const uint8_t>(bn_mask),
                    P<const float>(bn_mean), P<const float>(bn_scale), P<const float>(bn_shift), bn_mode,
-                   P<const uint8_t>(addend_mask));
+                   P<const uint8_t>(addend_mask), addend_up, H, W);
     check_launch("conv_pw_stream");
   }, pybind11::arg("dt"), pybind11::arg("x"), pybind11::arg("w"), pybind11::arg("y"), pybind11::arg("zero"),
      pybind11::arg("M"), pybind11::arg("kin"), pybind11::arg("nout"), pybind11::arg("part"), pybind11::arg("grid"),
      pybind11::arg("s"), pybind11::arg("addend"), pybind11::arg("wt") = 0, pybind11::arg("bn_z") = 0,
      pybind11::arg("bn_mask") = 0, pybind11::arg("bn_mean") = 0, pybind11::arg("bn_scale") = 0,
-     pybind11::arg("bn_shift") = 0, pybind11::arg("bn_mode") = 0, pybind11::arg("addend_mask") = 0);
+     pybind11::arg("bn_shift") = 0, pybind11::arg("bn_mode") = 0, pybind11::arg("addend_mask") = 0,
+     pybind11::arg("addend_up") = 0, pybind11::arg("H") = 0, pybind11::arg("W") = 0);
   m.def("conv_pw_stream_bnb_ok", &conv_pw_stream_bnb_ok);
   m.def("conv_gen", [](int dt, int mode, uintptr_t src, uintptr_t wsrc, uintptr_t bias, uintptr_t dst,
                        std::vector<int> geom, int splits, uintptr_t s) {
@@ -558,18 +559,18 @@
                                 int H, int W, int C, int K, int R, int Sf, int sh, int sw, int ph, int pw, int variant,
                                 uintptr_t part, int nparts, uintptr_t addend, uintptr_t s, uintptr_t bz,
                                 uintptr_t bmean, uintptr_t bscale, uintptr_t bshift, uintptr_t bmask, int bmode,
-                                uintptr_t bpart, int bnparts, int up, int dh, int dw) {
+                                uintptr_t bpart, int bnparts, int up, int dh, int dw, int aup) {
     conv_nhwc_fwd_big(dt, P<void>(x), P<void>(w), P<float>(bias), P<void>(y), P<void>(zero), N, H, W, C, K, R, Sf, sh,
                       sw, ph, pw, variant, P<float>(part), nparts, P<void>(addend), S(s), P<void>(bz), P<float>(bmean),
                       P<float>(bscale), P<float>(bshift), P<uint8_t>(bmask), bmode, P<float>(bpart), bnparts, up, dh,
-                      dw);
+                      dw, aup);
     check_launch("conv_nhwc_fwd_big");
   }, py::arg("dt"), py::arg("x"), py::arg("w"), py::arg("bias"), py::arg("y"), py::arg("zero"), py::arg("N"),
      py::arg("H"), py::arg("W"), py::arg("C"), py::arg("K"), py::arg("R"), py::arg("S"), py::arg("sh"),
      py::arg("sw"), py::arg("ph"), py::arg("pw"), py::arg("variant"), py::arg("part"), py::arg("nparts"),
      py::arg("addend"), py::arg("stream"), py::arg("bn_z") = 0, py::arg("bn_mean") = 0, py::arg("bn_scale") = 0,
      py::arg("bn_shift") = 0, py::arg("bn_mask") = 0, py::arg("bn_mode") = 0, py::arg("bn_part") = 0,
-     py::arg("bn_nparts") = 0, py::arg("up") = 0, py::arg("dh") = 1, py::arg("dw") = 1);
+     py::arg("bn_nparts") = 0, py::arg("up") = 0, py::arg("dh") = 1, py::arg("dw") = 1, py::arg("aup") = 0);
   m.def("conv_nhwc_fwd_ring_nparts", &conv_nhwc_fwd_ring_nparts);
   m.def("conv_nhwc_fwd_ring", [](int dt, uintptr_t x, uintptr_t w, uintptr_t y, uintptr_t zero, int N, int H, int W,
                                  int C, int K, int R, int Sf, int sh, int sw, int ph, int pw, int variant, uintptr_t part,
diff --git a/src/kernels/conv_big.hip b/src/kernels/conv_big.hip
--- a/src/kernels/conv_big.hip
+++ b/src/kernels/conv_big.hip
@@ -36,6 +36,7 @@
   int M;
   int Ktot;
   int up;
+  int aup;
   int dh, dw;
 };
 
@@ -317,11 +318,29 @@
     *off = out_pix(p < g.M ? p : 0) * g.K + co0 + c8 * 8;
     return p < g.M;
   };
+  auto ad_load = [&](int it, int64_t off, uint4* dst) {
+    if (g.aup == 2) {
+      const int e = tid + it * 512;
+      const int pl = e / CPR;
+      const int c8 = e - pl * CPR;
+      const int p = pix0 + pl;
+      const int n = p / (g.Ho * g.Wo);
+      const int rem = p - n * g.Ho * g.Wo;
+      const int ho = rem / g.Wo;
+      const int wo = rem - ho * g.Wo;
+      if ((ho | wo) & 1) {
+        *dst = uint4{0u, 0u, 0u, 0u};
+        return;
+      }
+      off = (((int64_t)n * (g.Ho >> 1) + (ho >> 1)) * (g.Wo >> 1) + (wo >> 1)) * g.K + co0 + c8 * 8;
+    }
+    *dst = *reinterpret_cast<const uint4*>(addend + off);
+  };
 #pragma unroll
   for (int it = 0; it < D; ++it) {
     int64_t off;
     const bool ok = row_off(it, &off);
-    if (addend != nullptr && ok) ad_ring[it] = *reinterpret_cast<const uint4*>(addend + off);
+    if (addend != nullptr && ok) ad_load(it, off, &ad_ring[it]);
     if (bnb && ok) z_ring[it] = *reinterpret_cast<const uint4*>(zsrc_b + off);
   }
 #pragma unroll
@@ -336,7 +355,7 @@
     if (it + D < ITERS) {
       int64_t off2;
       const bool ok2 = row_off(it + D, &off2);
-      if (addend != nullptr && ok2) ad_ring[it % D] = *reinterpret_cast<const uint4*>(addend + off2);
+      if (addend != nullptr && ok2) ad_load(it + D, off2, &ad_ring[it % D]);
       if (bnb && ok2) z_ring[it % D] = *reinterpret_cast<const uint4*>(zsrc_b + off2);
     }
     if (ok) {
@@ -476,7 +495,7 @@
                        int H, int W, int C, int K, int R, int S, int sh, int sw, int ph, int pw, int variant,
                        float* part, int nparts, const void* addend, hipStream_t s, const void* bn_z,
                        const float* bn_mean, const float* bn_scale, const float* bn_shift, const uint8_t* bn_mask,
-                       int bn_mode, float* bn_part, int bn_nparts, int up, int dh, int dw) {
+                       int bn_mode, float* bn_part, int bn_nparts, int up, int dh, int dw, int aup) {
   GeomB g;
   g.N = N; g.H = H; g.W = W; g.C = C; g.K = K; g.R = R; g.S = S;
   g.sh = sh; g.sw = sw; g.ph = ph; g.pw = pw;
@@ -490,11 +509,14 @@
   g.M = N * g.Ho * g.Wo;
   g.Ktot = R * S * C;
   g.up = up;
+  g.aup = aup;
   int bco, bpix;
   big_tile(variant, &bco, &bpix);
   MXAMD_HOST_CHECK(C % 64 == 0 && K % bco == 0, "conv_nhwc_fwd_big: need Cin % 64 == 0 and Cout % BCO == 0");
   MXAMD_HOST_CHECK(up == 0 || (up == 2 && addend == nullptr && (int64_t)g.M * 4 * K < (1ll << 31)),
                    "conv_nhwc_fwd_big: the 2x upsampled output takes no addend and must fit 32-bit indexing");
+  MXAMD_HOST_CHECK(aup == 0 || (aup == 2 && addend != nullptr && up == 0 && g.Ho % 2 == 0 && g.Wo % 2 == 0),
+                   "conv_nhwc_fwd_big: a half-resolution addend needs an even Ho and Wo and a dense output");
   MXAMD_HOST_CHECK((int64_t)N * H * W * C < (1ll << 31) && (int64_t)g.M * K < (1ll << 31) &&
                        (int64_t)K * g.Ktot < (1ll << 31),
                    "conv_nhwc_fwd_big: tensor too large for 32-bit indexing");
diff --git a/src/kernels/conv_pw.hip b/src/kernels/conv_pw.hip
--- a/src/kernels/conv_pw.hip
+++ b/src/kernels/conv_pw.hip
@@ -143,11 +143,17 @@
   else vm_wait<0>();
 }
 
-template <typename T, int KIN, int NOUT, bool STATS, bool ADD, int WPC, int S, int BNB, bool AMK = false>
+template <typename T, int KIN, int NOUT, bool STATS, bool ADD, int WPC, int S, int BNB, bool AMK = false,
+          typename... IMG>
 __global__ void __launch_bounds__(512) __attribute__((amdgpu_waves_per_eu(2 * WPC))) conv_pw_stream_kernel(
     const T* __restrict__ x, const T* __restrict__ w, T* __restrict__ y, const T* __restrict__ zero, int M, int ntiles,
-    float* __restrict__ part, const T* __restrict__ addend, int wt, PwBnb bnb) {
+    float* __restrict__ part, const T* __restrict__ addend, int wt, PwBnb bnb, IMG... img) {
   using C = PwCfg<KIN, NOUT, WPC, ADD, BNB, AMK>;
+  constexpr bool AUP = sizeof...(IMG) == 2;
+  static_assert(AUP || sizeof...(IMG) == 0, "IMG is (aH, aW) or empty");
+  const int img_hw[] = {static_cast<int>(img)..., 0, 0};
+  const int aH = img_hw[0], aW = img_hw[1];
+  static_assert(!AUP || (ADD && !AMK && !STATS), "the half-resolution addend is a plain addend");
   constexpr bool EXT = C::EXT;
   extern __shared__ __attribute__((aligned(1024))) char smem[];
   const int tid = threadIdx.x;
@@ -228,7 +234,17 @@
       const int byte = (i * 64 + lane) * 16;
       const int row = byte / (NOUT * 2);
       const int p = t * C::BM + row;
-      const T* src = p < M ? addend + static_cast<int64_t>(p) * NT + slice * NOUT + (byte % (NOUT * 2)) / 2 : zero;
+      const T* src;
+      if (AUP) {
+        const uint32_t q = static_cast<uint32_t>(p) / static_cast<uint32_t>(aW);
+        const uint32_t wx = static_cast<uint32_t>(p) - q * aW;
+        const uint32_t n = q / static_cast<uint32_t>(aH);
+        const uint32_t hx = q - n * aH;
+        const int64_t pc = (static_cast<int64_t>(n) * (aH >> 1) + (hx >> 1)) * (aW >> 1) + (wx >> 1);
+        src = (p < M && !((hx | wx) & 1u)) ? addend + pc * NT + slice * NOUT + (byte % (NOUT * 2)) / 2 : zero;
+      } else {
+        src = p < M ? addend + static_cast<int64_t>(p) * NT + slice * NOUT + (byte % (NOUT * 2)) / 2 : zero;
+      }
       __builtin_amdgcn_global_load_lds((gbl_void*)src, (lds_void*)(sb + C::STAGE_IN + i * 1024), 16, 0, 0);
     }
 #pragma unroll
@@ -425,6 +441,24 @@
   }
 }
 
+template <typename T, int KIN, int NOUT, int S, int BNB>
+void launch_pw_aup(const void* x, const void* w, void* y, const void* zero, int M, float* part, const void* addend,
+                   int grid, hipStream_t s, int wt, const PwBnb& bnb, int aH, int aW) {
+  using C = PwCfg<KIN, NOUT, 1, true, BNB, false>;
+  static_assert(C::SMEM <= C::LDS && C::NST >= 2, "LDS budget / ring depth");
+  static bool set = false;
+  if (!set) {
+    hipFuncSetAttribute(
+        reinterpret_cast<const void*>(&conv_pw_stream_kernel<T, KIN, NOUT, false, true, 1, S, BNB, false, int, int>),
+        hipFuncAttributeMaxDynamicSharedMemorySize, C::SMEM);
+    set = true;
+  }
+  const int ntiles = (M + C::BM - 1) / C::BM;
+  hipLaunchKernelGGL((conv_pw_stream_kernel<T, KIN, NOUT, false, true, 1, S, BNB, false, int, int>), dim3(grid),
+                     dim3(512), C::SMEM, s, static_cast<const T*>(x), static_cast<const T*>(w), static_cast<T*>(y),
+                     static_cast<const T*>(zero), M, ntiles, part, static_cast<const T*>(addend), wt, bnb, aH, aW);
+}
+
 template <typename T, int KIN, int NOUT, int WPC, int S, bool STATS, bool ADD, int BNB = kPwBnbNone, bool AMK = false>
 void launch_pw_v(const void* x, const void* w, void* y, const void* zero, int M, float* part, const void* addend,
                  int grid, hipStream_t s, int wt, const PwBnb& bnb = PwBnb{}) {
@@ -450,10 +484,12 @@
 
 template <typename T, int KIN, int NOUT, int S>
 bool launch_pw_bnb(const void* x, const void* w, void* y, const void* zero, int M, float* part, const void* addend,
-                   int grid, hipStream_t s, int wt, const PwBnb& bnb, int mode) {
+                   int grid, hipStream_t s, int wt, const PwBnb& bnb, int mode, int aup, int aH, int aW) {
   if constexpr ((NOUT / 8) % 16 == 0) {
     if (addend && mode == kPwBnbMask) {
-      if (bnb.amask)
+      if (aup)
+        launch_pw_aup<T, KIN, NOUT, S, kPwBnbMask>(x, w, y, zero, M, part, addend, grid, s, wt, bnb, aH, aW);
+      else if (bnb.amask)
         launch_pw_v<T, KIN, NOUT, 1, S, false, true, kPwBnbMask, true>(x, w, y, zero, M, part, addend, grid, s, wt,
                                                                         bnb);
       else
@@ -461,7 +497,7 @@
       return true;
     }
   }
-  if (!addend && mode == kPwBnbFromZ) {
+  if (!addend && mode == kPwBnbFromZ && !aup) {
     launch_pw_v<T, KIN, NOUT, 1, S, false, false, kPwBnbFromZ>(x, w, y, zero, M, part, addend, grid, s, wt, bnb);
     return true;
   }
@@ -470,10 +506,16 @@
 
 template <typename T, int KIN, int NOUT, int WPC, int S>
 void launch_pw(const void* x, const void* w, void* y, const void* zero, int M, float* part, const void* addend,
-               int grid, hipStream_t s, int wt, const PwBnb* bnb, int mode) {
+               int grid, hipStream_t s, int wt, const PwBnb* bnb, int mode, int aup, int aH, int aW) {
   if (bnb) {
-    MXAMD_HOST_CHECK((launch_pw_bnb<T, KIN, NOUT, S>(x, w, y, zero, M, part, addend, grid, s, wt, *bnb, mode)),
+    MXAMD_HOST_CHECK((launch_pw_bnb<T, KIN, NOUT, S>(x, w, y, zero, M, part, addend, grid, s, wt, *bnb, mode, aup, aH,
+                                                     aW)),
                      "conv_pw_stream: BN-backward variant not built");
+    return;
+  }
+  if (aup) {
+    MXAMD_HOST_CHECK(addend && !part, "conv_pw_stream: a half-resolution addend takes no forward statistics");
+    launch_pw_aup<T, KIN, NOUT, S, kPwBnbNone>(x, w, y, zero, M, part, addend, grid, s, wt, PwBnb{}, aH, aW);
     return;
   }
   using C = PwCfg<KIN, NOUT, WPC>;
@@ -496,11 +538,12 @@
 
 template <typename T>
 bool dispatch_pw(int kin, int nout, const void* x, const void* w, void* y, const void* zero, int M, float* part,
-                 const void* addend, int grid, hipStream_t s, int wt, const PwBnb* bnb, int mode) {
-#define MXAMD_PW_CASE(K, N, W, SL)                                        \
-  if (kin == K && nout == N * SL) {                                       \
-    launch_pw<T, K, N, W, SL>(x, w, y, zero, M, part, addend, grid, s, wt, bnb, mode); \
-    return true;                                                          \
+                 const void* addend, int grid, hipStream_t s, int wt, const PwBnb* bnb, int mode, int aup, int aH,
+                 int aW) {
+#define MXAMD_PW_CASE(K, N, W, SL)                                                                  \
+  if (kin == K && nout == N * SL) {                                                                 \
+    launch_pw<T, K, N, W, SL>(x, w, y, zero, M, part, addend, grid, s, wt, bnb, mode, aup, aH, aW); \
+    return true;                                                                                    \
   }
   MXAMD_PW_SHAPES(MXAMD_PW_CASE)
 #undef MXAMD_PW_CASE
@@ -547,8 +590,11 @@
 void conv_pw_stream(int dtype, const void* x, const void* w, void* y, const void* zero, int M, int kin, int nout,
                     float* part, int grid, hipStream_t s, const void* addend, int wt, const void* bn_z,
                     const uint8_t* bn_mask, const float* bn_mean, const float* bn_scale, const float* bn_shift,
-                    int bn_mode, const uint8_t* addend_mask) {
+                    int bn_mode, const uint8_t* addend_mask, int addend_up, int H, int W) {
   MXAMD_HOST_CHECK(conv_pw_stream_ok(kin, nout), "conv_pw_stream: unsupported (Cin, Cout)");
+  MXAMD_HOST_CHECK(addend_up == 0 || (addend_up == 2 && addend && !addend_mask && H > 0 && W > 0 && H % 2 == 0 &&
+                                      W % 2 == 0 && M > 0 && M % (H * W) == 0),
+                   "conv_pw_stream: a half-resolution addend needs an output image of even H and W with M = N*H*W");
   MXAMD_HOST_CHECK(grid >= 1 && grid % conv_pw_stream_slices(kin, nout) == 0 &&
                    (int64_t)M * nout * 2 < (1ll << 31) - 64 && (int64_t)M * kin < (1ll << 31),
                    "conv_pw_stream: tensor too large for 32-bit offsets");
@@ -563,9 +609,11 @@
     pb = &bnb;
   }
   bool ok = false;
-  if (dtype == kF16) ok = dispatch_pw<__half>(kin, nout, x, w, y, zero, M, part, addend, grid, s, wt, pb, bn_mode);
+  if (dtype == kF16)
+    ok = dispatch_pw<__half>(kin, nout, x, w, y, zero, M, part, addend, grid, s, wt, pb, bn_mode, addend_up, H, W);
   else if (dtype == kBF16)
-    ok = dispatch_pw<__hip_bfloat16>(kin, nout, x, w, y, zero, M, part, addend, grid, s, wt, pb, bn_mode);
+    ok = dispatch_pw<__hip_bfloat16>(kin, nout, x, w, y, zero, M, part, addend, grid, s, wt, pb, bn_mode, addend_up, H,
+                                     W);
   MXAMD_HOST_CHECK(ok, "conv_pw_stream: dtype must be f16 or bf16");
 }
 
```

Result: no change. 12680 images/sec, median of 6 (+0.9%).
